# PeterCalifano/gtsam_PeterCdev

Hardware: AMD Instinct MI355X
Metric: lm_iterations_per_sec (higher is better)
Workload: dtype f64; 1 GPU; bal1723; ordering=schur_nd, replicas=1, parallelism=replicas1

## Files before the change

### gtsam_petercdev_amd/csrc/handle.h

```cpp
#pragma once
#include <hip/hip_runtime.h>

#include <algorithm>
#include <new>
#include <stdexcept>
#include <string>
#include <utility>
#include <vector>

#include "gsx_internal.h"
#include "kernels.h"

#define HIPCHK(ctx, expr)                                                                  \
  do {                                                                                     \
    hipError_t e__ = (expr);                                                               \
    if (e__ != hipSuccess) {                                                               \
      (ctx)->err = std::string(#expr) + ": " + hipGetErrorString(e__);                     \
      return GSX_E_NO_DEVICE;                                                              \
    }                                                                                      \
  } while (0)

namespace gsx {

template <class Tp>
// ... 40 lines not shown
};

enum Phase { PH_LINEARIZE, PH_ASSEMBLE_H, PH_FACTORIZE, PH_BACKSOLVE, PH_LINERR, PH_RETRACT, PH_ERROR,
             PH_FACTOR_SMALL, PH_FACTOR_BIG, PH_FACTOR_LEAF, PH_K_SYRK, PH_K_TRSM, PH_K_POTRF0, PH_K_GATHER,
             PH_K_BACKSOLVE, PH_MARGINALS, PH_M_PREP, PH_M_KT, PH_M_SF, PH_M_FF, PH_M_EMIT, PH_M_LEAF, PH_COUNT };

struct Timer {
  std::vector<std::pair<hipEvent_t, hipEvent_t>> pending, pool;
  double ms = 0;
  int64_t count = 0;
};

}

namespace gsx {

struct Context {
  std::string err;
  int device = 0;
  bool has_device = false;
  hipStream_t stream = nullptr;
  HostProblem P;
  Symbolic S;
  bool has_symbolic = false;
  double relax = GSX_AMALGAMATION_AUTO;
  int relax_max_f = 128;
  std::vector<int> order;

  DevBuf<int> d_var_type, d_var_dim, d_var_state_off, d_var_tan_off, d_f_type, d_f_rows, d_f_key_ptr, d_f_vars,
      d_f_noise_kind, d_f_cols;
  DevBuf<i64> d_f_meas_off, d_f_noise_off, d_f_jac_off;
  DevBuf<double> d_meas, d_noise;
  DevBuf<FactorRec> d_frec;
  DevBuf<int> d_type_list[kNumTypeLists];
  int type_count[kNumTypeLists] = {};
  DevProblem DP{};
  int n_smart = 0;
  DevBuf<int> d_smart_slot, d_smart_status, d_smart_counters;
  DevBuf<double> d_smart_cams, d_smart_cache, d_smart_point;
  SmartDev SD{};
  void smart_begin(bool linearize) {
    if (n_smart) hipMemsetAsync(d_smart_counters.p + (linearize ? 0 : 1), 0, (linearize ? 2 : 1) * sizeof(int), stream);
  }
  DevBuf<i64> d_fr_off, d_cmap_ptr, d_gidx_ptr, d_h_off, d_hmap_ptr, d_term_ptr;
  DevBuf<TermRec> d_terms;
  DevBuf<VarRec> d_var_recs;
  DevBuf<ChildRec> d_child_recs;
  DevBuf<FrontRec> d_front_recs;
  DevBuf<i64> d_cond_last, d_cond_prev;
  DevBuf<int> d_cond_front;
  DevBuf<VarRec> d_fvar_recs;
  DevBuf<LeafRec> d_leaf_recs;
  int leaf_base = 0;
  int lin_err_slice = 0;
  DevBuf<int> d_fr_N, d_fr_F, d_fr_nfv, d_fr_fvar_ptr, d_fvars, d_fr_parent, d_fr_lean, d_fr_child_ptr, d_children, d_cmap,
      d_gidx, d_h_rows, d_hmap, d_h_loc, d_sched, d_hvars;
  DevBuf<BigDesc> d_big;
  DevSymbolic DS{};
  std::vector<std::vector<SmallLaunch>> small_launch;
  std::vector<std::vector<SmallLaunch>> leaf_launch;
  std::vector<int> leaf_max_F;
  std::vector<std::vector<SmallLaunch>> rest_launch;
  DevBuf<int> d_usched, d_rest_ids, d_tree_start, d_tree_up, d_tree_npend, d_tree_pending, d_tree_cursor;
  DevBuf<int> d_bst_roots, d_bst_child_ptr, d_bst_children, d_bst_counters;
  DevBuf<unsigned long long> d_bst_ready;
  int bst_roots = 0, bst_total = 0;
  unsigned bst_epoch = 0;
  struct TreeTier {
    int start0, nstart, max_n, threads;
    size_t med_lds;
  };
  std::vector<TreeTier> tree_tiers;
  DevBuf<i64> d_gt_dst;
  DevBuf<GatherSeg> d_gsegs;
  DevBuf<GatherSrc> d_gsrcs;
  DevBuf<int> d_gt_ld, d_gt_dims, d_gm_task, d_gm_slot, d_gm_nslots;
  DevBuf<double> d_gscratch;
  GatherArgs GA{};
  std::vector<BigLevel> big_level;
  struct ConLevel {
    int first = 0, count = 0, max_n = 0;
  };
  std::vector<ConLevel> con_level;
  std::vector<int> con_desc_of_front;
  DevBuf<ConDesc> d_con_descs;
  DevBuf<int> d_con_own_col_ptr, d_con_own_cols, d_con_own_m, d_con_child, d_con_fwd_map, d_con_iwork;
  DevBuf<i64> d_con_own_jac;
  DevBuf<double> d_con_work;
  ConTables CT{};
  int con_hd_n = 0;
  DevBuf<int> d_con_hd_tan, d_con_hd_ptr;
  DevBuf<i64> d_con_hd_jidx;
  DevBuf<double> d_con_hd_w;
  bool constrained() const { return !S.con_fronts.empty(); }
  std::vector<BigDesc> big_descs;
  int big_max_n = 0, big_max_nfv = 0;
  struct HGroup {
    int begin, count, threads, lds;
    bool global;
  };
  std::vector<HGroup> hgroups;
  DevBuf<int2> d_star_bundles;
  int n_star_bundles = 0;
  bool fused_star_env = true;
  bool fused_star = false;
  struct LeafSplit {
    int sbegin, scount;
    int rbegin, rcount;
  };
  std::vector<LeafSplit> leaf_split;
  DevBuf<StarLeafRec> d_star_recs;
  DevBuf<int> d_star_prow;
  DevBuf<LeafRec> d_leaf_rest_recs;
  DevBuf<int> d_star_rest_vars;
  int n_star_rest = 0;
  struct MargLevel {
    int begin[4], count[4];
  };
  struct MargPlan {
    std::vector<MargLevel> levels;
    DevBuf<MargItem> d_items;
    DevBuf<int2> d_emit;
    DevBuf<int> d_leaves;
    DevBuf<i64> d_out_off;
    int n_emit = 0, n_leaves = 0;
    int64_t total = 0;
    bool ready = false;
    void release() {
      levels.clear();
      d_items.release();
      d_emit.release();
      d_leaves.release();
      d_out_off.release();
      n_emit = n_leaves = 0;
      total = 0;
      ready = false;
    }
  };
  MargPlan marg_all;
  DevBuf<i64> d_marg_slot, d_marg_work;
  DevBuf<double> d_marg_cov;
  bool marg_arena = false;
  int64_t marg_cov_doubles = 0;
  void marg_release() {
    marg_all.release();
    d_marg_slot.release();
    d_marg_work.release();
    d_marg_cov.release();
    marg_arena = false;
    marg_cov_doubles = 0;
  }
  DevBuf<double> d_values, d_trial, d_delta, d_udelta, d_jac, d_H, d_arena, d_hdiag, d_damp, d_partials, d_scalars;
  DevBuf<double> d_dlu, d_dld;
  DevBuf<DevStatus> d_status;
  double* h_scalars = nullptr;
  DevStatus* h_status = nullptr;
  static constexpr int kPartials = 4096;
  int solver_kind = GSX_SOLVER_MULTIFRONTAL;
  gsx_pcg_params pcg_params{};
  PcgWork* pcg = nullptr;
  int64_t pcg_iterations = 0, pcg_solves = 0;
  int64_t pcg_run_iterations = 0;
  bool use_pcg() const { return solver_kind == GSX_SOLVER_PCG; }
  double lm_lambda = 0, lm_factor = 0, lm_error = 0;
  int lm_iterations = 0, lm_inner = 0;
  Timer timers[PH_COUNT];
  int profiling = -1;
  int64_t n_cheirality = 0;
  std::vector<LeafRec> h_leaf_recs;
  std::vector<GatherSeg> h_gsegs;
  std::vector<int> hv_list, hv_group_of_var, hv_pos;
  std::vector<int> fr_sched_pos, fr_group;
  std::vector<int> fr_seg_ptr, fr_segs, seg_level;
  std::vector<int> fr_gm_ptr, fr_gms, gm_level;
  struct PartialScratch {
    DevBuf<int> marked, src_off, lists[kNumTypeLists], hv, ids, gm_task, gm_slot, gm_nslots;
    DevBuf<double> states;
    DevBuf<LeafRec> leaf;
    DevBuf<BigDesc> big;
    DevBuf<GatherSeg> segs;
  } ps;
  hipStream_t bulk = nullptr;
  hipEvent_t bulk_go = nullptr, bulk_done = nullptr;
  size_t leaf_side_group0 = 0;
  bool bulk_pending = false;
  int shard_rank = 0, shard_world = 1;
  gsx_allreduce_fn shard_cb = nullptr;
  void* shard_user = nullptr;
  bool shard_failed = false;
  unsigned sc_dirty = 0;
  DevBuf<int> d_f_active;
  DevBuf<unsigned char> d_own_tan, d_sched_tan, d_own_state;
  DevBuf<double> d_xscal;
  std::vector<double> jac_stage;
  bool sharded() const { return shard_world > 1; }
  DevBuf<unsigned char> d_wf_replaced, d_wf_dirty, d_wf_changed;
  DevBuf<double> d_wf_old;
  DevBuf<int> d_wf_ids;
  bool values_set = false, linearized = false, h_ready = false, hdiag_ready = false, solved = false, damp_ready = false;
  bool lin0_ready = false;
  bool fact_valid = false;
  double fact_lambda = 0.0;
  bool fact_pending = false;
  int damp_kind = -1;
  double damp_min = 0, damp_max = 0;
  bool hstar_ready = true;
  bool values_synced = true;
  bool wf_all_replaced = true, wf_clear_pending = true;
  bool wf_delta_valid = false;
  void values_written() {
    values_set = true;
    values_synced = true;
    linearized = h_ready = solved = false;
  }
  void states_scattered() { values_synced = true; }
  void values_gathered() {
    std::swap(d_values.p, d_trial.p);
    values_synced = true;
  }
  void trial_accepted(bool drop_factorization) {
    std::swap(d_values.p, d_trial.p);
    values_synced = false;
    trial_discarded();
    if (drop_factorization) fact_valid = false;
  }
  void trial_discarded() { linearized = h_ready = solved = false; }
  void blocks_written(bool is_linearization) {
    if (is_linearization) linearized = true;
    else hdiag_ready = false;
    h_ready = false;
    lin0_ready = false;
    fact_valid = false;
    solved = false;
    if (damp_kind != 0) damp_ready = false;
  }
  void some_blocks_written() { lin0_ready = false; }
  void linear_graph_given() { linearized = true; }
  void lin0_computed() { lin0_ready = true; }
  void h_assembled(bool star_complete) {
    h_ready = true;
    hstar_ready = star_complete;
    hdiag_ready = false;
  }
  void hstar_completed() { hstar_ready = true; }
  void hdiag_extracted() { hdiag_ready = true; }
  void panels_reassembled() { hdiag_ready = false; }
  bool damping_is(int kind, double mind, double maxd) const {
    return damp_ready && damp_kind == kind && (kind == 0 || (damp_min == mind && damp_max == maxd));
  }
  void damping_made(int kind, double mind, double maxd) {
    damp_ready = true;
    damp_kind = kind;
    damp_min = mind;
    damp_max = maxd;
  }
  void factorization_queued(double lambda) {
    fact_valid = false;
    fact_pending = true;
    fact_lambda = lambda;
    wf_all_replaced = true;
  }
  void factorization_judged(bool bad) {
    if (fact_pending) fact_valid = !bad;
    else if (bad) fact_valid = false;
    fact_pending = false;
  }
  void factorization_failed() { fact_valid = false; }
  void delta_overwritten() { wf_delta_valid = false; }
  void delta_outdated() { solved = false; }
  void step_solved(bool complete_undamped) {
    solved = true;
    if (complete_undamped) {
      wf_delta_valid = true;
      wf_all_replaced = false;
      wf_clear_pending = true;
    }
  }
  void tree_replaced() {
    h_ready = false;
    solved = false;
    fact_valid = fact_pending = false;
    wf_all_replaced = true;
    wf_delta_valid = false;
    damp_ready = hdiag_ready = false;
    if (sharded()) linearized = false;
  }
  void problem_replaced() {
    has_symbolic = values_set = linearized = h_ready = solved = false;
    fact_valid = fact_pending = hdiag_ready = damp_ready = lin0_ready = false;
    wf_delta_valid = false;
    wf_all_replaced = true;
  }
  void problem_uploaded() {
    has_symbolic = true;
    values_set = true;
    values_synced = true;
  }
  void update_finished(bool kept_linearization) { linearized = kept_linearization; }
  hipError_t wf_flags_ready(hipStream_t st) {
    const size_t nf = (size_t)std::max(S.n_fronts, 1);
    if (d_wf_replaced.n != nf) {
      hipError_t e = d_wf_replaced.alloc(nf);
      if (e != hipSuccess) return e;
      wf_clear_pending = true;
    }
    if (wf_clear_pending) {
      hipError_t e = hipMemsetAsync(d_wf_replaced.p, 0, nf, st);
      if (e != hipSuccess) return e;
      wf_clear_pending = false;
    }
    return hipSuccess;
  }
};

int factor_type_list(const HostProblem& P, int f);
void whiten_linear_factor(const HostProblem& P, int f, const double* src, double* J);
gsx_status upload_problem(gsx_context* c);
gsx_status upload_symbolic(gsx_context* c);
void launch_lds_group(const DevProblem& P, const DevSymbolic& S, const int* ids, const SmallLaunch& g, const double* H,
                      const double* damp, const double* scalars, double* arena, DevStatus* status, hipStream_t st);
void timer_begin(gsx_context* c, int ph);
void timer_end(gsx_context* c, int ph);
void dev_linearize(gsx_context* c);
void dev_assemble_h(gsx_context* c);
void dev_ensure_hstar(gsx_context* c);
void dev_damping(gsx_context* c, int diagonal, double mind, double maxd);
void dev_big_factor(gsx_context* c, const BigDesc* descs, int count, const BigPlan& plan, hipStream_t st, bool prof);
void dev_backsolve(gsx_context* c, const WildfireArgs* wf = nullptr);
void dev_linear_error(gsx_context* c, bool solved_step = false);
void dev_retract(gsx_context* c, const double* d_delta);
void dev_error(gsx_context* c, const double* d_vals, int slot);
gsx_status readback(gsx_context* c);
bool factorization_ok(const gsx_context* c);
gsx_status compute_error_sync(gsx_context* c, double* out);
gsx_status need_device(gsx_context* c);
gsx_status begin_call(gsx_context* c, bool need_values, bool need_symbolic);
gsx_status indeterminate(gsx_context* c, uint64_t* bad_key, bool also_nonfinite);
gsx_status download(gsx_context* c, const double* src, double* out, int64_t n);
enum HMode { H_KEEP, H_IF_STALE, H_ALWAYS };
void direct_solve(gsx_context* c, HMode hm, int diagonal, double mind, double maxd, double lambda, bool backsolve);
gsx_status damped_step(gsx_context* c, HMode hm, int diagonal, double mind, double maxd, double lambda);

}

struct gsx_context : gsx::Context {};

#define GSX_GUARD(h, call)                          \
  try {                                             \
    return (call);                                  \
  } catch (const std::bad_alloc&) {                 \
    if (h) (h)->err = "out of host memory";         \
    return GSX_E_NOMEM;                             \
  } catch (const std::exception& e) {               \
    if (h) (h)->err = e.what();                     \
    return GSX_E_INVALID;                           \
  }
```

### gtsam_petercdev_amd/csrc/kernels.h

```cpp
#pragma once
#include <hip/hip_runtime.h>

#include <cstdint>
#include <vector>

#include "../../include/gsx.h"

namespace gsx {

typedef long long i64;

struct FactorRec {
  i64 jac_off;
  int s0, s1;
  int meas_off, noise_off;
  int type_kind;
  int rows_dim;
};
struct DevProblem {
  int n_vars, n_factors;
  const int *var_type, *var_dim, *var_state_off, *var_tan_off;
  const int *f_type, *f_rows, *f_key_ptr, *f_vars, *f_noise_kind, *f_cols;
  const i64 *f_meas_off, *f_noise_off, *f_jac_off;
  const double *meas, *noise;
  const FactorRec* frec;
  const int* f_active;
  int n_active;
};

struct TermRec {
  i64 jac;
  int m, colA, colB, dB, dst, pad;
};

struct VarRec {
  i64 h_off, hmap_off;
  int dA, rows, loc, toff;
};
struct LeafRec {
  i64 off, h_off, hmap_off, gidx_ptr;
  int n, F, nfv, lean;
  int dA, rows, loc, toff;
  int fvar_ptr, front, pad0, pad1;
};
constexpr int kStarMaxD = 3;
struct StarLeafRec {
  i64 off, h_off, t0;
  i64 jac0, prow_off;
  int n, nf, d, toff;
  int colA, colB, colR, dB;
  int front, jstride, rrow, pad0;
};
struct ChildRec {
  i64 src0, cmap_off;
  int nc, s1, pad0, pad1;
};
struct FrontRec {
  i64 off;
  int n, F, nfv, fvar_ptr, child_ptr, nchild;
};

struct DevSymbolic {
  int n_fronts;
  const i64* fr_off;
  const int *fr_N, *fr_F, *fr_nfv, *fr_fvar_ptr, *fvars, *fr_parent, *fr_child_ptr, *children;
  const int* fr_lean;
  const i64 *cmap_ptr, *gidx_ptr;
  const int *cmap, *gidx;
  const i64 *h_off, *hmap_ptr;
  const int *h_rows, *hmap, *h_loc;
  const i64* term_ptr;
  const TermRec* terms;
  const VarRec* var_recs;
  const ChildRec* child_recs;
  const FrontRec* front_recs;
  const VarRec* fvar_recs;
  unsigned char* wf_dirty;
  const unsigned char *wf_replaced, *wf_changed;
};
#ifdef __HIPCC__
__device__ __forceinline__ bool wildfire_skip(const DevSymbolic& S, int f, bool writer) {
  if (S.wf_dirty == nullptr) return false;
  const int p = S.fr_parent[f];
  bool dirty = (p < 0) || S.wf_dirty[p];
  if (dirty && !S.wf_replaced[f]) {
    dirty = false;
    for (int q = S.fr_fvar_ptr[f] + S.fr_nfv[f]; q < S.fr_fvar_ptr[f + 1]; ++q)
      if (S.wf_changed[S.fvars[q]]) {
        dirty = true;
        break;
      }
  }
  if (writer) S.wf_dirty[f] = dirty ? 1 : 0;
  return !dirty;
}
#endif

struct DevStatus {
  int n_fail;
  int first_front;
  int n_nonfinite;
  int n_cheirality;
  int n_backsub;
};

constexpr int kXScalars = 16;
constexpr unsigned kXFact = 1u << 12, kXLin = 1u << 13;
void launch_shard_pack(const double* scalars, const DevStatus* status, unsigned dirty, double* x, hipStream_t st);
void launch_shard_unpack(const double* x, unsigned dirty, double* scalars, DevStatus* status, hipStream_t st);
void launch_scatter_states(const DevProblem& P, const int* vars, const int* src_off, int n, const double* src,
                           double* values, hipStream_t st);
void launch_mask_copy(const double* in, const unsigned char* mask, int64_t n, double* out, hipStream_t st);

enum { SC_LAMBDA = 0, SC_ERR = 1, SC_LIN0 = 2, SC_LIND = 3, SC_TRIAL_ERR = 4, SC_DOT0 = 5, SC_DOT1 = 6, SC_DOT2 = 7,
       SC_DOT3 = 8, SC_LIN0_LOCAL = 9 , SC_COUNT = 12 };

struct BigDesc {
  i64 off, xoff;
  int N, F, front, parent;
};
constexpr int kStandaloneFront = -3;
void launch_cond_check(int n, const i64* last, const i64* prev, const int* front, const double* arena, DevStatus* status,
                       hipStream_t st);
__host__ __device__ inline i64 big_panel_offset(int n) { return ((i64)n * n + 1) & ~(i64)1; }

enum { TL_SFM = 0, TL_BETWEEN_POSE2 = 1, TL_BETWEEN_POSE3 = 2, TL_GENERIC = 3, TL_PROJECTION = 4, TL_BEARINGRANGE = 5,
       TL_RANGE_POSE2_POINT = 6, TL_RANGE_POSE2_POSE = 7, TL_RANGE_POSE3_POINT = 8, TL_RANGE_POSE3_POSE = 9,
       TL_BEARING = 10, TL_STEREO = 11,
       TL_PROJECTION_SENSOR = 12, TL_STEREO_SENSOR = 13, TL_RANGE_POSE2_POINT_SENSOR = 14, TL_RANGE_POSE2_POSE_SENSOR = 15,
       TL_RANGE_POSE3_POINT_SENSOR = 16, TL_RANGE_POSE3_POSE_SENSOR = 17, TL_SFM2 = 18,
       TL_SMART = 19, kNumTypeLists = 20 };
constexpr int kSensorListShift = TL_RANGE_POSE2_POINT_SENSOR - TL_RANGE_POSE2_POINT;
inline int type_list_of(int t, int vt0, int vt1, long long nmeas) {
  switch (t) {
    case GSX_F_LINEAR: return -1;
    case GSX_F_SFM: return TL_SFM;
    case GSX_F_SFM2: return TL_SFM2;
    case GSX_F_PROJECTION: return nmeas > 7 ? TL_PROJECTION_SENSOR : TL_PROJECTION;
    case GSX_F_BEARINGRANGE: return TL_BEARINGRANGE;
    case GSX_F_BETWEEN: return vt0 == GSX_VAR_POSE2 ? TL_BETWEEN_POSE2 : (vt0 == GSX_VAR_POSE3 ? TL_BETWEEN_POSE3 : TL_GENERIC);
    case GSX_F_RANGE:
      return (vt0 == GSX_VAR_POSE2 ? (vt1 == GSX_VAR_POSE2 ? TL_RANGE_POSE2_POSE : TL_RANGE_POSE2_POINT)
                                   : (vt1 == GSX_VAR_POSE3 ? TL_RANGE_POSE3_POSE : TL_RANGE_POSE3_POINT)) +
             (nmeas > 1 ? kSensorListShift : 0);
    case GSX_F_BEARING: return TL_BEARING;
    case GSX_F_STEREO: return nmeas > 9 ? TL_STEREO_SENSOR : TL_STEREO;
    case GSX_F_SMART_PROJECTION: return TL_SMART;
  }
  return TL_GENERIC;
}
struct SmartDev {
  const int* slot;
  double* cams;
  double* cache;
  double* point;
  int* status;
  int* counters;
  int n;
};
void launch_linearize(const DevProblem& P, const int* const type_lists[kNumTypeLists], const int type_counts[kNumTypeLists],
                      const double* values, double* jac, DevStatus* status, hipStream_t st, const SmartDev* smart = nullptr);
void launch_error(const DevProblem& P, const int* const type_lists[kNumTypeLists], const int type_counts[kNumTypeLists],
                  const double* values, double* partials, int n_partials_cap, double* scalars, int slot, hipStream_t st,
                  const SmartDev* smart = nullptr);
void launch_smart_triangulate(const DevProblem& P, const int* list, int n, const double* values, const SmartDev& S, hipStream_t st);
void launch_smart_linearize(const DevProblem& P, const int* list, int n, const SmartDev& S, double* jac, hipStream_t st);
void launch_smart_error(const DevProblem& P, const int* list, int n, const SmartDev& S, double* partials, int blocks,
                        hipStream_t st);
void launch_linear_error(const DevProblem& P, const double* jac, const double* delta, double* partials,
                         int n_partials_cap, double* scalars, int slice, hipStream_t st);
void launch_lin0(const DevProblem& P, const double* jac, double* partials, int cap, double* scalars, hipStream_t st);
void launch_model_error(const DevProblem& P, const DevSymbolic& S, const int* vars, int nvars, const double* H,
                        const double* delta, const double* damp, double* partials, int cap, double* scalars, hipStream_t st);
void launch_retract(const DevProblem& P, const double* values, const double* delta, double* out, hipStream_t st);
void launch_assemble_h_group(const DevProblem& P, const DevSymbolic& S, const int* vars, int count, int threads,
                             int lds_bytes, bool global, const double* jac, double* H, hipStream_t st);
void launch_assemble_h_star_bundles(const DevProblem& P, const DevSymbolic& S, const int* vars, const int2* bundles,
                                    int count, const double* jac, double* H, hipStream_t st);
void launch_assemble_h_diag_star(const DevProblem& P, const DevSymbolic& S, const int* dvars, int dcount, const int* svars,
                                 const int2* bundles, int scount, const double* jac, double* H, hipStream_t st);
void launch_hessian_diag(const DevProblem& P, const DevSymbolic& S, const double* H, double* diag, hipStream_t st);
void launch_make_damping(int n, const double* hdiag, int diagonal, double mind, double maxd, double* damp,
                         hipStream_t st);
void launch_front_small(const DevProblem& P, const DevSymbolic& S, const int* ids, int count, int max_n,
                        int threads, const double* H, const double* damp, const double* scalars, double* arena,
                        DevStatus* status, hipStream_t st);
struct TreeArgs {
  const int* start;
  int nstart;
  int* cursor;
  int* pending;
  const int *up, *npend;
};
void launch_front_tree(const DevProblem& P, const DevSymbolic& S, const TreeArgs& T, int max_n, int threads, const double* H,
                       const double* damp, const double* scalars, double* arena, DevStatus* status, hipStream_t st);
void launch_front_medium(const DevProblem& P, const DevSymbolic& S, const int* ids, int count, int max_panel, int max_n,
                         const double* H, const double* damp, const double* scalars, double* arena, DevStatus* status,
                         hipStream_t st);
void launch_front_tree_med(const DevProblem& P, const DevSymbolic& S, const TreeArgs& T, size_t lds_bytes, const double* H,
                           const double* damp, const double* scalars, double* arena, DevStatus* status, hipStream_t st);
void launch_big_init(const DevProblem& P, const DevSymbolic& S, const BigDesc* descs, int count, int max_n,
                     int max_nfv, const double* H, const double* damp, const double* scalars, double* arena,
                     hipStream_t st);
struct BigPlan {
  int chunk = 0;
  std::vector<int> fw, rb, pairs;
  int rounds() const { return (int)fw.size(); }
};
void plan_big_group(const BigDesc* host_descs, int count, BigPlan& plan);
void launch_big_diag(const BigDesc* descs, int count, const BigPlan& plan, int round, double* arena, DevStatus* status,
                     hipStream_t st);
#ifdef GSX_STAMP
void big_stamp_dump(const char* what);
#endif
size_t big_rows_lds(int fw, long tiles, int cus, int* rows);
void launch_big_rows(const BigDesc* descs, int count, const BigPlan& plan, int round, double* arena, DevStatus* status,
                     hipStream_t st);
void launch_big_schur(const BigDesc* descs, int count, const BigPlan& plan, int round, double* arena, hipStream_t st);
void launch_front_leaf(const DevProblem& P, const DevSymbolic& S, const LeafRec* recs, int count, int max_panel, int threads,
                       const double* H, const double* damp, const double* scalars, double* arena, DevStatus* status,
                       hipStream_t st);
void launch_front_star_leaf(const DevSymbolic& S, const StarLeafRec* recs, int count, const int* prow, const double* jac,
                            const double* damp, const double* scalars, double* H, double* arena, DevStatus* status,
                            hipStream_t st);
struct GatherSrc {
  i64 off;
  int d2;
  int ldF;
};
struct GatherSeg {
  i64 dst;
  i64 src;
  int n, ld, dims;
  int slot;
};
struct GatherArgs {
  const GatherSeg* segs;
  const GatherSrc* srcs;
  const i64* gt_dst;
  const int *gt_ld, *gt_dims, *gm_task, *gm_slot, *gm_nslots;
  double* scratch;
};
void launch_big_gather(const GatherArgs& G, int seg0, int nseg, int m0, int nm, double* arena, hipStream_t st);
void launch_backsolve(const DevSymbolic& S, const int* ids, int count, int threads, int max_n, const double* arena,
                      double* delta, DevStatus* status, hipStream_t st);
size_t backsolve_big_lds(int max_n, int max_F, int max_sep_rows);
void launch_backsolve_big(const DevSymbolic& S, const int* ids, int count, int max_n, int max_F, const double* arena,
                          double* delta, DevStatus* status, hipStream_t st);
bool backsolve_small_fits(int max_n, int max_F);
void launch_backsolve_small(const DevSymbolic& S, const int* ids, int count, int max_F, const double* arena, double* delta,
                            DevStatus* status, hipStream_t st);
struct BacksolveTreeArgs {
  const int* roots;
  int n_roots, n_tickets;
  const int *child_ptr, *children;
  unsigned long long* ready;
  int *head, *tail;
  unsigned epoch;
};
void launch_backsolve_tree(const DevSymbolic& S, const BacksolveTreeArgs& Q, const double* arena, double* delta,
                           DevStatus* status, hipStream_t st);
struct WildfireArgs {
  const unsigned char *replaced, *dirty;
  unsigned char* changed;
  const double* old_delta;
  DevStatus* status;
  double threshold;
};
void launch_mark_fronts(const int* ids, int count, unsigned char* flags, hipStream_t st);
void launch_wildfire_post(const DevSymbolic& S, const int* ids, int count, bool wave_per_clique, const WildfireArgs& W,
                          double* delta, hipStream_t st);
void launch_backsolve_leaf(const DevSymbolic& S, const LeafRec* recs, int count, int max_F, const double* arena,
                           double* delta, DevStatus* status, hipStream_t st);
void launch_gradient(const DevProblem& P, const DevSymbolic& S, const double* H, double* g, hipStream_t st);
void launch_ax_sqnorm(const DevProblem& P, const double* jac, const double* x, double* partials, int cap, double* scalars,
                      int slot, hipStream_t st);
void launch_vec_dot(const double* a, const double* b, int64_t n, double* partials, int cap, double* scalars, int slot,
                    hipStream_t st);
void launch_vec_axpby(double* out, double alpha, const double* a, double beta, const double* b, int64_t n, hipStream_t st);
void launch_marginal_path(const DevSymbolic& S, const int* path, int npath, int loc, int dA, int max_n, const double* arena,
                          double* out, double* Y, int64_t n_tan, hipStream_t st);
void launch_joint_cross(const double* Ya, const double* Yb, int64_t n_tan, int dA, int dB, double* out, hipStream_t st);
struct MargItem {
  int front, ti, tj, pad;
};
struct MargArgs {
  const i64 *slot, *work;
  double* cov;
  const double* arena;
  const i64* out_off;
  const int* var_dim;
  double* out;
};
void launch_marg_prep(const DevSymbolic& S, const MargArgs& M, const MargItem* items, int count, hipStream_t st);
void launch_marg_kt(const DevSymbolic& S, const MargArgs& M, const MargItem* items, int count, hipStream_t st);
void launch_marg_sf(const DevSymbolic& S, const MargArgs& M, const MargItem* items, int count, hipStream_t st);
void launch_marg_ff(const DevSymbolic& S, const MargArgs& M, const MargItem* items, int count, hipStream_t st);
void launch_marg_emit(const DevSymbolic& S, const MargArgs& M, const int2* vars, int count, hipStream_t st);
void launch_marg_leaf(const DevSymbolic& S, const MargArgs& M, const int* ids, int count, hipStream_t st);
void launch_set_scalar(double* scalars, int slot, double v, hipStream_t st);
struct ConDesc {
  i64 off;
  i64 work, fwd;
  i64 iwork;
  int N, F, K, n_fwd;
  int own_begin, own_end;
  int child_begin, child_end;
  int front;
  int fwd_map;
};
struct ConTables {
  const ConDesc* descs;
  const int *own_col_ptr, *own_cols, *own_m;
  const i64* own_jac;
  const int* child_list;
  const int* fwd_map;
  double* work;
  int* iwork;
};
void launch_constraint_fronts(const DevSymbolic& S, const ConTables& T, int first, int count, int max_n, const double* jac,
                              double* arena, DevStatus* status, hipStream_t st);
void launch_constraint_hdiag(int n, const int* tan, const int* ptr, const i64* jidx, const double* w, const double* jac,
                             double* hdiag, hipStream_t st);
constexpr int kTreeCursors = 8;
void launch_begin_factorization(double* scalars, double lambda, DevStatus* status, int* tree_cursors, hipStream_t st);
void launch_dense_partial(double* a, int n, int nf, DevStatus* status, hipStream_t st);
// ... 25 lines not shown
```

### gtsam_petercdev_amd/csrc/kernels.hip

```cpp
#include <hip/hip_runtime.h>

#include <climits>
#include <cstdio>
#include <cstdlib>

#include "device_geometry.h"
#include "gsx_internal.h"
#include "kernels.h"

namespace gsx {
using namespace gsxd;

#define T kTile

__device__ __forceinline__ double wave_sum(double v) {
#pragma unroll
  for (int o = 32; o > 0; o >>= 1) v += __shfl_down(v, o, 64);
  return v;
}
typedef double v4d __attribute__((ext_vector_type(4)));
__device__ __forceinline__ i64 readlane_i64(i64 v, int src_lane) {
  int lo = (int)(v & 0xFFFFFFFFll), hi = (int)(v >> 32);
  lo = __builtin_amdgcn_readlane(lo, src_lane);
  hi = __builtin_amdgcn_readlane(hi, src_lane);
// ... 56 lines not shown
#pragma unroll
    for (int c = 0; c < NC; ++c)
#pragma unroll
      for (int r = 0; r < M; ++r) J[c * M + r] *= inv[r];
  } else if (kind == GSX_NOISE_GAUSSIAN) {
    double R[M * M];
#pragma unroll
    for (int i = 0; i < M * M; ++i) R[i] = np[i];
#pragma unroll
    for (int c = 0; c < NC; ++c) {
      double col[M];
#pragma unroll
      for (int r = 0; r < M; ++r) {
        double s = 0;
#pragma unroll
        for (int k = r; k < M; ++k) s += R[r * M + k] * J[c * M + k];
        col[r] = s;
      }
#pragma unroll
      for (int r = 0; r < M; ++r) J[c * M + r] = col[r];
    }
  }
  if (loss) {
    double s = 0;
#pragma unroll
    for (int r = 0; r < M; ++r) s += J[(NC - 1) * M + r] * J[(NC - 1) * M + r];
    const double w = sqrt(robust_weight(loss, np[noise_base_params(kind, M)], sqrt(s)));
#pragma unroll
    for (int i = 0; i < M * NC; ++i) J[i] *= w;
  }
  if constexpr ((M * NC) % 2 == 0) {
    if ((reinterpret_cast<size_t>(out) & 15) == 0) {
      double2* out2 = reinterpret_cast<double2*>(out);
#pragma unroll
      for (int i = 0; i < M * NC / 2; ++i) out2[i] = double2{J[2 * i], J[2 * i + 1]};
      return;
    }
  }
#pragma unroll
  for (int i = 0; i < M * NC; ++i) out[i] = J[i];
}

template <int M>
__device__ __forceinline__ double whitened_half_sqnorm(double (&e)[M], int kind_full, const double* np) {
  const int kind = kind_full & GSX_NOISE_BASE_MASK, loss = kind_full >> 4;
  double s = 0;
  if (kind == GSX_NOISE_UNIT) {
#pragma unroll
    for (int r = 0; r < M; ++r) s += e[r] * e[r];
  } else if (kind == GSX_NOISE_ISOTROPIC) {
    const double inv = 1.0 / np[0];
#pragma unroll
    for (int r = 0; r < M; ++r) s += (e[r] * inv) * (e[r] * inv);
  } else if (kind == GSX_NOISE_DIAGONAL) {
#pragma unroll
    for (int r = 0; r < M; ++r) {
      const double x = e[r] * (1.0 / np[r]);
      s += x * x;
    }
  } else {
#pragma unroll
    for (int r = 0; r < M; ++r) {
      double x = 0;
#pragma unroll
      for (int k = r; k < M; ++k) x += np[r * M + k] * e[k];
      s += x * x;
    }
  }
  if (loss) return robust_loss(loss, np[noise_base_params(kind, M)], sqrt(s));
  return 0.5 * s;
}

__device__ inline void whiten_inplace(double* J, int m, int nc, int kind_full, const double* np) {
  const int kind = kind_full & GSX_NOISE_BASE_MASK, loss = kind_full >> 4;
  if (kind == GSX_NOISE_UNIT) {
  } else if (kind == GSX_NOISE_ISOTROPIC) {
    const double inv = 1.0 / np[0];
    for (int i = 0; i < m * nc; ++i) J[i] *= inv;
  } else if (kind == GSX_NOISE_DIAGONAL) {
    for (int c = 0; c < nc; ++c)
      for (int r = 0; r < m; ++r) J[c * m + r] *= (1.0 / np[r]);
  } else {
    for (int c = 0; c < nc; ++c)
      for (int r = 0; r < m; ++r) {
        double s = 0;
        for (int k = r; k < m; ++k) s += np[r * m + k] * J[c * m + k];
        J[c * m + r] = s;
      }
  }
  if (loss) {
    double s = 0;
    for (int r = 0; r < m; ++r) s += J[(nc - 1) * m + r] * J[(nc - 1) * m + r];
    const double w = sqrt(robust_weight(loss, np[noise_base_params(kind, m)], sqrt(s)));
    for (int i = 0; i < m * nc; ++i) J[i] *= w;
  }
}

__device__ inline void local_coords(int type, int dim, const double* x, const double* y, double* out) {
  if (type == GSX_VAR_VECTOR) {
    for (int i = 0; i < dim; ++i) out[i] = y[i] - x[i];
  } else if (type == GSX_VAR_POSE2) {
    const P2 h = compose(inverse(load_pose2(x)), load_pose2(y));
    out[0] = h.x; out[1] = h.y; out[2] = theta(h);
  } else {
    pose3_logmap(between(load_pose3(x), load_pose3(y)), out);
    if (type == GSX_VAR_CAMERA) {
      out[6] = y[12] - x[12]; out[7] = y[13] - x[13]; out[8] = y[14] - x[14];
    }
  }
}

__device__ __forceinline__ void linearize_generic_body(const DevProblem& P, const int* list, int n, const double* values,
                                                       double* jac, int bid);
__global__ void __launch_bounds__(256) linearize_sfm_kernel(DevProblem P, const int* list, int n, const double* values,
                                                            double* jac, DevStatus* status, const int* glist, int gn) {
  const int gb = (gn + 255) >> 8;
  if ((int)blockIdx.x < gb) {
    linearize_generic_body(P, glist, gn, values, jac, blockIdx.x);
    return;
  }
  const int i = ((int)blockIdx.x - gb) * blockDim.x + threadIdx.x;
  if (i >= n) return;
  const int f = list[i];
  const FactorRec fr = P.frec[f];
  const double* cam = values + fr.s0;
  const double* pt = values + fr.s1;
  const double* z = P.meas + fr.meas_off;
  double camr[17], ptr3[3], pi[2], H1[18], H2[6], J[26];
#pragma unroll
  for (int k = 0; k < 17; ++k) camr[k] = cam[k];
  ptr3[0] = pt[0]; ptr3[1] = pt[1]; ptr3[2] = pt[2];
  const bool ok = sfm_project(camr, ptr3, pi, H1, H2);
  if (ok) {
#pragma unroll
    for (int c = 0; c < 9; ++c) {
      J[2 * c] = H1[c];
      J[2 * c + 1] = H1[9 + c];
    }
#pragma unroll
    for (int c = 0; c < 3; ++c) {
      J[18 + 2 * c] = H2[c];
      J[18 + 2 * c + 1] = H2[3 + c];
    }
    J[24] = z[0] - pi[0];
    J[25] = z[1] - pi[1];
  } else {
#pragma unroll
    for (int k = 0; k < 26; ++k) J[k] = 0;
    atomicAdd(&status->n_cheirality, 1);
  }
  whiten_store<2, 13>(J, (fr.type_kind >> 8) & 0xffff, P.noise + fr.noise_off, jac + fr.jac_off);
}

__global__ void __launch_bounds__(256) linearize_bearingrange_kernel(DevProblem P, const int* list, int n,
                                                                     const double* values, double* jac) {
  const int i = blockIdx.x * blockDim.x + threadIdx.x;
  if (i >= n) return;
  const int f = list[i];
  const int kp = P.f_key_ptr[f];
  const double* pose = values + P.var_state_off[P.f_vars[kp]];
  const double* pt = values + P.var_state_off[P.f_vars[kp + 1]];
  const double* z = P.meas + P.f_meas_off[f];
  double ps[3] = {pose[0], pose[1], pose[2]}, p2[2] = {pt[0], pt[1]}, br[2], H1[6], H2[4], J[12];
  bearing_range_2d(ps, p2, br, H1, H2);
#pragma unroll
  for (int c = 0; c < 3; ++c) {
    J[2 * c] = H1[c];
    J[2 * c + 1] = H1[3 + c];
  }
#pragma unroll
  for (int c = 0; c < 2; ++c) {
    J[6 + 2 * c] = H2[c];
    J[6 + 2 * c + 1] = H2[2 + c];
  }
  J[10] = -wrap_angle(br[0] - z[0]);
  J[11] = -(br[1] - z[1]);
  whiten_store<2, 6>(J, P.f_noise_kind[f], P.noise + P.f_noise_off[f], jac + P.f_jac_off[f]);
}

template <bool SENSOR>
__global__ void __launch_bounds__(256) linearize_projection_kernel(DevProblem P, const int* list, int n, const double* values,
                                                                   double* jac, DevStatus* status) {
  const int i = blockIdx.x * blockDim.x + threadIdx.x;
  if (i >= n) return;
  const int f = list[i];
  const int kp = P.f_key_ptr[f];
  const double* pose = values + P.var_state_off[P.f_vars[kp]];
  const double* pt = values + P.var_state_off[P.f_vars[kp + 1]];
  const double* z = P.meas + P.f_meas_off[f];
  double pr[12], p3[3], K[5], pi[2], H1[12], H2[6], J[20];
#pragma unroll
  for (int k = 0; k < 12; ++k) pr[k] = pose[k];
  p3[0] = pt[0]; p3[1] = pt[1]; p3[2] = pt[2];
#pragma unroll
  for (int k = 0; k < 5; ++k) K[k] = z[2 + k];
  if constexpr (SENSOR) pose3_compose_sensor(pr, z + 7);
  if (pinhole_project_s2(pr, p3, K, pi, H1, H2)) {
    if constexpr (SENSOR) {
      row_times_sensor_adjoint(H1, z + 7);
      row_times_sensor_adjoint(H1 + 6, z + 7);
    }
#pragma unroll
    for (int c = 0; c < 6; ++c) {
      J[2 * c] = H1[c];
      J[2 * c + 1] = H1[6 + c];
    }
#pragma unroll
    for (int c = 0; c < 3; ++c) {
      J[12 + 2 * c] = H2[c];
      J[12 + 2 * c + 1] = H2[3 + c];
    }
    J[18] = z[0] - pi[0];
    J[19] = z[1] - pi[1];
  } else {
#pragma unroll
    for (int k = 0; k < 18; ++k) J[k] = 0;
    J[18] = J[19] = -2.0 * K[0];
    if constexpr (SENSOR) atomicAdd(&status->n_cheirality, 1);
  }
  whiten_store<2, 10>(J, P.f_noise_kind[f], P.noise + P.f_noise_off[f], jac + P.f_jac_off[f]);
}

__global__ void __launch_bounds__(256) linearize_between_pose2_kernel(DevProblem P, const int* list, int n,
                                                                      const double* values, double* jac, const int* glist,
                                                                      int gn) {
  const int gb = (gn + 255) >> 8;
  if ((int)blockIdx.x < gb) {
    linearize_generic_body(P, glist, gn, values, jac, blockIdx.x);
    return;
  }
  const int i = ((int)blockIdx.x - gb) * blockDim.x + threadIdx.x;
  if (i >= n) return;
  const int f = list[i];
  const FactorRec fr = P.frec[f];
  const P2 x1 = load_pose2(values + fr.s0);
  const P2 x2 = load_pose2(values + fr.s1);
  const P2 h = compose(inverse(x1), x2);
  const P2 zh = compose(inverse(load_pose2(P.meas + fr.meas_off)), h);
  const P2 hi = inverse(h);
  double J[21];
  J[0] = -hi.c; J[1] = -hi.s; J[2] = 0;
  J[3] = hi.s; J[4] = -hi.c; J[5] = 0;
  J[6] = -hi.y; J[7] = hi.x; J[8] = -1;
  J[9] = 1; J[10] = 0; J[11] = 0;
  J[12] = 0; J[13] = 1; J[14] = 0;
  J[15] = 0; J[16] = 0; J[17] = 1;
  J[18] = -zh.x; J[19] = -zh.y; J[20] = -theta(zh);
  whiten_store<3, 7>(J, (fr.type_kind >> 8) & 0xffff, P.noise + fr.noise_off, jac + fr.jac_off);
}

__global__ void __launch_bounds__(256) linearize_between_pose3_kernel(DevProblem P, const int* list, int n,
                                                                      const double* values, double* jac, const int* glist,
                                                                      int gn) {
  const int gb = (gn + 255) >> 8;
  if ((int)blockIdx.x < gb) {
    linearize_generic_body(P, glist, gn, values, jac, blockIdx.x);
    return;
  }
  const int i = ((int)blockIdx.x - gb) * blockDim.x + threadIdx.x;
  if (i >= n) return;
  const int f = list[i];
  const FactorRec fr = P.frec[f];
  const P3 x1 = load_pose3(values + fr.s0);
  const P3 x2 = load_pose3(values + fr.s1);
  const P3 h = between(x1, x2);
  const P3 zh = compose(inverse(load_pose3(P.meas + fr.meas_off)), h);
  double e[6], Ad[36], J[78];
  pose3_logmap(zh, e);
  pose3_adjoint(inverse(h), Ad);
#pragma unroll
  for (int c = 0; c < 6; ++c)
#pragma unroll
    for (int r = 0; r < 6; ++r) {
      J[c * 6 + r] = -Ad[6 * r + c];
      J[36 + c * 6 + r] = (r == c) ? 1.0 : 0.0;
    }
#pragma unroll
  for (int r = 0; r < 6; ++r) J[72 + r] = -e[r];
  whiten_store<6, 13>(J, (fr.type_kind >> 8) & 0xffff, P.noise + fr.noise_off, jac + fr.jac_off);
}

__device__ __forceinline__ void linearize_generic_body(const DevProblem& P, const int* list, int n, const double* values,
                                                       double* jac, int bid) {
  const int i = bid * blockDim.x + threadIdx.x;
  if (i >= n) return;
  const int f = list[i];
  const int kp = P.f_key_ptr[f];
  const int m = P.f_rows[f];
  double* J = jac + P.f_jac_off[f];
  const double* z = P.meas + P.f_meas_off[f];
  if (P.f_type[f] == GSX_F_PRIOR) {
    const int v = P.f_vars[kp];
    double l[9];
    local_coords(P.var_type[v], P.var_dim[v], values + P.var_state_off[v], z, l);
    for (int c = 0; c < m; ++c)
      for (int r = 0; r < m; ++r) J[c * m + r] = (r == c) ? 1.0 : 0.0;
    for (int r = 0; r < m; ++r) J[m * m + r] = l[r];
    whiten_inplace(J, m, m + 1, P.f_noise_kind[f], P.noise + P.f_noise_off[f]);
  } else {
    const double* x1 = values + P.var_state_off[P.f_vars[kp]];
    const double* x2 = values + P.var_state_off[P.f_vars[kp + 1]];
    for (int c = 0; c < m; ++c)
      for (int r = 0; r < m; ++r) {
        J[c * m + r] = (r == c) ? -1.0 : 0.0;
        J[m * m + c * m + r] = (r == c) ? 1.0 : 0.0;
      }
    for (int r = 0; r < m; ++r) J[2 * m * m + r] = -((x2[r] - x1[r]) - z[r]);
    whiten_inplace(J, m, 2 * m + 1, P.f_noise_kind[f], P.noise + P.f_noise_off[f]);
  }
}
__global__ void linearize_generic_kernel(DevProblem P, const int* list, int n, const double* values, double* jac) {
  linearize_generic_body(P, list, n, values, jac, blockIdx.x);
}

template <int V1, int V2, bool SENSOR>
__global__ void __launch_bounds__(256) linearize_range_kernel(DevProblem P, const int* list, int n, const double* values,
                                                              double* jac) {
  const int i = blockIdx.x * blockDim.x + threadIdx.x;
  if (i >= n) return;
  const FactorRec fr = P.frec[list[i]];
  const double* a1 = values + fr.s0;
  const double* a2 = values + fr.s1;
  const double z = P.meas[fr.meas_off];
  if constexpr (V1 == GSX_VAR_POSE2) {
    constexpr int NC = (V2 == GSX_VAR_POSE2) ? 7 : 6;
    double ps[3] = {a1[0], a1[1], a1[2]}, p2[2] = {a2[0], a2[1]}, H1[3], Dd[2], J[NC];
    double r;
    if constexpr (SENSOR) {
      r = range_2d_cs(pose2_compose_sensor(ps, P.meas + fr.meas_off + 1), p2, H1, Dd);
      row_times_sensor_adjoint2(H1, P.meas + fr.meas_off + 1);
    } else {
      r = range_2d(ps, p2, H1, Dd);
    }
    J[0] = H1[0]; J[1] = H1[1]; J[2] = H1[2];
    if constexpr (V2 == GSX_VAR_POSE2) {
      const double c2 = cos(a2[2]), s2 = sin(a2[2]);
      J[3] = Dd[0] * c2 + Dd[1] * s2; J[4] = -Dd[0] * s2 + Dd[1] * c2; J[5] = 0.0;
    } else {
      J[3] = Dd[0]; J[4] = Dd[1];
    }
    J[NC - 1] = -(r - z);
    whiten_store<1, NC>(J, (fr.type_kind >> 8) & 0xffff, P.noise + fr.noise_off, jac + fr.jac_off);
  } else {
    constexpr int NC = (V2 == GSX_VAR_POSE3) ? 13 : 10;
    constexpr int TO = (V2 == GSX_VAR_POSE3) ? 9 : 0;
    double pr[12], p3[3] = {a2[TO], a2[TO + 1], a2[TO + 2]}, H1[6], H2[3], J[NC];
#pragma unroll
    for (int k = 0; k < 12; ++k) pr[k] = a1[k];
    if constexpr (SENSOR) pose3_compose_sensor(pr, P.meas + fr.meas_off + 1);
    const double r = range_3d(pr, p3, H1, H2);
    if constexpr (SENSOR) row_times_sensor_adjoint(H1, P.meas + fr.meas_off + 1);
#pragma unroll
    for (int c = 0; c < 6; ++c) J[c] = H1[c];
    if constexpr (V2 == GSX_VAR_POSE3) {
      J[6] = J[7] = J[8] = 0.0;
#pragma unroll
      for (int c = 0; c < 3; ++c) J[9 + c] = H2[0] * a2[c] + H2[1] * a2[3 + c] + H2[2] * a2[6 + c];
    } else {
      J[6] = H2[0]; J[7] = H2[1]; J[8] = H2[2];
    }
    J[NC - 1] = -(r - z);
    whiten_store<1, NC>(J, (fr.type_kind >> 8) & 0xffff, P.noise + fr.noise_off, jac + fr.jac_off);
  }
}

__global__ void __launch_bounds__(256) linearize_bearing_kernel(DevProblem P, const int* list, int n, const double* values,
                                                                double* jac) {
  const int i = blockIdx.x * blockDim.x + threadIdx.x;
  if (i >= n) return;
  const FactorRec fr = P.frec[list[i]];
  const double* pose = values + fr.s0;
  const double* pt = values + fr.s1;
  double ps[3] = {pose[0], pose[1], pose[2]}, p2[2] = {pt[0], pt[1]}, br[2], H1[6], H2[4], J[6];
  bearing_range_2d(ps, p2, br, H1, H2);
  J[0] = H1[0]; J[1] = H1[1]; J[2] = H1[2];
  J[3] = H2[0]; J[4] = H2[1];
  J[5] = -wrap_angle(br[0] - P.meas[fr.meas_off]);
  whiten_store<1, 6>(J, (fr.type_kind >> 8) & 0xffff, P.noise + fr.noise_off, jac + fr.jac_off);
}

template <bool SENSOR>
__global__ void __launch_bounds__(256) linearize_stereo_kernel(DevProblem P, const int* list, int n, const double* values,
                                                               double* jac, DevStatus* status) {
  const int i = blockIdx.x * blockDim.x + threadIdx.x;
  if (i >= n) return;
  const FactorRec fr = P.frec[list[i]];
  const double* pose = values + fr.s0;
  const double* pt = values + fr.s1;
  const double* z = P.meas + fr.meas_off;
  double pr[12], p3[3], K[6], pi[3], H1[18], H2[9], J[30];
#pragma unroll
  for (int k = 0; k < 12; ++k) pr[k] = pose[k];
  p3[0] = pt[0]; p3[1] = pt[1]; p3[2] = pt[2];
#pragma unroll
  for (int k = 0; k < 6; ++k) K[k] = z[3 + k];
  if constexpr (SENSOR) pose3_compose_sensor(pr, z + 9);
  if (stereo_project(pr, p3, K, pi, H1, H2)) {
    if constexpr (SENSOR) {
#pragma unroll
      for (int r = 0; r < 3; ++r) row_times_sensor_adjoint(H1 + 6 * r, z + 9);
    }
#pragma unroll
    for (int c = 0; c < 6; ++c)
#pragma unroll
      for (int r = 0; r < 3; ++r) J[3 * c + r] = H1[6 * r + c];
#pragma unroll
    for (int c = 0; c < 3; ++c)
#pragma unroll
      for (int r = 0; r < 3; ++r) J[18 + 3 * c + r] = H2[3 * r + c];
#pragma unroll
    for (int r = 0; r < 3; ++r) J[27 + r] = z[r] - pi[r];
  } else {
#pragma unroll
    for (int k = 0; k < 27; ++k) J[k] = 0;
    J[27] = J[28] = J[29] = -2.0 * K[0];
    if constexpr (SENSOR) atomicAdd(&status->n_cheirality, 1);
  }
  whiten_store<3, 10>(J, (fr.type_kind >> 8) & 0xffff, P.noise + fr.noise_off, jac + fr.jac_off);
}

__global__ void __launch_bounds__(256) linearize_sfm2_kernel(DevProblem P, const int* list, int n, const double* values,
                                                             double* jac, DevStatus* status) {
  const int i = blockIdx.x * blockDim.x + threadIdx.x;
  if (i >= n) return;
  const int f = list[i];
  const FactorRec fr = P.frec[f];
  const double* pose = values + fr.s0;
  const double* pt = values + fr.s1;
  const double* cal = values + P.var_state_off[P.f_vars[P.f_key_ptr[f] + 2]];
  const double* z = P.meas + fr.meas_off;
  double pr[12], p3[3], K[5], pi[2], H1[12], H2[6], H3[10], J[30];
#pragma unroll
  for (int k = 0; k < 12; ++k) pr[k] = pose[k];
  p3[0] = pt[0]; p3[1] = pt[1]; p3[2] = pt[2];
#pragma unroll
  for (int k = 0; k < 5; ++k) K[k] = cal[k];
  if (pinhole_project_s2_cal(pr, p3, K, pi, H1, H2, H3)) {
#pragma unroll
    for (int c = 0; c < 6; ++c) {
      J[2 * c] = H1[c];
      J[2 * c + 1] = H1[6 + c];
    }
#pragma unroll
    for (int c = 0; c < 3; ++c) {
      J[12 + 2 * c] = H2[c];
      J[12 + 2 * c + 1] = H2[3 + c];
    }
#pragma unroll
    for (int c = 0; c < 5; ++c) {
      J[18 + 2 * c] = H3[c];
      J[18 + 2 * c + 1] = H3[5 + c];
    }
    J[28] = z[0] - pi[0];
    J[29] = z[1] - pi[1];
  } else {
#pragma unroll
    for (int k = 0; k < 30; ++k) J[k] = 0;
    atomicAdd(&status->n_cheirality, 1);
  }
  whiten_store<2, 15>(J, (fr.type_kind >> 8) & 0xffff, P.noise + fr.noise_off, jac + fr.jac_off);
}

void launch_linearize(const DevProblem& P, const int* const type_lists[kNumTypeLists], const int type_counts[kNumTypeLists],
                      const double* values, double* jac, DevStatus* status, hipStream_t st, const SmartDev* smart) {
  auto grid = [](int n) { return dim3((n + 255) / 256); };
  const int* glist = type_lists[3];
  int gn = type_counts[3];
  auto take = [&](int n) {
    const int g = gn;
    gn = 0;
    return std::make_pair(dim3((n + 255) / 256 + (g + 255) / 256), g);
  };
  if (type_counts[0]) {
    const auto gg = take(type_counts[0]);
    linearize_sfm_kernel<<<gg.first, 256, 0, st>>>(P, type_lists[0], type_counts[0], values, jac, status, glist, gg.second);
  }
  if (type_counts[1]) {
    const auto gg = take(type_counts[1]);
    linearize_between_pose2_kernel<<<gg.first, 256, 0, st>>>(P, type_lists[1], type_counts[1], values, jac, glist, gg.second);
  }
  if (type_counts[2]) {
    const auto gg = take(type_counts[2]);
    linearize_between_pose3_kernel<<<gg.first, 256, 0, st>>>(P, type_lists[2], type_counts[2], values, jac, glist, gg.second);
  }
  if (gn) linearize_generic_kernel<<<grid(gn), 256, 0, st>>>(P, glist, gn, values, jac);
  if (type_counts[4])
    linearize_projection_kernel<false><<<grid(type_counts[4]), 256, 0, st>>>(P, type_lists[4], type_counts[4], values, jac,
                                                                             status);
  if (type_counts[5])
    linearize_bearingrange_kernel<<<grid(type_counts[5]), 256, 0, st>>>(P, type_lists[5], type_counts[5], values, jac);
  auto run = [&](auto kernel, int k) {
    if (type_counts[k]) kernel<<<grid(type_counts[k]), 256, 0, st>>>(P, type_lists[k], type_counts[k], values, jac);
  };
  run(linearize_range_kernel<GSX_VAR_POSE2, GSX_VAR_VECTOR, false>, TL_RANGE_POSE2_POINT);
  run(linearize_range_kernel<GSX_VAR_POSE2, GSX_VAR_POSE2, false>, TL_RANGE_POSE2_POSE);
  run(linearize_range_kernel<GSX_VAR_POSE3, GSX_VAR_VECTOR, false>, TL_RANGE_POSE3_POINT);
  run(linearize_range_kernel<GSX_VAR_POSE3, GSX_VAR_POSE3, false>, TL_RANGE_POSE3_POSE);
  run(linearize_bearing_kernel, TL_BEARING);
  auto run_s = [&](auto kernel, int k) {
    if (type_counts[k]) kernel<<<grid(type_counts[k]), 256, 0, st>>>(P, type_lists[k], type_counts[k], values, jac, status);
  };
  run_s(linearize_stereo_kernel<false>, TL_STEREO);
  run_s(linearize_projection_kernel<true>, TL_PROJECTION_SENSOR);
  run_s(linearize_stereo_kernel<true>, TL_STEREO_SENSOR);
  run(linearize_range_kernel<GSX_VAR_POSE2, GSX_VAR_VECTOR, true>, TL_RANGE_POSE2_POINT_SENSOR);
  run(linearize_range_kernel<GSX_VAR_POSE2, GSX_VAR_POSE2, true>, TL_RANGE_POSE2_POSE_SENSOR);
  run(linearize_range_kernel<GSX_VAR_POSE3, GSX_VAR_VECTOR, true>, TL_RANGE_POSE3_POINT_SENSOR);
  run(linearize_range_kernel<GSX_VAR_POSE3, GSX_VAR_POSE3, true>, TL_RANGE_POSE3_POSE_SENSOR);
  run_s(linearize_sfm2_kernel, TL_SFM2);
  if (type_counts[TL_SMART] && smart) {
    launch_smart_triangulate(P, type_lists[TL_SMART], type_counts[TL_SMART], values, *smart, st);
    launch_smart_linearize(P, type_lists[TL_SMART], type_counts[TL_SMART], *smart, jac, st);
  }
}

template <int FT = -1, int FV = -1, bool SENSOR = false>
__device__ inline double factor_error(const DevProblem& P, int f, const double* values) {
  const FactorRec fr = P.frec[f];
  const int type = FT >= 0 ? FT : (fr.type_kind & 0xff);
  if (type == GSX_F_LINEAR) return 0.0;
  const int kind = (fr.type_kind >> 8) & 0xffff;
  const double* np = P.noise + fr.noise_off;
  const double* z = P.meas + fr.meas_off;
  if (type == GSX_F_SFM) {
    const double* cam = values + fr.s0;
    const double* pt = values + fr.s1;
    double camr[17], ptr3[3], pi[2], e[2];
#pragma unroll
    for (int k = 0; k < 17; ++k) camr[k] = cam[k];
    ptr3[0] = pt[0]; ptr3[1] = pt[1]; ptr3[2] = pt[2];
    if (!sfm_project(camr, ptr3, pi, nullptr, nullptr)) return 0.0;
    e[0] = pi[0] - z[0];
    e[1] = pi[1] - z[1];
    return whitened_half_sqnorm<2>(e, kind, np);
  }
  if (type == GSX_F_BEARINGRANGE) {
    const double* pose = values + fr.s0;
    const double* pt = values + fr.s1;
    double ps[3] = {pose[0], pose[1], pose[2]}, p2[2] = {pt[0], pt[1]}, br[2], e[2];
    bearing_range_2d(ps, p2, br, nullptr, nullptr);
    e[0] = wrap_angle(br[0] - z[0]);
    e[1] = br[1] - z[1];
    return whitened_half_sqnorm<2>(e, kind, np);
  }
  if (type == GSX_F_PROJECTION) {
    const double* pose = values + fr.s0;
    const double* pt = values + fr.s1;
    double pr[12], p3[3], K[5], pi[2], e[2];
#pragma unroll
    for (int k = 0; k < 12; ++k) pr[k] = pose[k];
    p3[0] = pt[0]; p3[1] = pt[1]; p3[2] = pt[2];
#pragma unroll
    for (int k = 0; k < 5; ++k) K[k] = z[2 + k];
    if constexpr (SENSOR) pose3_compose_sensor(pr, z + 7);
    if (pinhole_project_s2(pr, p3, K, pi, nullptr, nullptr)) {
      e[0] = pi[0] - z[0];
      e[1] = pi[1] - z[1];
    } else {
      e[0] = e[1] = 2.0 * K[0];
    }
    return whitened_half_sqnorm<2>(e, kind, np);
  }
  if constexpr (FT == GSX_F_RANGE && FV == GSX_VAR_POSE2) {
    const double* a1 = values + fr.s0;
    const double* a2 = values + fr.s1;
    double ps[3] = {a1[0], a1[1], a1[2]}, p2[2] = {a2[0], a2[1]}, e[1];
    if constexpr (SENSOR) e[0] = range_2d_cs(pose2_compose_sensor(ps, z + 1), p2, nullptr, nullptr) - z[0];
    else e[0] = range_2d(ps, p2, nullptr, nullptr) - z[0];
    return whitened_half_sqnorm<1>(e, kind, np);
  }
  if constexpr (FT == GSX_F_RANGE && FV == GSX_VAR_POSE3) {
    const double* a1 = values + fr.s0;
    const double* a2 = values + fr.s1 + ((fr.rows_dim >> 16) == 13 ? 9 : 0);
    double pr[12], p3[3] = {a2[0], a2[1], a2[2]}, e[1];
#pragma unroll
    for (int k = 0; k < 12; ++k) pr[k] = a1[k];
    if constexpr (SENSOR) pose3_compose_sensor(pr, z + 1);
    e[0] = range_3d(pr, p3, nullptr, nullptr) - z[0];
    return whitened_half_sqnorm<1>(e, kind, np);
  }
  if constexpr (FT == GSX_F_BEARING) {
    const double* pose = values + fr.s0;
    const double* pt = values + fr.s1;
    double ps[3] = {pose[0], pose[1], pose[2]}, p2[2] = {pt[0], pt[1]}, br[2], e[1];
    bearing_range_2d(ps, p2, br, nullptr, nullptr);
    e[0] = wrap_angle(br[0] - z[0]);
    return whitened_half_sqnorm<1>(e, kind, np);
  }
  if constexpr (FT == GSX_F_STEREO) {
    const double* pose = values + fr.s0;
    const double* pt = values + fr.s1;
    double pr[12], p3[3], K[6], pi[3], e[3];
#pragma unroll
    for (int k = 0; k < 12; ++k) pr[k] = pose[k];
    p3[0] = pt[0]; p3[1] = pt[1]; p3[2] = pt[2];
#pragma unroll
    for (int k = 0; k < 6; ++k) K[k] = z[3 + k];
    if constexpr (SENSOR) pose3_compose_sensor(pr, z + 9);
    if (stereo_project(pr, p3, K, pi, nullptr, nullptr)) {
#pragma unroll
      for (int r = 0; r < 3; ++r) e[r] = pi[r] - z[r];
    } else {
      e[0] = e[1] = e[2] = 2.0 * K[0];
    }
    return whitened_half_sqnorm<3>(e, kind, np);
  }
  if constexpr (FT == GSX_F_SFM2) {
    const double* pose = values + fr.s0;
    const double* pt = values + fr.s1;
    const double* cal = values + P.var_state_off[P.f_vars[P.f_key_ptr[f] + 2]];
    double pr[12], p3[3], K[5], pi[2], e[2];
#pragma unroll
    for (int k = 0; k < 12; ++k) pr[k] = pose[k];
    p3[0] = pt[0]; p3[1] = pt[1]; p3[2] = pt[2];
#pragma unroll
    for (int k = 0; k < 5; ++k) K[k] = cal[k];
    if (!pinhole_project_s2(pr, p3, K, pi, nullptr, nullptr)) return 0.0;
    e[0] = pi[0] - z[0];
    e[1] = pi[1] - z[1];
    return whitened_half_sqnorm<2>(e, kind, np);
  }
  const int vt = FV >= 0 ? FV : ((fr.type_kind >> 24) & 0xff);
  if (type == GSX_F_BETWEEN && vt == GSX_VAR_POSE2) {
    const P2 h = compose(inverse(load_pose2(values + fr.s0)), load_pose2(values + fr.s1));
    const P2 zh = compose(inverse(load_pose2(z)), h);
    double e[3] = {zh.x, zh.y, theta(zh)};
    return whitened_half_sqnorm<3>(e, kind, np);
  }
  if (type == GSX_F_BETWEEN && vt == GSX_VAR_POSE3) {
    const P3 h = between(load_pose3(values + fr.s0), load_pose3(values + fr.s1));
    double e[6];
    pose3_logmap(compose(inverse(load_pose3(z)), h), e);
    return whitened_half_sqnorm<6>(e, kind, np);
  }
  const int m = fr.rows_dim & 0xff;
  double e[9];
  if (type == GSX_F_PRIOR) {
    local_coords(vt, (fr.rows_dim >> 8) & 0xff, values + fr.s0, z, e);
  } else {
    const double* x1 = values + fr.s0;
    const double* x2 = values + fr.s1;
    for (int r = 0; r < m; ++r) e[r] = (x2[r] - x1[r]) - z[r];
  }
  const int base = kind & GSX_NOISE_BASE_MASK, loss = kind >> 4;
  double s = 0;
  for (int r = 0; r < m; ++r) {
    double x;
    if (base == GSX_NOISE_UNIT) x = e[r];
    else if (base == GSX_NOISE_ISOTROPIC) x = e[r] * (1.0 / np[0]);
    else if (base == GSX_NOISE_DIAGONAL) x = e[r] * (1.0 / np[r]);
    else {
      x = 0;
      for (int k = r; k < m; ++k) x += np[r * m + k] * e[k];
    }
    s += x * x;
  }
  if (loss) return robust_loss(loss, np[noise_base_params(base, m)], sqrt(s));
  return 0.5 * s;
}

__global__ void __launch_bounds__(256) reduce_final_kernel(const double* partials, int n, int stride, double* scalars,
                                                           int slot) {
  double acc = 0;
  for (int i = threadIdx.x; i < n; i += blockDim.x) acc += partials[(size_t)i * stride];
  const double s = block_sum(acc);
  if (threadIdx.x == 0) scalars[slot] = s;
}

__global__ void __launch_bounds__(256) reduce_final_pair_kernel(const double* partials, int n, double* scalars, int slot0) {
  double acc = 0;
  for (int i = threadIdx.x; i < n; i += blockDim.x) acc += partials[(size_t)i * 2 + blockIdx.x];
  const double s = block_sum(acc);
  if (threadIdx.x == 0) scalars[slot0 + blockIdx.x] = s;
}

template <int FT, int FV, bool SENSOR = false>
__global__ void __launch_bounds__(256) error_list_kernel(DevProblem P, const int* list, int n, const double* values,
                                                         double* partials) {
  double acc = 0;
  for (int i = blockIdx.x * blockDim.x + threadIdx.x; i < n; i += gridDim.x * blockDim.x)
    acc += factor_error<FT, FV, SENSOR>(P, list[i], values);
  const double s = block_sum(acc);
  if (threadIdx.x == 0) partials[blockIdx.x] = s;
}

void launch_error(const DevProblem& P, const int* const type_lists[kNumTypeLists],
                  const int type_counts[kNumTypeLists], const double* values, double* partials, int cap, double* scalars,
                  int slot, hipStream_t st, const SmartDev* smart) {
  long long total = 0;
  for (int k = 0; k < kNumTypeLists; ++k) total += type_counts[k];
  bool new_lists = false;
  for (int k = TL_PROJECTION_SENSOR; k < TL_SMART; ++k) new_lists = new_lists || type_counts[k] > 0;
  const int held = type_counts[TL_SMART] > 0 ? kNumTypeLists : (new_lists ? TL_SMART : TL_PROJECTION_SENSOR);
  int off = 0;
  for (int k = 0; k < kNumTypeLists; ++k) {
    const int n = type_counts[k];
    if (!n) continue;
    int nb = (n + 255) / 256;
    const int share = (int)std::max<long long>(1, (long long)(cap - held) * n / std::max<long long>(total, 1));
    nb = std::min(nb, share);
    double* out = partials + off;
    switch (k) {
      case 0: error_list_kernel<GSX_F_SFM, GSX_VAR_CAMERA><<<nb, 256, 0, st>>>(P, type_lists[k], n, values, out); break;
      case 1: error_list_kernel<GSX_F_BETWEEN, GSX_VAR_POSE2><<<nb, 256, 0, st>>>(P, type_lists[k], n, values, out); break;
      case 2: error_list_kernel<GSX_F_BETWEEN, GSX_VAR_POSE3><<<nb, 256, 0, st>>>(P, type_lists[k], n, values, out); break;
      case 4: error_list_kernel<GSX_F_PROJECTION, GSX_VAR_POSE3><<<nb, 256, 0, st>>>(P, type_lists[k], n, values, out); break;
      case 5: error_list_kernel<GSX_F_BEARINGRANGE, GSX_VAR_POSE2><<<nb, 256, 0, st>>>(P, type_lists[k], n, values, out); break;
      case TL_RANGE_POSE2_POINT:
      case TL_RANGE_POSE2_POSE: error_list_kernel<GSX_F_RANGE, GSX_VAR_POSE2><<<nb, 256, 0, st>>>(P, type_lists[k], n, values, out); break;
      case TL_RANGE_POSE3_POINT:
      case TL_RANGE_POSE3_POSE: error_list_kernel<GSX_F_RANGE, GSX_VAR_POSE3><<<nb, 256, 0, st>>>(P, type_lists[k], n, values, out); break;
      case TL_BEARING: error_list_kernel<GSX_F_BEARING, GSX_VAR_POSE2><<<nb, 256, 0, st>>>(P, type_lists[k], n, values, out); break;
      case TL_STEREO: error_list_kernel<GSX_F_STEREO, GSX_VAR_POSE3><<<nb, 256, 0, st>>>(P, type_lists[k], n, values, out); break;
      case TL_PROJECTION_SENSOR: error_list_kernel<GSX_F_PROJECTION, GSX_VAR_POSE3, true><<<nb, 256, 0, st>>>(P, type_lists[k], n, values, out); break;
      case TL_STEREO_SENSOR: error_list_kernel<GSX_F_STEREO, GSX_VAR_POSE3, true><<<nb, 256, 0, st>>>(P, type_lists[k], n, values, out); break;
      case TL_RANGE_POSE2_POINT_SENSOR:
      case TL_RANGE_POSE2_POSE_SENSOR: error_list_kernel<GSX_F_RANGE, GSX_VAR_POSE2, true><<<nb, 256, 0, st>>>(P, type_lists[k], n, values, out); break;
      case TL_RANGE_POSE3_POINT_SENSOR:
      case TL_RANGE_POSE3_POSE_SENSOR: error_list_kernel<GSX_F_RANGE, GSX_VAR_POSE3, true><<<nb, 256, 0, st>>>(P, type_lists[k], n, values, out); break;
      case TL_SFM2: error_list_kernel<GSX_F_SFM2, GSX_VAR_POSE3><<<nb, 256, 0, st>>>(P, type_lists[k], n, values, out); break;
      case TL_SMART:
        launch_smart_triangulate(P, type_lists[k], n, values, *smart, st);
        launch_smart_error(P, type_lists[k], n, *smart, out, nb, st);
        break;
      default: error_list_kernel<-1, -1><<<nb, 256, 0, st>>>(P, type_lists[k], n, values, out); break;
    }
    off += nb;
  }
  reduce_final_kernel<<<1, 256, 0, st>>>(partials, off, 1, scalars, slot);
}

__global__ void __launch_bounds__(256) linear_error_kernel(DevProblem P, const double* jac, const double* delta,
                                                           double* partials) {
  double acc0 = 0, accd = 0;
  for (int i = blockIdx.x * blockDim.x + threadIdx.x; i < P.n_active; i += gridDim.x * blockDim.x) {
    const int f = P.f_active ? P.f_active[i] : i;
    const int m = P.f_rows[f], nc = P.f_cols[f];
    const double* J = jac + P.f_jac_off[f];
    if (m == 2 && (P.f_jac_off[f] & 1) == 0) {
      const double2* J2 = reinterpret_cast<const double2*>(J);
      const double2 b = J2[nc - 1];
      double e0 = -b.x, e1 = -b.y;
      int col = 0;
      for (int k = P.f_key_ptr[f]; k < P.f_key_ptr[f + 1]; ++k) {
        const int v = P.f_vars[k];
        const double* x = delta + P.var_tan_off[v];
        const int d = P.var_dim[v];
        for (int c = 0; c < d; ++c, ++col) {
          const double2 j = J2[col];
          e0 += j.x * x[c];
          e1 += j.y * x[c];
        }
      }
      acc0 += b.x * b.x;
      accd += e0 * e0;
      acc0 += b.y * b.y;
      accd += e1 * e1;
      continue;
    }
    for (int r = 0; r < m; ++r) {
      const double b = J[(nc - 1) * m + r];
      double e = -b;
      int col = 0;
      for (int k = P.f_key_ptr[f]; k < P.f_key_ptr[f + 1]; ++k) {
        const int v = P.f_vars[k];
        const double* x = delta + P.var_tan_off[v];
        const int d = P.var_dim[v];
        for (int c = 0; c < d; ++c, ++col) e += J[col * m + r] * x[c];
      }
      acc0 += b * b;
      accd += e * e;
    }
  }
  const double s0 = block_sum(0.5 * acc0);
  const double sd = block_sum(0.5 * accd);
  if (threadIdx.x == 0) {
    partials[2 * blockIdx.x] = s0;
    partials[2 * blockIdx.x + 1] = sd;
  }
}

__global__ void __launch_bounds__(128) linear_error_staged_kernel(DevProblem P, const double* jac, const double* delta,
                                                                  double* partials, int slice) {
  extern __shared__ double stage[];
  const int wave = threadIdx.x >> 6, lane = threadIdx.x & 63;
  double* W = stage + (size_t)wave * slice;
  const int ngroups = (P.n_factors + 63) >> 6;
  double acc0 = 0, accd = 0;
  for (int g = blockIdx.x * 2 + wave; g < ngroups; g += gridDim.x * 2) {
    const int i0 = g * 64;
    const bool live = i0 + lane < P.n_factors;
    const int f = live ? i0 + lane : P.n_factors - 1;
    const int m = P.f_rows[f], nc = P.f_cols[f];
    const i64 off = P.f_jac_off[f];
    const i64 base = readlane_i64(off, 0);
    const int last = min(63, P.n_factors - 1 - i0);
    const int len = (int)(readlane_i64(off + (i64)m * nc, last) - base);
    const double* src = jac + base;
    for (int e0 = lane; e0 < len; e0 += 64 * 8) {
      double v[8];
#pragma unroll
      for (int u = 0; u < 8; ++u) v[u] = (e0 + 64 * u < len) ? src[e0 + 64 * u] : 0.0;
#pragma unroll
      for (int u = 0; u < 8; ++u)
        if (e0 + 64 * u < len) W[e0 + 64 * u] = v[u];
    }
    asm volatile("s_waitcnt lgkmcnt(0)" ::: "memory");
    __builtin_amdgcn_wave_barrier();
    if (live) {
      const double* J = W + (off - base);
      for (int r = 0; r < m; ++r) {
        const double b = J[(nc - 1) * m + r];
        double e = -b;
        int col = 0;
        for (int k = P.f_key_ptr[f]; k < P.f_key_ptr[f + 1]; ++k) {
          const int v = P.f_vars[k];
          const double* x = delta + P.var_tan_off[v];
          const int d = P.var_dim[v];
          for (int c = 0; c < d; ++c, ++col) e += J[col * m + r] * x[c];
        }
        acc0 += b * b;
        accd += e * e;
      }
    }
    asm volatile("s_waitcnt lgkmcnt(0)" ::: "memory");
    __builtin_amdgcn_wave_barrier();
  }
  const double s0 = block_sum(0.5 * acc0);
  const double sd = block_sum(0.5 * accd);
  if (threadIdx.x == 0) {
    partials[2 * blockIdx.x] = s0;
    partials[2 * blockIdx.x + 1] = sd;
  }
}

void launch_linear_error(const DevProblem& P, const double* jac, const double* delta, double* partials, int cap,
                         double* scalars, int slice, hipStream_t st) {
  int nb;
  if (slice > 0 && !P.f_active) {
    static bool attr = false;
    if (!attr) {
      hipFuncSetAttribute((const void*)linear_error_staged_kernel, hipFuncAttributeMaxDynamicSharedMemorySize, 128 * 1024);
      attr = true;
    }
    nb = ((P.n_factors + 63) / 64 + 1) / 2;
    nb = nb < 1 ? 1 : (nb > cap / 2 ? cap / 2 : nb);
    linear_error_staged_kernel<<<nb, 128, (size_t)2 * slice * sizeof(double), st>>>(P, jac, delta, partials, slice);
  } else {
    nb = (P.n_active + 255) / 256;
    nb = nb < 1 ? 1 : (nb > cap / 2 ? cap / 2 : nb);
    linear_error_kernel<<<nb, 256, 0, st>>>(P, jac, delta, partials);
  }
  static_assert(SC_LIND == SC_LIN0 + 1, "the two linearized errors are reduced by one launch, a block each");
  reduce_final_pair_kernel<<<2, 256, 0, st>>>(partials, nb, scalars, SC_LIN0);
}

__global__ void __launch_bounds__(256) lin0_kernel(DevProblem P, const double* jac, double* partials) {
  double acc = 0;
  for (int k = blockIdx.x * blockDim.x + threadIdx.x; k < P.n_active; k += gridDim.x * blockDim.x) {
    const int f = P.f_active ? P.f_active[k] : k;
    const FactorRec fr = P.frec[f];
    const int m = fr.rows_dim & 0xff;
    const double* b = jac + fr.jac_off + (i64)m * (int)(((unsigned)fr.rows_dim >> 16) - 1u);
    double s = 0;
    for (int r = 0; r < m; ++r) s += b[r] * b[r];
    acc += 0.5 * s;
  }
  const double t = block_sum(acc);
  if (threadIdx.x == 0) partials[blockIdx.x] = t;
}
__global__ void __launch_bounds__(256) model_error_kernel(DevProblem P, DevSymbolic S, const int* vars, int nvars,
                                                          const double* H, const double* delta, const double* damp,
                                                          const double* scalars, double* partials) {
  const double lambda = scalars[SC_LAMBDA];
  double acc = 0;
  for (int k = blockIdx.x * blockDim.x + threadIdx.x; k < nvars; k += gridDim.x * blockDim.x) {
    const int v = vars[k];
    const int d = P.var_dim[v], rows = S.h_rows[v], to = P.var_tan_off[v];
    const double* p = H + S.h_off[v] + (rows - 1);
    for (int j = 0; j < d; ++j) {
      const double x = delta[to + j];
      acc += x * (p[(i64)j * rows] + lambda * damp[to + j] * x);
    }
  }
  const double t = block_sum(acc);
  if (threadIdx.x == 0) partials[blockIdx.x] = t;
}
__global__ void __launch_bounds__(256) model_final_kernel(const double* partials, int n, double* scalars) {
  double acc = 0;
  for (int i = threadIdx.x; i < n; i += blockDim.x) acc += partials[i];
  const double s = block_sum(acc);
  if (threadIdx.x == 0) {
    const double e0 = scalars[SC_LIN0_LOCAL];
    scalars[SC_LIN0] = e0;
    scalars[SC_LIND] = e0 - 0.5 * s;
  }
}
void launch_lin0(const DevProblem& P, const double* jac, double* partials, int cap, double* scalars, hipStream_t st) {
  int nb = (P.n_active + 255) / 256;
  nb = nb < 1 ? 1 : (nb > cap ? cap : nb);
  lin0_kernel<<<nb, 256, 0, st>>>(P, jac, partials);
  reduce_final_kernel<<<1, 256, 0, st>>>(partials, nb, 1, scalars, SC_LIN0_LOCAL);
}
void launch_model_error(const DevProblem& P, const DevSymbolic& S, const int* vars, int nvars, const double* H,
                        const double* delta, const double* damp, double* partials, int cap, double* scalars,
                        hipStream_t st) {
  int nb = (nvars + 255) / 256;
  nb = nb < 1 ? 1 : (nb > cap ? cap : nb);
  model_error_kernel<<<nb, 256, 0, st>>>(P, S, vars, nvars, H, delta, damp, scalars, partials);
  model_final_kernel<<<1, 256, 0, st>>>(partials, nb, scalars);
}

__global__ void __launch_bounds__(256) retract_kernel(DevProblem P, const double* values, const double* delta,
                                                      double* out) {
  const int v = blockIdx.x * blockDim.x + threadIdx.x;
  if (v >= P.n_vars) return;
  const double* x = values + P.var_state_off[v];
  const double* d = delta + P.var_tan_off[v];
  double* y = out + P.var_state_off[v];
  const int type = P.var_type[v];
  if (type == GSX_VAR_VECTOR) {
    for (int i = 0; i < P.var_dim[v]; ++i) y[i] = x[i] + d[i];
  } else if (type == GSX_VAR_POSE2) {
    const P2 r = compose(load_pose2(x), load_pose2(d));
    y[0] = r.x; y[1] = r.y; y[2] = theta(r);
  } else {
    double xi[6];
#pragma unroll
    for (int i = 0; i < 6; ++i) xi[i] = d[i];
    store_pose3(compose(load_pose3(x), pose3_expmap(xi)), y);
    if (type == GSX_VAR_CAMERA) {
      y[12] = x[12] + d[6]; y[13] = x[13] + d[7]; y[14] = x[14] + d[8];
      y[15] = x[15]; y[16] = x[16];
    }
  }
}
void launch_retract(const DevProblem& P, const double* values, const double* delta, double* out, hipStream_t st) {
  if (P.n_vars) retract_kernel<<<(P.n_vars + 255) / 256, 256, 0, st>>>(P, values, delta, out);
}

__global__ void assemble_h_kernel(DevProblem P, DevSymbolic S, const int* vars, const double* jac, double* H) {
  extern __shared__ double lds[];
  const int v = vars[blockIdx.x];
  const int dA = P.var_dim[v], rows = S.h_rows[v], psize = rows * dA;
  const int wave = threadIdx.x >> 6, lane = threadIdx.x & 63, nw = blockDim.x >> 6;
  double* panel = lds + (size_t)wave * psize;
  for (int e = lane; e < psize; e += 64) panel[e] = 0;
  constexpr int kTG = 3;
  const int uw = __builtin_amdgcn_readfirstlane(wave);
  const i64 tb0 = S.term_ptr[v], tn = S.term_ptr[v + 1] - tb0;
  const i64 chunk = ((tn + nw - 1) / nw + 1) & ~i64(1);
  const i64 t1 = min(tb0 + tn, tb0 + (uw + 1) * chunk);
  for (i64 base = tb0 + uw * chunk; base < t1; base += 64) {
    const int nblk = (int)min((i64)64, t1 - base);
    TermRec rec{0, 0, 0, 0, 0, 0, 0};
    if (lane < nblk) rec = S.terms[base + lane];
    for (int g = 0; g < nblk; g += kTG) {
      const double* tj[kTG];
      int tm[kTG], tA[kTG], tB[kTG], tdB[kTG], tdst[kTG];
      float trd[kTG];
      bool tpair[kTG];
      int mmax = 0, nemax = 0;
#pragma unroll
      for (int i = 0; i < kTG; ++i) {
        const int src = min(g + i, 63);
        const bool in = g + i < nblk;
        const i64 joff = readlane_i64(rec.jac, src);
        tj[i] = jac + joff;
        tm[i] = in ? __builtin_amdgcn_readlane(rec.m, src) : 0;
        tA[i] = __builtin_amdgcn_readlane(rec.colA, src);
        tB[i] = __builtin_amdgcn_readlane(rec.colB, src);
        tdB[i] = in ? __builtin_amdgcn_readlane(rec.dB, src) : 0;
        tdst[i] = __builtin_amdgcn_readlane(rec.dst, src);
        trd[i] = __builtin_amdgcn_rcpf((float)max(tdB[i], 1));
        tpair[i] = tm[i] == 2 && (joff & 1) == 0;
        mmax = max(mmax, tm[i]);
        nemax = max(nemax, tdB[i] * dA);
      }
      for (int e = lane; e < nemax; e += 64) {
        double acc[kTG], a0[kTG], b0[kTG], a1[kTG], b1[kTG];
        unsigned oa[kTG], ob[kTG];
        bool on[kTG];
        int ii[kTG], jj[kTG];
#pragma unroll
        for (int i = 0; i < kTG; ++i) {
          on[i] = e < tdB[i] * dA;
          divmod_small(e, tdB[i], trd[i], jj[i], ii[i]);
          oa[i] = (unsigned)((tB[i] + ii[i]) * tm[i]);
          ob[i] = (unsigned)((tA[i] + jj[i]) * tm[i]);
        }
#pragma unroll
        for (int i = 0; i < kTG; ++i) {
          if (tpair[i]) {
            double2 av = {0.0, 0.0}, bv = {0.0, 0.0};
            if (on[i]) {
              av = *reinterpret_cast<const double2*>(tj[i] + oa[i]);
              bv = *reinterpret_cast<const double2*>(tj[i] + ob[i]);
            }
            a0[i] = av.x; a1[i] = av.y; b0[i] = bv.x; b1[i] = bv.y;
          } else {
            const bool r0 = on[i] && tm[i] > 0, r1 = on[i] && tm[i] > 1;
            a0[i] = r0 ? tj[i][oa[i]] : 0.0;
            b0[i] = r0 ? tj[i][ob[i]] : 0.0;
            a1[i] = r1 ? tj[i][oa[i] + 1u] : 0.0;
            b1[i] = r1 ? tj[i][ob[i] + 1u] : 0.0;
          }
        }
#pragma unroll
        for (int i = 0; i < kTG; ++i) acc[i] = a0[i] * b0[i] + a1[i] * b1[i];
        for (int r = 2; r < mmax; ++r) {
          double ar[kTG], br[kTG];
#pragma unroll
          for (int i = 0; i < kTG; ++i) {
            const bool rr = on[i] && r < tm[i];
            ar[i] = rr ? tj[i][oa[i] + (unsigned)r] : 0.0;
            br[i] = rr ? tj[i][ob[i] + (unsigned)r] : 0.0;
          }
#pragma unroll
          for (int i = 0; i < kTG; ++i) acc[i] += ar[i] * br[i];
        }
#pragma unroll
        for (int i = 0; i < kTG; ++i)
          if (on[i]) panel[tdst[i] + ii[i] + jj[i] * rows] += acc[i];
      }
    }
  }
  __syncthreads();
  double* out = H + S.h_off[v];
  for (int e = threadIdx.x; e < psize; e += blockDim.x) {
    double s = 0;
    for (int w = 0; w < nw; ++w) s += lds[(size_t)w * psize + e];
    out[e] = s;
  }
}
constexpr int kTF = 8;
__global__ void __launch_bounds__(256) assemble_h_tile_kernel(DevProblem P, DevSymbolic S, const int* vars, int count,
                                                              int panel_stride, const double* jac, double* H) {
  extern __shared__ double lds[];
  const int wave = threadIdx.x >> 6, lane = threadIdx.x & 63;
  const int slot = __builtin_amdgcn_readfirstlane(blockIdx.x * 4 + wave);
  if (slot >= count) return;
  const int v = vars[slot];
  const int dA = P.var_dim[v], rows = S.h_rows[v], psize = rows * dA;
  double* panel = lds + (size_t)wave * panel_stride;
  for (int e = lane; e < psize; e += 64) panel[e] = 0;
  const i64 tb0 = S.term_ptr[v];
  const int nt = (int)(S.term_ptr[v + 1] - tb0);
  TermRec rec{0, 0, 0, 0, 0, 0, 0};
  if (lane < nt) rec = S.terms[tb0 + lane];
  const int li = lane & 15, lk = lane >> 4;
  int t = 0;
  while (t < nt) {
    int fbeg[kTF + 1];
    double x0[kTF], x1[kTF];
    int nf = 0, tt = t;
#pragma unroll
    for (int q = 0; q < kTF; ++q) {
      fbeg[q] = tt;
      if (tt < nt) {
        const i64 jo = readlane_i64(rec.jac, tt);
        int te = tt + 1;
        while (te < nt && readlane_i64(rec.jac, te) == jo) ++te;
        const int m = __builtin_amdgcn_readlane(rec.m, tt);
        const int ncols = __builtin_amdgcn_readlane(rec.colB, te - 1) + 1;
        const double* J = jac + jo;
        const bool in = li < ncols;
        x0[q] = (in && lk < m) ? J[li * m + lk] : 0.0;
        x1[q] = (in && lk + 4 < m) ? J[li * m + lk + 4] : 0.0;
        tt = te;
        nf = q + 1;
      } else {
        x0[q] = x1[q] = 0.0;
      }
    }
    fbeg[kTF] = tt;
#pragma unroll
    for (int q = 0; q < kTF; ++q) {
      if (q >= nf) break;
      v4d g = {0.0, 0.0, 0.0, 0.0};
      g = __builtin_amdgcn_mfma_f64_16x16x4f64(x0[q], x0[q], g, 0, 0, 0);
      g = __builtin_amdgcn_mfma_f64_16x16x4f64(x1[q], x1[q], g, 0, 0, 0);
      const int te = fbeg[q + 1];
      for (int k = fbeg[q]; k < te; ++k) {
        const int colA = __builtin_amdgcn_readlane(rec.colA, k), colB = __builtin_amdgcn_readlane(rec.colB, k);
        const int dB = __builtin_amdgcn_readlane(rec.dB, k), dst = __builtin_amdgcn_readlane(rec.dst, k);
        const int j = li - colA;
        if (j >= 0 && j < dA) {
#pragma unroll
          for (int r4 = 0; r4 < 4; ++r4) {
            const int i = lk + 4 * r4 - colB;
            if (i >= 0 && i < dB) panel[dst + i + j * rows] += g[r4];
// ... 2198 lines not shown
```

### gtsam_petercdev_amd/csrc/optimizers.hip

```cpp
#include <hip/hip_runtime.h>

#include <algorithm>
#include <cstdlib>
#include <chrono>
#include <climits>
#include <cmath>
#include <cstdio>
#include <cstring>
#include <limits>
#include <array>
#include <map>
#include <string>
#include <vector>

#include "handle.h"

using namespace gsx;

using namespace gsx;

namespace {

struct Trace {
  gsx_lm_result* r;
  void push(double err, double lambda, int acc) {
    if (!r) return;
    if (r->trace_len < r->trace_cap) {
      if (r->trace_error) r->trace_error[r->trace_len] = err;
      if (r->trace_lambda) r->trace_lambda[r->trace_len] = lambda;
      if (r->trace_accepted) r->trace_accepted[r->trace_len] = acc;
    }
    r->trace_len++;
  }
};

gsx_status lm_try_lambda(gsx_context* c, const gsx_lm_params& p, Trace& tr, gsx_lm_result* res, bool* done) {
  gsx_status ps = damped_step(c, H_KEEP, p.diagonal_damping, p.min_diagonal, p.max_diagonal, c->lm_lambda);
  if (ps != GSX_OK && ps != GSX_E_INDETERMINATE) return ps;
  const bool pcg_ok = ps == GSX_OK;
  if (!pcg_ok) hipMemsetAsync(c->d_delta.p, 0, (size_t)c->P.tan_size * sizeof(double), c->stream);
  dev_linear_error(c, true);
  dev_retract(c, c->d_delta.p);
  dev_error(c, c->d_trial.p, SC_TRIAL_ERR);
  gsx_status st = readback(c);
  if (st != GSX_OK) return st;
  const bool solved = c->use_pcg() ? pcg_ok : factorization_ok(c);
  if (!solved && res) res->n_solve_failures++;
  gsx_lm_state ctl{c->lm_lambda, c->lm_factor, c->lm_error, c->lm_iterations, c->lm_inner};
  gsx_lm_decision d;
  gsx_lm_decide(&p, &ctl, solved, c->h_scalars[SC_LIN0], c->h_scalars[SC_LIND], c->h_scalars[SC_TRIAL_ERR], &d);
  if (p.verbosity >= 1)
    std::printf("%4d %12.6g %12.2e %10.2e %6d\n", c->lm_iterations, d.trial_cost, d.cost_change, d.lambda_tried, d.solved);
  if (d.verdict == GSX_LM_TAKE) c->trial_accepted(true);
  c->lm_lambda = ctl.lambda;
  c->lm_factor = ctl.factor;
  c->lm_error = ctl.cost;
  c->lm_iterations = ctl.outer_iterations;
  c->lm_inner = ctl.inner_iterations;
  tr.push(d.trial_cost, d.lambda_tried, d.verdict == GSX_LM_TAKE ? 1 : (solved ? 0 : -1));
  *done = d.verdict != GSX_LM_RETRY;
  return GSX_OK;
}

gsx_status lm_iterate(gsx_context* c, const gsx_lm_params& p, Trace& tr, gsx_lm_result* res) {
  dev_linearize(c);
  if (!c->use_pcg() || p.diagonal_damping) dev_assemble_h(c);
  bool done = false;
  while (!done) {
    gsx_status st = lm_try_lambda(c, p, tr, res, &done);
    if (st != GSX_OK) return st;
  }
  return GSX_OK;
}

bool check_convergence(double relTol, double absTol, double errTol, double currentError, double newError) {
  if (newError <= errTol) return true;
  const double absoluteDecrease = currentError - newError;
  const double relativeDecrease = absoluteDecrease / currentError;
  return (relTol && (relativeDecrease <= relTol)) || (absoluteDecrease <= absTol);
}

template <class Iterate>
gsx_status default_optimize(gsx_context* h, int max_iterations, double relTol, double absTol, double errTol,
                            gsx_lm_result* r, Iterate& iterate) {
  gsx_status st = compute_error_sync(h, &h->lm_error);
  if (st != GSX_OK) return st;
  h->lm_iterations = 0;
  h->pcg_run_iterations = 0;
  Trace tr{r};
  if (r) {
    r->initial_error = h->lm_error;
    r->trace_len = 0;
    r->n_solve_failures = 0;
  }
  double currentError = h->lm_error;
  if (!(currentError <= errTol) && !(h->lm_iterations >= max_iterations)) {
    double newError = currentError;
    do {
      currentError = newError;
      st = iterate(tr);
      if (st != GSX_OK) return st;
      newError = h->lm_error;
    } while (h->lm_iterations < max_iterations && !check_convergence(relTol, absTol, errTol, currentError, newError) &&
             std::isfinite(currentError));
  }
  if (r) {
    r->final_error = h->lm_error;
    r->iterations = h->lm_iterations;
    r->inner_iterations = h->lm_iterations;
    if (h->use_pcg()) r->pcg_iterations = (int32_t)h->pcg_run_iterations;
  }
  return GSX_OK;
}

}

extern "C" {

void gsx_lm_params_legacy(gsx_lm_params* p) {
  *p = gsx_lm_params{100, 1e-5, 1e-5, 0.0, 1e-5, 10.0, 1e5, 0.0, 1e-3, 0, 1, 1e-6, 1e32, 0};
}
void gsx_lm_params_ceres(gsx_lm_params* p) {
  *p = gsx_lm_params{50, 1e-6, 0.0, 0.0, 1e-4, 2.0, 1e32, 1e-16, 1e-3, 1, 0, 1e-6, 1e32, 0};
}

gsx_status gsx_lm_reset(gsx_handle h, const gsx_lm_params* p) {
  if (!h || !p) return GSX_E_INVALID;
  gsx_status st = begin_call(h, true, false);
  if (st != GSX_OK) return st;
  st = compute_error_sync(h, &h->lm_error);
  if (st != GSX_OK) return st;
  h->lm_lambda = p->lambda_initial;
  h->lm_factor = p->lambda_factor;
  h->lm_iterations = 0;
  h->lm_inner = 0;
  return GSX_OK;
}

gsx_status gsx_lm_iterate(gsx_handle h, const gsx_lm_params* p, double* error, double* lambda) {
  if (!h || !p) return GSX_E_INVALID;
  gsx_status st = begin_call(h, true, true);
  if (st != GSX_OK) return st;
  Trace tr{nullptr};
  st = lm_iterate(h, *p, tr, nullptr);
  if (st != GSX_OK) return st;
  if (error) *error = h->lm_error;
  if (lambda) *lambda = h->lm_lambda;
  return GSX_OK;
}

gsx_status gsx_lm_trial(gsx_handle h, int32_t relinearize, double lambda, int32_t diagonal_damping, double min_diagonal,
                        double max_diagonal, double* lin0, double* lind, double* trial_error) {
  if (!h || !(lambda >= 0.0)) return GSX_E_INVALID;
  gsx_status st = begin_call(h, true, true);
  if (st != GSX_OK) return st;
  if (!relinearize && !h->linearized) {
    h->err = "linearize first";
    return GSX_E_STATE;
  }
  if (relinearize) dev_linearize(h);
  st = damped_step(h, H_IF_STALE, diagonal_damping, min_diagonal, max_diagonal, lambda);
  if (st != GSX_OK) return st;
  dev_linear_error(h, true);
  dev_retract(h, h->d_delta.p);
  dev_error(h, h->d_trial.p, SC_TRIAL_ERR);
  st = readback(h);
  if (st != GSX_OK) return st;
  if (!h->use_pcg()) {
    st = indeterminate(h, nullptr, true);
    if (st != GSX_OK) {
      h->delta_outdated();
      return st;
    }
  }
  h->step_solved(false);
  if (lin0) *lin0 = h->h_scalars[SC_LIN0];
  if (lind) *lind = h->h_scalars[SC_LIND];
  if (trial_error) *trial_error = h->h_scalars[SC_TRIAL_ERR];
  return GSX_OK;
}

gsx_status gsx_lm_optimize(gsx_handle h, const gsx_lm_params* p, gsx_lm_result* r) {
  if (!h || !p) return GSX_E_INVALID;
  gsx_status st = begin_call(h, true, true);
  if (st != GSX_OK) return st;
  h->lm_lambda = p->lambda_initial;
  h->lm_factor = p->lambda_factor;
  h->lm_inner = 0;
  auto iterate = [&](Trace& tr) -> gsx_status { return lm_iterate(h, *p, tr, r); };
  st = default_optimize(h, p->max_iterations, p->relative_error_tol, p->absolute_error_tol, p->error_tol, r, iterate);
  if (st == GSX_OK && r) {
    r->final_lambda = h->lm_lambda;
    r->inner_iterations = h->lm_inner;
  }
  return st;
}

gsx_status gsx_gn_optimize(gsx_handle h, int32_t max_iterations, double relTol, double absTol, double errTol,
                           gsx_lm_result* r) {
  if (!h) return GSX_E_INVALID;
  gsx_status st = begin_call(h, true, true);
  if (st != GSX_OK) return st;
  auto iterate = [&](Trace& tr) -> gsx_status {
    dev_linearize(h);
    gsx_status is = damped_step(h, H_ALWAYS, 0, 0, 0, 0.0);
    if (is != GSX_OK) return is;
    dev_retract(h, h->d_delta.p);
    dev_error(h, h->d_trial.p, SC_TRIAL_ERR);
    is = readback(h);
    if (is != GSX_OK) return is;
    if (!h->use_pcg()) {
      is = indeterminate(h, nullptr, true);
      if (is != GSX_OK) return is;
    }
    h->trial_accepted(false);
    h->lm_error = h->h_scalars[SC_TRIAL_ERR];
    h->lm_iterations++;
    tr.push(h->lm_error, 0.0, 1);
    return GSX_OK;
  };
  st = default_optimize(h, max_iterations, relTol, absTol, errTol, r, iterate);
  if (st == GSX_OK && r) r->final_lambda = 0;
  return st;
}

static void dogleg_coefficients(double delta, double uu, double nn, double un, double* cu, double* cn) {
  const double deltaSq = delta * delta;
  if (deltaSq < uu) {
    *cu = std::sqrt(deltaSq / uu);
    *cn = 0.0;
  } else if (deltaSq < nn) {
    const double a = uu - 2. * un + nn, b = 2. * (un - uu), c = uu - deltaSq;
    const double sq = std::sqrt(b * b - 4 * a * c);
    const double tau1 = (-b + sq) / (2. * a), tau2 = (-b - sq) / (2. * a);
    const double eps = std::numeric_limits<double>::epsilon();
    const double tau = (-eps <= tau1 && tau1 <= 1.0 + eps) ? tau1 : tau2;
    *cu = 1. - tau;
    *cn = tau;
  } else {
    *cu = 0.0;
    *cn = 1.0;
  }
}

gsx_status gsx_dogleg_point(double delta, const double* dx_u, const double* dx_n, int64_t n, double* out) {
  if (!dx_u || !dx_n || !out || n < 0 || !(delta >= 0)) return GSX_E_INVALID;
  double uu = 0, nn = 0, un = 0;
  for (int64_t i = 0; i < n; ++i) {
    uu += dx_u[i] * dx_u[i];
    nn += dx_n[i] * dx_n[i];
    un += dx_u[i] * dx_n[i];
  }
  double cu, cn;
  dogleg_coefficients(delta, uu, nn, un, &cu, &cn);
  for (int64_t i = 0; i < n; ++i) out[i] = (cn == 0.0 ? cu * dx_u[i] : (cu == 0.0 ? dx_n[i] : cu * dx_u[i] + cn * dx_n[i]));
  return GSX_OK;
}

gsx_status gsx_dogleg_optimize(gsx_handle h, double delta_initial, int32_t max_iterations, double relTol, double absTol,
                               double errTol, gsx_lm_result* r) {
  if (!h || !(delta_initial >= 0)) return GSX_E_INVALID;
  gsx_status st = begin_call(h, true, true);
  if (st != GSX_OK) return st;
  if (h->sharded()) {
    h->err = "Dogleg is not available on a sharded handle";
    return GSX_E_STATE;
  }
  if (h->constrained()) {
    h->err = "Dogleg is not available on a problem with hard constraints";
    return GSX_E_STATE;
  }
  if (h->use_pcg()) {
    h->err = "Dogleg is not available on a handle whose linear solver is PCG";
    return GSX_E_STATE;
  }
  const int64_t nt = h->P.tan_size;
  if (!h->d_dlu.p) {
    HIPCHK(h, h->d_dlu.alloc(std::max<int64_t>(nt, 1)));
    HIPCHK(h, h->d_dld.alloc(std::max<int64_t>(nt, 1)));
  }
  double delta = delta_initial;
  auto iterate = [&](Trace& tr) -> gsx_status {
    dev_linearize(h);
    direct_solve(h, H_ALWAYS, 0, 0, 0, 0.0, true);
    dev_ensure_hstar(h);
    launch_gradient(h->DP, h->DS, h->d_H.p, h->d_dlu.p, h->stream);
    launch_vec_dot(h->d_dlu.p, h->d_dlu.p, nt, h->d_partials.p, gsx_context::kPartials, h->d_scalars.p, SC_DOT0, h->stream);
    launch_ax_sqnorm(h->DP, h->d_jac.p, h->d_dlu.p, h->d_partials.p, gsx_context::kPartials, h->d_scalars.p, SC_DOT1,
                     h->stream);
    launch_vec_dot(h->d_delta.p, h->d_delta.p, nt, h->d_partials.p, gsx_context::kPartials, h->d_scalars.p, SC_DOT2,
                   h->stream);
    launch_vec_dot(h->d_dlu.p, h->d_delta.p, nt, h->d_partials.p, gsx_context::kPartials, h->d_scalars.p, SC_DOT3,
                   h->stream);
    gsx_status is = readback(h);
    if (is != GSX_OK) return is;
    is = indeterminate(h, nullptr, true);
    if (is != GSX_OK) return is;
    const double gg = h->h_scalars[SC_DOT0], ag2 = h->h_scalars[SC_DOT1];
    const double step = gg / ag2;
    const double uu = step * step * gg, nn = h->h_scalars[SC_DOT2], un = step * h->h_scalars[SC_DOT3];
    const double f_error = h->lm_error;
    double result_f = f_error, cu = 0, cn = 0;
    bool stay = true, zero_step = false;
    while (stay) {
      dogleg_coefficients(delta, uu, nn, un, &cu, &cn);
      launch_vec_axpby(h->d_dld.p, cu * step, h->d_dlu.p, cn, h->d_delta.p, nt, h->stream);
      dev_retract(h, h->d_dld.p);
      dev_error(h, h->d_trial.p, SC_TRIAL_ERR);
      launch_linear_error(h->DP, h->d_jac.p, h->d_dld.p, h->d_partials.p, gsx_context::kPartials, h->d_scalars.p,
                          h->lin_err_slice, h->stream);
      is = readback(h);
      if (is != GSX_OK) return is;
      result_f = h->h_scalars[SC_TRIAL_ERR];
      const double M_error = h->h_scalars[SC_LIN0], new_M = h->h_scalars[SC_LIND];
      const double rho = (std::abs(f_error - result_f) < 1e-15 || std::abs(M_error - new_M) < 1e-15)
                             ? 0.5
                             : (f_error - result_f) / (M_error - new_M);
      if (rho >= 0.75) {
// ... 33 lines not shown
```

### gtsam_petercdev_amd/csrc/solver.hip

```cpp
#include <hip/hip_runtime.h>

#include <algorithm>
#include <cstdlib>
#include <chrono>
#include <climits>
#include <cmath>
#include <cstdio>
#include <cstring>
#include <limits>
#include <array>
#include <map>
#include <string>
#include <vector>

#include "handle.h"

using namespace gsx;

using namespace gsx;

namespace gsx {

void launch_lds_group(const DevProblem& P, const DevSymbolic& S, const int* ids, const SmallLaunch& g, const double* H,
                      const double* damp, const double* scalars, double* arena, DevStatus* status, hipStream_t st) {
  if (g.medium) launch_front_medium(P, S, ids, g.count, g.max_panel, g.max_n, H, damp, scalars, arena, status, st);
  else launch_front_small(P, S, ids, g.count, g.max_n, g.threads, H, damp, scalars, arena, status, st);
}

static const char* kPhaseNames[PH_COUNT] = {"linearize", "assemble_hessian", "factorize", "backsolve", "linear_error",
                                     "retract", "error", "factor_small", "factor_big", "factor_leaf",
                                     "big_schur", "big_rows", "big_diag", "big_gather", "backsolve_launch",
                                     "all_marginals", "marg_prep", "marg_kt", "marg_sf", "marg_ff", "marg_emit",
                                     "marg_leaf"};

void timer_begin(gsx_context* c, int ph) {
  if (c->profiling < 0) return;
  Timer& t = c->timers[ph];
  std::pair<hipEvent_t, hipEvent_t> ev;
  if (!t.pool.empty()) {
    ev = t.pool.back();
    t.pool.pop_back();
  } else {
    hipEventCreate(&ev.first);
    hipEventCreate(&ev.second);
  }
  hipEventRecord(ev.first, c->stream);
  t.pending.push_back(ev);
}
void timer_end(gsx_context* c, int ph) {
  if (c->profiling < 0) return;
  hipEventRecord(c->timers[ph].pending.back().second, c->stream);
}
static void timers_resolve(gsx_context* c) {
  hipStreamSynchronize(c->stream);
  for (int ph = 0; ph < PH_COUNT; ++ph) {
    Timer& t = c->timers[ph];
    for (auto& ev : t.pending) {
      float ms = 0;
      if (hipEventElapsedTime(&ms, ev.first, ev.second) == hipSuccess) {
        t.ms += ms;
        t.count++;
      }
      t.pool.push_back(ev);
    }
    t.pending.clear();
  }
}

static void shard_allreduce(gsx_context* c, double* dptr, int64_t n) {
  if (!c->sharded() || n <= 0) return;
  if (hipStreamSynchronize(c->stream) != hipSuccess) {
    c->shard_failed = true;
    (void)hipGetLastError();
    (void)hipMemset(dptr, 0xFF, (size_t)n * sizeof(double));
  }
  if (c->shard_cb(c->shard_user, dptr, n) != 0) c->shard_failed = true;
}

void dev_linearize(gsx_context* c) {
  timer_begin(c, PH_LINEARIZE);
  hipMemsetAsync(&c->d_status.p->n_cheirality, 0, sizeof(int), c->stream);
  c->smart_begin(true);
  const int* lists[kNumTypeLists];
  for (int k = 0; k < kNumTypeLists; ++k) lists[k] = c->d_type_list[k].p;
  launch_linearize(c->DP, lists, c->type_count, c->d_values.p, c->d_jac.p, c->d_status.p, c->stream, &c->SD);
  timer_end(c, PH_LINEARIZE);
  c->sc_dirty |= kXLin;
  c->blocks_written(true);
}

void dev_assemble_h(gsx_context* c) {
  timer_begin(c, PH_ASSEMBLE_H);
  const gsx_context::HGroup *gs = nullptr, *gd = nullptr;
  for (const auto& g : c->hgroups) {
    if (g.threads == -1 && c->n_star_bundles) gs = &g;
    if (g.threads == 0 && g.count > 0) gd = &g;
  }
  const bool fs = c->fused_star;
  const bool fused = gs && gd && !fs;
  if (fused)
    launch_assemble_h_diag_star(c->DP, c->DS, c->d_hvars.p + gd->begin, gd->count, c->d_hvars.p + gs->begin,
                                c->d_star_bundles.p, c->n_star_bundles, c->d_jac.p, c->d_H.p, c->stream);
  for (const auto& g : c->hgroups) {
    if (fused && (&g == gs || &g == gd)) continue;
    if (fs && g.threads == -1) {
      if (c->n_star_rest)
        launch_assemble_h_group(c->DP, c->DS, c->d_star_rest_vars.p, c->n_star_rest, -1, 0, false, c->d_jac.p, c->d_H.p,
                                c->stream);
      continue;
    }
    if (g.threads == -1 && c->n_star_bundles) {
      launch_assemble_h_star_bundles(c->DP, c->DS, c->d_hvars.p + g.begin, c->d_star_bundles.p, c->n_star_bundles,
                                     c->d_jac.p, c->d_H.p, c->stream);
      continue;
    }
    launch_assemble_h_group(c->DP, c->DS, c->d_hvars.p + g.begin, g.count, g.threads, g.lds, g.global, c->d_jac.p,
                            c->d_H.p, c->stream);
  }
  timer_end(c, PH_ASSEMBLE_H);
  c->h_assembled(!fs);
}

void dev_ensure_hstar(gsx_context* c) {
  if (c->hstar_ready) return;
  for (const auto& g : c->hgroups) {
    if (g.threads != -1) continue;
    if (c->n_star_bundles)
      launch_assemble_h_star_bundles(c->DP, c->DS, c->d_hvars.p + g.begin, c->d_star_bundles.p, c->n_star_bundles,
                                     c->d_jac.p, c->d_H.p, c->stream);
    else
      launch_assemble_h_group(c->DP, c->DS, c->d_hvars.p + g.begin, g.count, g.threads, g.lds, g.global, c->d_jac.p,
                              c->d_H.p, c->stream);
  }
  c->hstar_completed();
}

static void dev_hessian_diag(gsx_context* c) {
  if (c->hdiag_ready) return;
  dev_ensure_hstar(c);
  launch_hessian_diag(c->DP, c->DS, c->d_H.p, c->d_hdiag.p, c->stream);
  if (c->con_hd_n)
    launch_constraint_hdiag(c->con_hd_n, c->d_con_hd_tan.p, c->d_con_hd_ptr.p, c->d_con_hd_jidx.p, c->d_con_hd_w.p,
                            c->d_jac.p, c->d_hdiag.p, c->stream);
  if (c->sharded()) {
    launch_mask_copy(c->d_hdiag.p, c->d_sched_tan.p, c->P.tan_size, c->d_hdiag.p, c->stream);
    shard_allreduce(c, c->d_hdiag.p, c->P.tan_size);
  }
  c->hdiag_extracted();
}

void dev_damping(gsx_context* c, int diagonal, double mind, double maxd) {
  if (c->damping_is(diagonal, mind, maxd)) return;
  if (diagonal) dev_hessian_diag(c);
  launch_make_damping((int)c->P.tan_size, c->d_hdiag.p, diagonal, mind, maxd, c->d_damp.p, c->stream);
  if (c->sharded()) launch_mask_copy(c->d_damp.p, c->d_own_tan.p, c->P.tan_size, c->d_damp.p, c->stream);
  c->damping_made(diagonal, mind, maxd);
}

void dev_big_factor(gsx_context* c, const BigDesc* descs, int count, const BigPlan& plan, hipStream_t st, bool prof) {
  for (int r = 0; r < plan.rounds(); ++r) {
    if (prof) timer_begin(c, PH_K_POTRF0);
    launch_big_diag(descs, count, plan, r, c->d_arena.p, c->d_status.p, st);
    if (prof) timer_end(c, PH_K_POTRF0);
    if (prof) timer_begin(c, PH_K_TRSM);
    launch_big_rows(descs, count, plan, r, c->d_arena.p, c->d_status.p, st);
    if (prof) timer_end(c, PH_K_TRSM);
    if (prof) timer_begin(c, PH_K_SYRK);
    launch_big_schur(descs, count, plan, r, c->d_arena.p, st);
    if (prof) timer_end(c, PH_K_SYRK);
  }
}

static void debug_sync(gsx_context* c, const char* what, int a, int b) {
  static const bool on = std::getenv("GSX_DEBUG_LAUNCH") != nullptr;
  if (!on) return;
  fprintf(stderr, "[gsx] %s (%d, %d) ...", what, a, b);
  fflush(stderr);
  const hipError_t e = hipStreamSynchronize(c->stream);
  const hipError_t e2 = hipGetLastError();
  fprintf(stderr, " %s / %s\n", hipGetErrorString(e), hipGetErrorString(e2));
  fflush(stderr);
}

static void dev_leaf_group(gsx_context* c, size_t g, hipStream_t st) {
  const SmallLaunch& sl = c->leaf_launch[0][g];
  if (c->fused_star && c->leaf_split[g].scount) {
    const gsx_context::LeafSplit& ls = c->leaf_split[g];
    launch_front_star_leaf(c->DS, c->d_star_recs.p + ls.sbegin, ls.scount, c->d_star_prow.p, c->d_jac.p, c->d_damp.p,
                           c->d_scalars.p, c->d_H.p, c->d_arena.p, c->d_status.p, st);
    if (ls.rcount)
      launch_front_leaf(c->DP, c->DS, c->d_leaf_rest_recs.p + ls.rbegin, ls.rcount, sl.max_panel, sl.threads, c->d_H.p,
                        c->d_damp.p, c->d_scalars.p, c->d_arena.p, c->d_status.p, st);
    return;
  }
  launch_front_leaf(c->DP, c->DS, c->d_leaf_recs.p + (sl.begin - c->leaf_base), sl.count, sl.max_panel, sl.threads, c->d_H.p,
                    c->d_damp.p, c->d_scalars.p, c->d_arena.p, c->d_status.p, st);
}

static bool bulk_ready(gsx_context* c) {
  if (c->bulk) return true;
  int least = 0, greatest = 0;
  if (hipDeviceGetStreamPriorityRange(&least, &greatest) != hipSuccess) return false;
  if (hipStreamCreateWithPriority(&c->bulk, hipStreamNonBlocking, least) != hipSuccess) {
    c->bulk = nullptr;
    return false;
  }
  if (hipEventCreateWithFlags(&c->bulk_go, hipEventDisableTiming) != hipSuccess ||
      hipEventCreateWithFlags(&c->bulk_done, hipEventDisableTiming) != hipSuccess)
    return false;
  return true;
}

static void dev_factorize(gsx_context* c, double lambda) {
  const Symbolic& S = c->S;
  c->factorization_queued(lambda);
  c->sc_dirty |= kXFact;
  timer_begin(c, PH_FACTORIZE);
  launch_begin_factorization(c->d_scalars.p, lambda, c->d_status.p, c->d_tree_cursor.p, c->stream);
  if (!c->big_descs.empty())
    launch_big_init(c->DP, c->DS, c->d_big.p, (int)c->big_descs.size(), c->big_max_n, c->big_max_nfv, c->d_H.p,
                    c->d_damp.p, c->d_scalars.p, c->d_arena.p, c->stream);
  const int sg = S.n_ulevels;
  const bool have_side = S.side_level0 >= 0;
  const bool use_bulk = have_side && c->profiling <= 0 && bulk_ready(c);
  if (S.n_levels > 0) {
    const std::vector<SmallLaunch>& LL = c->leaf_launch[0];
    const size_t n_main_leaf = c->leaf_side_group0 != (size_t)-1 ? c->leaf_side_group0 : LL.size();
    if (use_bulk) {
      hipEventRecord(c->bulk_go, c->stream);
      hipStreamWaitEvent(c->bulk, c->bulk_go, 0);
      for (size_t g = n_main_leaf; g < LL.size(); ++g) dev_leaf_group(c, g, c->bulk);
      launch_big_gather(c->GA, S.gseg_lvl_ptr[sg], S.gseg_lvl_ptr[sg + 1] - S.gseg_lvl_ptr[sg], S.gm_lvl_ptr[sg],
                        S.gm_lvl_ptr[sg + 1] - S.gm_lvl_ptr[sg], c->d_arena.p, c->bulk);
      hipEventRecord(c->bulk_done, c->bulk);
      c->bulk_pending = true;
    }
    for (size_t g = 0; g < (use_bulk ? n_main_leaf : LL.size()); ++g) {
      if (c->profiling > 0) timer_begin(c, PH_FACTOR_LEAF);
      dev_leaf_group(c, g, c->stream);
      if (c->profiling > 0) timer_end(c, PH_FACTOR_LEAF);
    }
// ... 36 lines not shown
    }
    if (l == 0 && have_side && !use_bulk && S.gseg_lvl_ptr[sg + 1] > S.gseg_lvl_ptr[sg]) {
      if (prof) timer_begin(c, PH_K_GATHER);
      launch_big_gather(c->GA, S.gseg_lvl_ptr[sg], S.gseg_lvl_ptr[sg + 1] - S.gseg_lvl_ptr[sg], S.gm_lvl_ptr[sg],
                        S.gm_lvl_ptr[sg + 1] - S.gm_lvl_ptr[sg], c->d_arena.p, c->stream);
      if (prof) timer_end(c, PH_K_GATHER);
    }
    if (B.count) {
      if (l == S.cap_ulevel0) shard_allreduce(c, c->d_arena.p + S.cap_begin, S.cap_end - S.cap_begin);
      if (c->con_level[l].count)
        launch_constraint_fronts(c->DS, c->CT, c->con_level[l].first, c->con_level[l].count, c->con_level[l].max_n,
                                 c->d_jac.p, c->d_arena.p, c->d_status.p, c->stream);
      dev_big_factor(c, c->d_big.p + B.begin, B.count, B.plan, c->stream, prof);
      if (prof) timer_end(c, PH_FACTOR_BIG);
    }
  }
  launch_cond_check((int)S.cond_last.size(), c->d_cond_last.p, c->d_cond_prev.p, c->d_cond_front.p, c->d_arena.p,
                    c->d_status.p, c->stream);
  timer_end(c, PH_FACTORIZE);
}

static void dev_backsolve_levels(gsx_context* c, const WildfireArgs* wf) {
  const Symbolic& S = c->S;
  timer_begin(c, PH_BACKSOLVE);
  c->delta_overwritten();
  for (int l = S.n_levels - 1; l >= 0; --l) {
    const int se = S.lvl_small_end[l];
    const struct {
      int count;
    } B{S.lvl_ptr[l + 1] - se};
    const int le = S.lvl_leaf_end[l], n_rest = S.lvl_ptr[l + 1] - le;
    int big_maxn = 0, big_maxF = 0, big_maxS = 0;
    for (int k = se; k < S.lvl_ptr[l + 1]; ++k) {
      big_maxn = std::max(big_maxn, S.N[S.sched[k]]);
      big_maxF = std::max(big_maxF, S.F[S.sched[k]]);
      big_maxS = std::max(big_maxS, S.N[S.sched[k]] - S.F[S.sched[k]]);
    }
    const bool big_own = B.count > 0 && backsolve_big_lds(big_maxn, big_maxF, big_maxS) > 0;
    if (big_own) {
      if (c->profiling > 0) timer_begin(c, PH_K_BACKSOLVE);
      launch_backsolve_big(c->DS, c->d_sched.p + se, S.lvl_ptr[l + 1] - se, big_maxn, big_maxF, c->d_arena.p, c->d_delta.p,
                           c->d_status.p, c->stream);
      if (c->profiling > 0) timer_end(c, PH_K_BACKSOLVE);
    }
    const int* small_ids = c->d_sched.p + le;
    const int n_small = se - le;
    int small_maxn = 0, small_maxF = 0;
    for (int k = le; k < se; ++k) {
      small_maxn = std::max(small_maxn, S.N[S.sched[k]]);
      small_maxF = std::max(small_maxF, S.F[S.sched[k]]);
    }
    const bool small_own = n_small > 0 && backsolve_small_fits(small_maxn, small_maxF);
    if (small_own) {
      if (c->profiling > 0) timer_begin(c, PH_K_BACKSOLVE);
      launch_backsolve_small(c->DS, small_ids, n_small, small_maxF, c->d_arena.p, c->d_delta.p, c->d_status.p,
                             c->stream);
      if (c->profiling > 0) timer_end(c, PH_K_BACKSOLVE);
    }
    const bool big_left = B.count > 0 && !big_own, small_left = n_small > 0 && !small_own;
    if (big_left && small_left && n_rest <= 512 && n_rest > B.count) {
      int maxn = 0;
      for (int k = le; k < S.lvl_ptr[l + 1]; ++k) maxn = std::max(maxn, S.N[S.sched[k]]);
      if (c->profiling > 0) timer_begin(c, PH_K_BACKSOLVE);
      launch_backsolve(c->DS, c->d_sched.p + le, n_rest, 1024, maxn, c->d_arena.p, c->d_delta.p, c->d_status.p, c->stream);
      if (c->profiling > 0) timer_end(c, PH_K_BACKSOLVE);
    } else {
      if (big_left) {
        int maxn = 0;
        for (int k = se; k < S.lvl_ptr[l + 1]; ++k) maxn = std::max(maxn, S.N[S.sched[k]]);
        if (c->profiling > 0) timer_begin(c, PH_K_BACKSOLVE);
        launch_backsolve(c->DS, c->d_sched.p + se, S.lvl_ptr[l + 1] - se, 1024, maxn, c->d_arena.p, c->d_delta.p,
                         c->d_status.p, c->stream);
        if (c->profiling > 0) timer_end(c, PH_K_BACKSOLVE);
      }
      if (small_left) {
        if (c->profiling > 0) timer_begin(c, PH_K_BACKSOLVE);
        launch_backsolve(c->DS, small_ids, n_small, small_maxn <= 48 ? 64 : 256, small_maxn, c->d_arena.p,
                         c->d_delta.p, c->d_status.p, c->stream);
        if (c->profiling > 0) timer_end(c, PH_K_BACKSOLVE);
      }
    }
    if (S.lvl_leaf_end[l] > S.lvl_ptr[l])
      launch_backsolve_leaf(c->DS, c->d_leaf_recs.p + (S.lvl_ptr[l] - c->leaf_base), S.lvl_leaf_end[l] - S.lvl_ptr[l],
                            c->leaf_max_F[l], c->d_arena.p, c->d_delta.p, c->d_status.p, c->stream);
    if (wf) {
      launch_wildfire_post(c->DS, c->d_sched.p + S.lvl_ptr[l], le - S.lvl_ptr[l], false, *wf, c->d_delta.p, c->stream);
      launch_wildfire_post(c->DS, c->d_sched.p + le, n_rest, true, *wf, c->d_delta.p, c->stream);
    }
  }
  timer_end(c, PH_BACKSOLVE);
}


void dev_backsolve(gsx_context* c, const WildfireArgs* wf) {
  static const bool levels_only = std::getenv("GSX_BS_TREE_OFF") != nullptr;
  if (wf != nullptr || levels_only) {
    dev_backsolve_levels(c, wf);
    return;
  }
  const Symbolic& S = c->S;
  timer_begin(c, PH_BACKSOLVE);
  c->delta_overwritten();
  for (int l = S.n_ulevels - 1; l >= 0; --l) {
    const int b0 = S.ulvl_ptr[l], se = S.ulvl_small_end[l], e = S.ulvl_ptr[l + 1];
    if (e > se) {
      int big_maxn = 0, big_maxF = 0, big_maxS = 0;
      for (int k = se; k < e; ++k) {
        big_maxn = std::max(big_maxn, S.N[S.usched[k]]);
        big_maxF = std::max(big_maxF, S.F[S.usched[k]]);
        big_maxS = std::max(big_maxS, S.N[S.usched[k]] - S.F[S.usched[k]]);
      }
      if (c->profiling > 0) timer_begin(c, PH_K_BACKSOLVE);
      if (backsolve_big_lds(big_maxn, big_maxF, big_maxS) > 0)
        launch_backsolve_big(c->DS, c->d_usched.p + se, e - se, big_maxn, big_maxF, c->d_arena.p, c->d_delta.p, c->d_status.p,
                             c->stream);
      else
        launch_backsolve(c->DS, c->d_usched.p + se, e - se, 1024, big_maxn, c->d_arena.p, c->d_delta.p, c->d_status.p,
                         c->stream);
      if (c->profiling > 0) timer_end(c, PH_K_BACKSOLVE);
    }
    if (se > b0) {
      int maxn = 0, maxF = 0;
      for (int k = b0; k < se; ++k) {
        maxn = std::max(maxn, S.N[S.usched[k]]);
        maxF = std::max(maxF, S.F[S.usched[k]]);
      }
      if (c->profiling > 0) timer_begin(c, PH_K_BACKSOLVE);
      if (backsolve_small_fits(maxn, maxF))
        launch_backsolve_small(c->DS, c->d_usched.p + b0, se - b0, maxF, c->d_arena.p, c->d_delta.p, c->d_status.p, c->stream);
      else
        launch_backsolve(c->DS, c->d_usched.p + b0, se - b0, maxn <= 48 ? 64 : 256, maxn, c->d_arena.p, c->d_delta.p,
                         c->d_status.p, c->stream);
      if (c->profiling > 0) timer_end(c, PH_K_BACKSOLVE);
    }
  }
  if (c->bst_total > 0) {
    hipMemsetAsync(c->d_bst_counters.p, 0, 2 * sizeof(int), c->stream);
    if (++c->bst_epoch == 0) c->bst_epoch = 1;
    if (c->profiling > 0) timer_begin(c, PH_K_BACKSOLVE);
    launch_backsolve_tree(c->DS,
                          BacksolveTreeArgs{c->d_bst_roots.p, c->bst_roots, c->bst_total, c->d_bst_child_ptr.p,
                                            c->d_bst_children.p, c->d_bst_ready.p, c->d_bst_counters.p,
                                            c->d_bst_counters.p + 1, c->bst_epoch},
                          c->d_arena.p, c->d_delta.p, c->d_status.p, c->stream);
    if (c->profiling > 0) timer_end(c, PH_K_BACKSOLVE);
    debug_sync(c, "backsolve_tree", c->bst_roots, c->bst_total);
  }
  if (S.n_levels > 0 && S.lvl_leaf_end[0] > S.lvl_ptr[0])
    launch_backsolve_leaf(c->DS, c->d_leaf_recs.p + (S.lvl_ptr[0] - c->leaf_base), S.lvl_leaf_end[0] - S.lvl_ptr[0],
                          c->leaf_max_F[0], c->d_arena.p, c->d_delta.p, c->d_status.p, c->stream);
  timer_end(c, PH_BACKSOLVE);
}

void dev_linear_error(gsx_context* c, bool solved_step) {
  static const bool direct_env = std::getenv("GSX_LINERR_DIRECT") != nullptr;
  const bool direct_only = direct_env || c->constrained() || c->use_pcg();
  timer_begin(c, PH_LINERR);
  if (solved_step && !direct_only && c->h_ready) {
    if (!c->lin0_ready) {
      launch_lin0(c->DP, c->d_jac.p, c->d_partials.p, gsx_context::kPartials, c->d_scalars.p, c->stream);
      c->lin0_computed();
    }
    launch_model_error(c->DP, c->DS, c->d_hvars.p, (int)c->hv_list.size(), c->d_H.p, c->d_delta.p, c->d_damp.p,
                       c->d_partials.p, gsx_context::kPartials, c->d_scalars.p, c->stream);
  } else {
    launch_linear_error(c->DP, c->d_jac.p, c->d_delta.p, c->d_partials.p, gsx_context::kPartials, c->d_scalars.p,
                        c->lin_err_slice, c->stream);
  }
  c->sc_dirty |= (1u << SC_LIN0) | (1u << SC_LIND);
  timer_end(c, PH_LINERR);
}
void dev_retract(gsx_context* c, const double* d_delta) {
  timer_begin(c, PH_RETRACT);
  launch_retract(c->DP, c->d_values.p, d_delta, c->d_trial.p, c->stream);
  timer_end(c, PH_RETRACT);
}
void dev_error(gsx_context* c, const double* d_vals, int slot) {
  timer_begin(c, PH_ERROR);
  const int* lists[kNumTypeLists];
  for (int k = 0; k < kNumTypeLists; ++k) lists[k] = c->d_type_list[k].p;
  c->smart_begin(false);
  launch_error(c->DP, lists, c->type_count, d_vals, c->d_partials.p, gsx_context::kPartials, c->d_scalars.p, slot, c->stream,
               &c->SD);
  c->sc_dirty |= 1u << slot;
  timer_end(c, PH_ERROR);
}
gsx_status readback(gsx_context* c) {
  if (c->sharded() && c->sc_dirty) {
    launch_shard_pack(c->d_scalars.p, c->d_status.p, c->sc_dirty, c->d_xscal.p, c->stream);
    shard_allreduce(c, c->d_xscal.p, kXScalars);
    launch_shard_unpack(c->d_xscal.p, c->sc_dirty, c->d_scalars.p, c->d_status.p, c->stream);
  }
  c->sc_dirty = 0;
  if (c->shard_failed) {
    c->shard_failed = false;
    c->err = "the all-reduce callback of a sharded handle failed";
    return GSX_E_NO_DEVICE;
  }
  HIPCHK(c, hipMemcpyAsync(c->h_scalars, c->d_scalars.p, SC_COUNT * sizeof(double), hipMemcpyDeviceToHost, c->stream));
  HIPCHK(c, hipMemcpyAsync(c->h_status, c->d_status.p, sizeof(DevStatus), hipMemcpyDeviceToHost, c->stream));
  HIPCHK(c, hipStreamSynchronize(c->stream));
  HIPCHK(c, hipGetLastError());
  c->n_cheirality = c->h_status->n_cheirality;
  c->factorization_judged(c->h_status->n_fail > 0 || c->h_status->n_nonfinite > 0);
  return GSX_OK;
}

bool factorization_ok(const gsx_context* c) { return c->h_status->n_fail == 0 && c->h_status->n_nonfinite == 0; }

static uint64_t failing_key(gsx_context* c) {
  const DevStatus& s = *c->h_status;
  if (s.n_fail > 0 && s.first_front >= 0 && s.first_front < c->S.n_fronts)
    return c->P.keys[c->S.fvars[c->S.fvar_ptr[s.first_front]]];
  return c->P.n_vars ? c->P.keys[c->S.order.empty() ? 0 : c->S.order[0]] : 0;
}

gsx_status need_device(gsx_context* c) {
  if (!c->has_device) {
    c->err = "no usable gfx950 device (the hot path has no CPU fallback)";
    return GSX_E_NO_DEVICE;
  }
  return GSX_OK;
}

static gsx_status ensure_ready(gsx_context* c, bool need_values, bool need_symbolic) {
  gsx_status st = need_device(c);
  if (st != GSX_OK) return st;
  if (need_values && !c->values_set && c->P.state_size > 0) {
    c->err = "values not set";
    return GSX_E_STATE;
  }
  if (need_symbolic && !c->has_symbolic) {
    c->err = "ordering not set";
    return GSX_E_STATE;
  }
  return GSX_OK;
}
gsx_status begin_call(gsx_context* c, bool need_values, bool need_symbolic) {
  gsx_status st = ensure_ready(c, need_values, need_symbolic);
  if (st != GSX_OK) return st;
  hipSetDevice(c->device);
  return GSX_OK;
}

gsx_status indeterminate(gsx_context* c, uint64_t* bad_key, bool also_nonfinite) {
  if (!(c->h_status->n_fail > 0 || (also_nonfinite && c->h_status->n_nonfinite > 0))) return GSX_OK;
  if (bad_key) *bad_key = failing_key(c);
  c->factorization_failed();
  c->err = "indeterminate linear system";
  return GSX_E_INDETERMINATE;
}

gsx_status download(gsx_context* c, const double* src, double* out, int64_t n) {
  if (!out || n <= 0) return GSX_OK;
  HIPCHK(c, hipMemcpyAsync(out, src, n * sizeof(double), hipMemcpyDeviceToHost, c->stream));
  HIPCHK(c, hipStreamSynchronize(c->stream));
  return GSX_OK;
}

static const char* pcg_params_error(const gsx_pcg_params& p) {
  if (p.max_iterations < 0 || p.min_iterations < 0) return "PCG: negative iteration bound";
  if (p.reset < 1) return "PCG: reset must be at least 1 (the reference takes k % reset)";
  if (!(p.epsilon_rel >= 0.0) || !(p.epsilon_abs >= 0.0)) return "PCG: a negative or NaN epsilon";
  if (p.preconditioner != GSX_PRECOND_DUMMY && p.preconditioner != GSX_PRECOND_BLOCK_JACOBI)
    return "PCG: unknown preconditioner (the subgraph preconditioner is not offered)";
  return nullptr;
}
static gsx_status pcg_refusal(gsx_context* c) {
  if (c->sharded()) {
    c->err = "the PCG solver is not available on a sharded handle";
    return GSX_E_STATE;
  }
  if (!c->P.con_factor.empty()) {
    c->err = "the PCG solver is not available on a problem with hard constraints (the step there is a KKT solve)";
    return GSX_E_STATE;
  }
  return GSX_OK;
}
static gsx_status pcg_solve(gsx_context* c, double lambda, const gsx_pcg_params& prm, gsx_pcg_stats* stats, uint64_t* bad_key) {
  gsx_status rs = pcg_refusal(c);
  if (rs != GSX_OK) return rs;
  if (pcg_max_dim(c->P) > kPcgMaxDim) {
    c->err = "PCG takes variables of tangent dimension up to 32";
    return GSX_E_INVALID;
  }
  if (!c->pcg) HIPCHK(c, pcg_work_create(c->P, c->stream, &c->pcg));
  PcgScalars sc{};
  HIPCHK(c, pcg_run(c->pcg, c->d_jac.p, c->d_damp.p, lambda, prm, c->d_delta.p, c->d_status.p, c->stream, &sc));
  c->delta_overwritten();
  c->pcg_iterations += sc.k;
  c->pcg_run_iterations += sc.k;
  c->pcg_solves++;
  if (stats) {
    stats->iterations = sc.k;
    stats->converged = sc.gamma <= sc.threshold ? 1 : 0;
    stats->gamma_initial = sc.gamma0;
    stats->gamma_final = sc.gamma;
    stats->threshold = sc.threshold;
  }
  if (sc.fail) {
    c->delta_outdated();
    if (sc.fail == 2) {
      if (bad_key && sc.bad_var >= 0 && sc.bad_var < c->P.n_vars) *bad_key = c->P.keys[sc.bad_var];
      c->err = "indeterminate linear system: a diagonal block of the damped Hessian has no Cholesky factor";
    } else {
      c->err = "indeterminate linear system: p'Ap is not positive in the conjugate-gradient iteration";
    }
    return GSX_E_INDETERMINATE;
  }
  c->step_solved(false);
  return GSX_OK;
}

void direct_solve(gsx_context* c, HMode hm, int diagonal, double mind, double maxd, double lambda, bool backsolve) {
  if (hm == H_ALWAYS || (hm == H_IF_STALE && !c->h_ready)) dev_assemble_h(c);
  dev_damping(c, diagonal, mind, maxd);
  dev_factorize(c, lambda);
  if (backsolve) dev_backsolve(c);
}
gsx_status damped_step(gsx_context* c, HMode hm, int diagonal, double mind, double maxd, double lambda) {
  if (!c->use_pcg()) {
    direct_solve(c, hm, diagonal, mind, maxd, lambda, true);
    return GSX_OK;
// ... 1045 lines not shown
```

### gtsam_petercdev_amd/csrc/upload.hip

```cpp
#include <hip/hip_runtime.h>

#include <algorithm>
#include <cstdlib>
#include <chrono>
#include <climits>
#include <cmath>
#include <cstdio>
#include <cstring>
#include <limits>
#include <array>
#include <map>
#include <string>
#include <vector>

#include "handle.h"

using namespace gsx;

namespace gsx {

int factor_type_list(const HostProblem& P, int f) {
  const int kp = P.f_key_ptr[f], nk = P.f_key_ptr[f + 1] - kp;
  return type_list_of(P.f_type[f], nk > 0 ? P.types[P.f_vars[kp]] : -1, nk > 1 ? P.types[P.f_vars[kp + 1]] : -1,
                      P.f_meas_ptr[f + 1] - P.f_meas_ptr[f]);
}
gsx_status upload_factor_lists(gsx_context* c, const std::vector<char>* owned) {
  const HostProblem& P = c->P;
  hipStream_t st = c->stream;
  std::vector<int> lists[kNumTypeLists], active;
  for (int f = 0; f < P.n_factors; ++f) {
    if (owned && !(*owned)[f]) continue;
    active.push_back(f);
    const int k = factor_type_list(P, f);
    if (k >= 0) lists[k].push_back(f);
  }
  for (int k = 0; k < kNumTypeLists; ++k) {
    c->type_count[k] = (int)lists[k].size();
    HIPCHK(c, c->d_type_list[k].upload(lists[k], st));
  }
  if (owned) {
    HIPCHK(c, c->d_f_active.upload(active, st));
    c->DP.f_active = c->d_f_active.p;
  } else {
    c->DP.f_active = nullptr;
  }
  c->DP.n_active = (int)active.size();
  HIPCHK(c, hipStreamSynchronize(st));
  return GSX_OK;
}

void whiten_linear_factor(const HostProblem& P, int f, const double* src, double* J) {
  const int m = P.f_rows[f], nc = P.f_cols[f];
  std::copy(src, src + (size_t)m * nc, J);
  const double* np = P.noise.data() + P.f_noise_ptr[f];
  const int kind = P.f_noise_kind[f];
  for (int cidx = 0; cidx < nc; ++cidx) {
    if (kind == GSX_NOISE_ISOTROPIC)
      for (int r = 0; r < m; ++r) J[cidx * m + r] *= 1.0 / np[0];
    else if (kind == GSX_NOISE_DIAGONAL)
      for (int r = 0; r < m; ++r) J[cidx * m + r] *= 1.0 / np[r];
    else if (kind == GSX_NOISE_GAUSSIAN)
      for (int r = 0; r < m; ++r) {
        double sacc = 0;
        for (int k = r; k < m; ++k) sacc += np[r * m + k] * J[cidx * m + k];
        J[cidx * m + r] = sacc;
      }
  }
}

gsx_status upload_problem(gsx_context* c) {
  const HostProblem& P = c->P;
  hipStream_t st = c->stream;
  pcg_work_destroy(c->pcg);
  c->pcg = nullptr;
  HIPCHK(c, c->d_var_type.upload(P.types, st));
  HIPCHK(c, c->d_var_dim.upload(P.dims, st));
  HIPCHK(c, c->d_var_state_off.upload(P.state_off, st));
  HIPCHK(c, c->d_var_tan_off.upload(P.tan_off, st));
  HIPCHK(c, c->d_f_type.upload(P.f_type, st));
  HIPCHK(c, c->d_f_rows.upload(P.f_rows, st));
  HIPCHK(c, c->d_f_key_ptr.upload(P.f_key_ptr, st));
  HIPCHK(c, c->d_f_vars.upload(P.f_vars, st));
  HIPCHK(c, c->d_f_noise_kind.upload(P.f_noise_kind, st));
  HIPCHK(c, c->d_f_cols.upload(P.f_cols, st));
  std::vector<i64> mo(P.f_meas_ptr.begin(), P.f_meas_ptr.end()), no(P.f_noise_ptr.begin(), P.f_noise_ptr.end()),
      jo(P.f_jac_off.begin(), P.f_jac_off.end());
  HIPCHK(c, c->d_f_meas_off.upload(mo, st));
  HIPCHK(c, c->d_f_noise_off.upload(no, st));
  HIPCHK(c, c->d_f_jac_off.upload(jo, st));
  {
    int64_t worst = 0;
    bool ordered = true;
    for (int i0 = 0; i0 < P.n_factors; i0 += 64) {
      const int l = std::min(P.n_factors, i0 + 64) - 1;
      worst = std::max<int64_t>(worst, P.f_jac_off[l] + (int64_t)P.f_rows[l] * P.f_cols[l] - P.f_jac_off[i0]);
    }
    for (int f = 1; f < P.n_factors; ++f) ordered = ordered && P.f_jac_off[f] >= P.f_jac_off[f - 1];
    worst = (worst + 1) & ~(int64_t)1;
    c->lin_err_slice = (ordered && worst > 0 && 2 * worst * (int64_t)sizeof(double) <= 96 * 1024) ? (int)worst : 0;
  }
  HIPCHK(c, c->d_meas.upload(P.meas, st));
  HIPCHK(c, c->d_noise.upload(P.noise, st));
  c->con_hd_n = 0;
  if (!P.con_factor.empty()) {
    struct E {
      int tan;
      i64 jidx;
      double w;
    };
    std::vector<E> es;
    for (size_t i = 0; i < P.con_factor.size(); ++i) {
      const int f = P.con_factor[i], m = P.f_rows[f];
      int col = 0;
      for (int q = P.f_key_ptr[f]; q < P.f_key_ptr[f + 1]; ++q)
        for (int d = 0; d < P.dims[P.f_vars[q]]; ++d, ++col)
          es.push_back(E{P.tan_off[P.f_vars[q]] + d, P.f_jac_off[f] + (i64)col * m + P.con_row[i], 1.0 - 1.0 / P.con_mu[i]});
    }
    std::stable_sort(es.begin(), es.end(), [](const E& a, const E& b) { return a.tan < b.tan; });
    std::vector<int> tan, ptr;
    std::vector<i64> jidx;
    std::vector<double> w;
    for (const E& e : es) {
      if (tan.empty() || tan.back() != e.tan) {
        tan.push_back(e.tan);
        ptr.push_back((int)jidx.size());
      }
      jidx.push_back(e.jidx);
      w.push_back(e.w);
    }
    ptr.push_back((int)jidx.size());
    c->con_hd_n = (int)tan.size();
    HIPCHK(c, c->d_con_hd_tan.upload(tan, st));
    HIPCHK(c, c->d_con_hd_ptr.upload(ptr, st));
    HIPCHK(c, c->d_con_hd_jidx.upload(jidx, st));
    HIPCHK(c, c->d_con_hd_w.upload(w, st));
  }
  gsx_status fl = upload_factor_lists(c, nullptr);
  if (fl != GSX_OK) return fl;
  if (c->n_smart) {
    std::vector<int> slot(P.n_factors, -1), never(c->n_smart, -1);
    int ns = 0;
    for (int f = 0; f < P.n_factors; ++f)
      if (P.f_type[f] == GSX_F_SMART_PROJECTION) slot[f] = ns++;
    HIPCHK(c, c->d_smart_slot.upload(slot, st));
    HIPCHK(c, c->d_smart_status.upload(never, st));
    HIPCHK(c, c->d_smart_counters.alloc(2));
    HIPCHK(c, c->d_smart_cams.alloc((size_t)ns * 8 * 32));
    HIPCHK(c, c->d_smart_cache.alloc((size_t)ns * 8 * 12));
    HIPCHK(c, c->d_smart_point.alloc((size_t)ns * 3));
    HIPCHK(c, hipMemsetAsync(c->d_smart_counters.p, 0, 2 * sizeof(int), st));
    HIPCHK(c, hipMemsetAsync(c->d_smart_cache.p, 0, (size_t)ns * 8 * 12 * sizeof(double), st));
    HIPCHK(c, hipMemsetAsync(c->d_smart_point.p, 0xFF, (size_t)ns * 3 * sizeof(double), st));
    c->SD = SmartDev{c->d_smart_slot.p, c->d_smart_cams.p, c->d_smart_cache.p, c->d_smart_point.p, c->d_smart_status.p,
                     c->d_smart_counters.p, ns};
  } else {
    c->SD = SmartDev{};
  }
  HIPCHK(c, c->d_values.alloc(std::max<int64_t>(P.state_size, 1)));
  HIPCHK(c, c->d_trial.alloc(std::max<int64_t>(P.state_size, 1)));
  HIPCHK(c, c->d_delta.alloc(std::max<int64_t>(P.tan_size, 1)));
  HIPCHK(c, c->d_udelta.alloc(std::max<int64_t>(P.tan_size, 1)));
  HIPCHK(c, c->d_hdiag.alloc(std::max<int64_t>(P.tan_size, 1)));
  HIPCHK(c, c->d_damp.alloc(std::max<int64_t>(P.tan_size, 1)));
  HIPCHK(c, c->d_jac.alloc(std::max<int64_t>(P.jac_size, 1)));
  HIPCHK(c, c->d_partials.alloc(gsx_context::kPartials));
  HIPCHK(c, c->d_scalars.alloc(SC_COUNT));
  HIPCHK(c, c->d_status.alloc(1));
  if (!c->h_scalars) HIPCHK(c, hipHostMalloc((void**)&c->h_scalars, SC_COUNT * sizeof(double)));
  if (!c->h_status) HIPCHK(c, hipHostMalloc((void**)&c->h_status, sizeof(DevStatus)));
  HIPCHK(c, hipMemsetAsync(c->d_scalars.p, 0, SC_COUNT * sizeof(double), st));
  HIPCHK(c, hipMemsetAsync(c->d_delta.p, 0, std::max<int64_t>(P.tan_size, 1) * sizeof(double), st));
  {
    std::vector<double> jac;
    bool any = false;
    for (int f = 0; f < P.n_factors; ++f) any = any || P.f_type[f] == GSX_F_LINEAR;
    if (any) {
      jac.assign(P.jac_size, 0.0);
      for (int f = 0; f < P.n_factors; ++f)
        if (P.f_type[f] == GSX_F_LINEAR) whiten_linear_factor(P, f, P.meas.data() + P.f_meas_ptr[f], jac.data() + P.f_jac_off[f]);
      HIPCHK(c, hipMemcpyAsync(c->d_jac.p, jac.data(), jac.size() * sizeof(double), hipMemcpyHostToDevice, st));
      HIPCHK(c, hipStreamSynchronize(st));
    }
  }
  {
    if (P.meas.size() >= (size_t)INT32_MAX || P.noise.size() >= (size_t)INT32_MAX || P.state_size >= INT32_MAX) {
      c->err = "problem too large for 32-bit measurement / noise / state offsets";
      return GSX_E_INVALID;
    }
    std::vector<FactorRec> fr(std::max(P.n_factors, 1));
    for (int f = 0; f < P.n_factors; ++f) {
      if (P.f_cols[f] >= 32768 || P.f_rows[f] > 255) {
        c->err = "factor too wide for the packed factor record";
        return GSX_E_INVALID;
      }
      const int kp = P.f_key_ptr[f], nk = P.f_key_ptr[f + 1] - kp;
      const int v0 = nk > 0 ? P.f_vars[kp] : -1, v1 = nk > 1 ? P.f_vars[kp + 1] : -1;
      fr[f] = FactorRec{(i64)P.f_jac_off[f], v0 >= 0 ? P.state_off[v0] : -1, v1 >= 0 ? P.state_off[v1] : -1,
                        (int)P.f_meas_ptr[f], (int)P.f_noise_ptr[f],
                        P.f_type[f] | (P.f_noise_kind[f] << 8) | ((v0 >= 0 ? P.types[v0] : 0) << 24),
                        P.f_rows[f] | (std::min(v0 >= 0 ? P.dims[v0] : 0, 255) << 8) | (P.f_cols[f] << 16)};
    }
    HIPCHK(c, c->d_frec.upload(fr, st));
  }
  DevProblem& D = c->DP;
  D.n_vars = P.n_vars;
  D.n_factors = P.n_factors;
  D.frec = c->d_frec.p;
  D.var_type = c->d_var_type.p; D.var_dim = c->d_var_dim.p;
  D.var_state_off = c->d_var_state_off.p; D.var_tan_off = c->d_var_tan_off.p;
  D.f_type = c->d_f_type.p; D.f_rows = c->d_f_rows.p; D.f_key_ptr = c->d_f_key_ptr.p; D.f_vars = c->d_f_vars.p;
  D.f_noise_kind = c->d_f_noise_kind.p; D.f_cols = c->d_f_cols.p;
  D.f_meas_off = c->d_f_meas_off.p; D.f_noise_off = c->d_f_noise_off.p; D.f_jac_off = c->d_f_jac_off.p;
  D.meas = c->d_meas.p; D.noise = c->d_noise.p;
  HIPCHK(c, hipStreamSynchronize(st));
  return GSX_OK;
}

static int small_threads_for(int n) {
  static const int shift = std::getenv("GSX_SMALL_THREADS_SHIFT") ? std::atoi(std::getenv("GSX_SMALL_THREADS_SHIFT")) : 1;
  int t = 512;
  if (n <= 48) t = 64;
  else if (n <= 72) t = 128;
  else if (n <= 100) t = 256;
  return std::min(512, t << shift);
}

gsx_status upload_symbolic(gsx_context* c) {
  const Symbolic& S = c->S;
  const HostProblem& P = c->P;
  hipStream_t st = c->stream;
  c->marg_release();
  HIPCHK(c, c->d_fr_off.upload(std::vector<i64>(S.off.begin(), S.off.end()), st));
  HIPCHK(c, c->d_fr_N.upload(S.N, st));
  HIPCHK(c, c->d_fr_F.upload(S.F, st));
  HIPCHK(c, c->d_fr_nfv.upload(S.nfrontal_vars, st));
  HIPCHK(c, c->d_fr_fvar_ptr.upload(S.fvar_ptr, st));
  HIPCHK(c, c->d_fvars.upload(S.fvars, st));
  HIPCHK(c, c->d_fr_parent.upload(S.parent, st));
  {
    std::vector<int> flags(S.n_fronts);
    for (int f = 0; f < S.n_fronts; ++f) flags[f] = (S.lean[f] ? 1 : 0) | (S.cls[f] == 2 ? 2 : 0);
    HIPCHK(c, c->d_fr_lean.upload(flags, st));
  }
  if (c->sharded()) {
    gsx_status fl = upload_factor_lists(c, &S.f_owned);
    if (fl != GSX_OK) return fl;
    std::vector<unsigned char> own_tan(std::max<int64_t>(P.tan_size, 1), 0), sched_tan(own_tan.size(), 0),
        own_state(std::max<int64_t>(P.state_size, 1), 0);
    for (int v = 0; v < P.n_vars; ++v) {
      const int o = S.owner[S.front_of_var[v]];
      const bool own = o < 0 ? c->shard_rank == 0 : o == c->shard_rank;
      const bool sched = o < 0 || o == c->shard_rank;
      for (int d = 0; d < P.dims[v]; ++d) {
        own_tan[P.tan_off[v] + d] = own;
        sched_tan[P.tan_off[v] + d] = sched;
      }
      const int sd = (v + 1 < P.n_vars ? P.state_off[v + 1] : (int)P.state_size) - P.state_off[v];
      for (int d = 0; d < sd; ++d) own_state[P.state_off[v] + d] = own;
    }
    HIPCHK(c, c->d_own_tan.upload(own_tan, st));
    HIPCHK(c, c->d_sched_tan.upload(sched_tan, st));
    HIPCHK(c, c->d_own_state.upload(own_state, st));
    HIPCHK(c, c->d_xscal.alloc(kXScalars));
    HIPCHK(c, hipMemsetAsync(c->d_delta.p, 0, std::max<int64_t>(P.tan_size, 1) * sizeof(double), st));
  }
  HIPCHK(c, c->d_fr_child_ptr.upload(S.child_ptr, st));
  HIPCHK(c, c->d_children.upload(S.children, st));
  HIPCHK(c, c->d_cmap_ptr.upload(std::vector<i64>(S.cmap_ptr.begin(), S.cmap_ptr.end()), st));
  HIPCHK(c, c->d_gidx_ptr.upload(std::vector<i64>(S.gidx_ptr.begin(), S.gidx_ptr.end()), st));
  HIPCHK(c, c->d_cmap.upload(S.cmap, st));
  HIPCHK(c, c->d_gidx.upload(S.gidx, st));
  HIPCHK(c, c->d_h_off.upload(std::vector<i64>(S.h_off.begin(), S.h_off.end()), st));
  HIPCHK(c, c->d_hmap_ptr.upload(std::vector<i64>(S.hmap_ptr.begin(), S.hmap_ptr.end()), st));
  HIPCHK(c, c->d_h_rows.upload(S.h_rows, st));
  HIPCHK(c, c->d_hmap.upload(S.hmap, st));
  HIPCHK(c, c->d_h_loc.upload(S.h_loc, st));
  HIPCHK(c, c->d_term_ptr.upload(std::vector<i64>(S.term_ptr.begin(), S.term_ptr.end()), st));
  {
    std::vector<TermRec> terms(S.t_jac.size());
    for (size_t i = 0; i < terms.size(); ++i)
      terms[i] = TermRec{(i64)S.t_jac[i], S.t_m[i], S.t_colA[i], S.t_colB[i], S.t_dB[i], S.t_dst[i], 0};
    HIPCHK(c, c->d_terms.upload(terms, st));
    std::vector<VarRec> vrec(P.n_vars);
    for (int v = 0; v < P.n_vars; ++v)
      vrec[v] = VarRec{(i64)S.h_off[v], (i64)S.hmap_ptr[v], P.dims[v], S.h_rows[v], S.h_loc[v], P.tan_off[v]};
    std::vector<ChildRec> crec(S.children.size());
    for (size_t i = 0; i < crec.size(); ++i) {
      const int ch = S.children[i];
      crec[i] = ChildRec{(i64)S.off[ch] + (i64)S.F[ch] * S.N[ch] + S.F[ch], (i64)S.cmap_ptr[ch], S.N[ch],
                         S.N[ch] - S.F[ch], 0, 0};
    }
    std::vector<VarRec> fvrec(S.fvars.size());
    for (size_t i = 0; i < fvrec.size(); ++i) fvrec[i] = vrec[S.fvars[i]];
    std::vector<FrontRec> frec(S.n_fronts);
    for (int f = 0; f < S.n_fronts; ++f)
      frec[f] = FrontRec{(i64)S.off[f], S.N[f], S.F[f], S.nfrontal_vars[f], S.fvar_ptr[f], S.child_ptr[f],
                         S.child_ptr[f + 1] - S.child_ptr[f]};
    HIPCHK(c, c->d_var_recs.upload(vrec, st));
    HIPCHK(c, c->d_child_recs.upload(crec, st));
    HIPCHK(c, c->d_front_recs.upload(frec, st));
    HIPCHK(c, c->d_cond_last.upload(std::vector<i64>(S.cond_last.begin(), S.cond_last.end()), st));
    HIPCHK(c, c->d_cond_prev.upload(std::vector<i64>(S.cond_prev.begin(), S.cond_prev.end()), st));
    HIPCHK(c, c->d_cond_front.upload(S.cond_front, st));
    HIPCHK(c, c->d_fvar_recs.upload(fvrec, st));
    HIPCHK(c, hipStreamSynchronize(st));
  }
  HIPCHK(c, c->d_sched.upload(S.sched, st));
  {
    const int b = S.n_levels ? S.lvl_ptr[0] : 0, e = S.n_levels ? S.lvl_leaf_end[0] : 0;
    std::vector<LeafRec> lr((size_t)std::max(e - b, 0));
    for (int k = b; k < e; ++k) {
      const int f = S.sched[k];
      const int v0 = S.fvars[S.fvar_ptr[f]];
      lr[k - b] = LeafRec{(i64)S.off[f], (i64)S.h_off[v0], (i64)S.hmap_ptr[v0], (i64)S.gidx_ptr[f],
                          S.N[f], S.F[f], S.nfrontal_vars[f], (int)S.lean[f],
                          P.dims[v0], S.h_rows[v0], S.h_loc[v0], P.tan_off[v0],
                          S.fvar_ptr[f], f, 0, 0};
    }
    c->leaf_base = b;
    c->h_leaf_recs = lr;
    HIPCHK(c, c->d_leaf_recs.upload(lr, st));
  }
  HIPCHK(c, c->d_H.alloc(std::max<int64_t>(S.h_size, 1)));
  HIPCHK(c, c->d_arena.alloc(std::max<int64_t>(S.arena_size, 1)));
  {
    struct VI {
      int v, psize;
      int64_t terms;
    };
    std::vector<VI> light, heavy, huge, diag, star, tile;
    static const bool tile_off = std::getenv("GSX_H_TILE_OFF") != nullptr;
    auto is_tile = [&](int v) {
      const int64_t tb = S.term_ptr[v], te = S.term_ptr[v + 1];
      if (tile_off || te - tb < 2 || te - tb > 64 || (int64_t)S.h_rows[v] * P.dims[v] * 8 * 4 > 48 * 1024) return false;
      int64_t t = tb;
      while (t < te) {
        int64_t e = t + 1;
        while (e < te && S.t_jac[e] == S.t_jac[t]) ++e;
        if (S.t_m[t] > 8 || S.t_dB[e - 1] != 1 || S.t_dst[e - 1] != S.h_rows[v] - 1 || S.t_colB[e - 1] + 1 > 16) return false;
        t = e;
      }
      return true;
    };
    std::vector<int> star_dst;
    auto is_star = [&](int v) {
      const int64_t tb = S.term_ptr[v], te = S.term_ptr[v + 1];
      if (te - tb < 3 || (te - tb) % 3 != 0 || P.dims[v] > 7) return false;
      star_dst.clear();
      for (int64_t t = tb; t < te; t += 3) {
        star_dst.push_back(S.t_dst[t + 1]);
        if (S.t_dst[t] != 0 || S.t_dst[t + 2] != S.h_rows[v] - 1 || S.t_dB[t + 2] != 1) return false;
        if (S.t_dst[t + 1] == 0 || S.t_dst[t + 1] == S.h_rows[v] - 1) return false;
        if (S.t_m[t] != S.t_m[tb] || S.t_colA[t] != S.t_colA[tb] || S.t_colB[t + 1] != S.t_colB[tb + 1] ||
            S.t_dB[t + 1] != S.t_dB[tb + 1] || S.t_colB[t + 2] != S.t_colB[tb + 2] || S.t_jac[t] != S.t_jac[t + 1] ||
            S.t_jac[t] != S.t_jac[t + 2])
          return false;
      }
      std::sort(star_dst.begin(), star_dst.end());
      return std::adjacent_find(star_dst.begin(), star_dst.end()) == star_dst.end();
    };
    for (int v = 0; v < P.n_vars; ++v) {
      if (!S.scheduled[S.front_of_var[v]]) continue;
      const int psize = S.h_rows[v] * P.dims[v];
      const int64_t terms = S.term_ptr[v + 1] - S.term_ptr[v];
      if (is_star(v)) {
        star.push_back({v, psize, terms});
        continue;
      }
      if (terms >= 64 && S.h_rows[v] == P.dims[v] + 1 && P.dims[v] <= 15) diag.push_back({v, psize, terms});
      else if (is_tile(v)) tile.push_back({v, psize, terms});
      else if (terms >= 96 && (int64_t)psize * 4 * 8 <= 48 * 1024) heavy.push_back({v, psize, terms});
      else if ((int64_t)psize * 8 <= 48 * 1024) light.push_back({v, psize, terms});
      else huge.push_back({v, psize, terms});
    }
    auto by_psize = [](const VI& a, const VI& b) { return a.psize < b.psize; };
    std::stable_sort(light.begin(), light.end(), by_psize);
    std::stable_sort(heavy.begin(), heavy.end(), by_psize);
    std::vector<int> hv;
    c->hgroups.clear();
    auto emit = [&](std::vector<VI>& L, int threads, int copies, bool global) {
      size_t i = 0;
      while (i < L.size()) {
        size_t j = i;
        const int lo = std::max(L[i].psize, 128);
        while (j < L.size() && L[j].psize <= 2 * lo) ++j;
        const int maxp = L[j - 1].psize;
        c->hgroups.push_back({(int)hv.size(), (int)(j - i), threads, global ? 0 : maxp * copies * 8, global});
        for (size_t k = i; k < j; ++k) hv.push_back(L[k].v);
        i = j;
      }
    };
    std::stable_sort(tile.begin(), tile.end(), by_psize);
    emit(tile, -2, 4, false);
    emit(light, 64, 1, false);
    emit(heavy, 256, 4, false);
    emit(huge, 64, 1, true);
    c->n_star_bundles = 0;
    if (!star.empty()) {
      c->hgroups.push_back({(int)hv.size(), (int)star.size(), -1, 0, false});
      for (const VI& x : star) hv.push_back(x.v);
      auto shape = [&](int v) {
        const int64_t t = S.term_ptr[v];
        return std::array<int, 6>{P.dims[v], S.t_m[t], S.t_colA[t], S.t_colB[t + 1], S.t_dB[t + 1], S.t_colB[t + 2]};
      };
      std::vector<int2> bundles;
      size_t i = 0;
      while (i < star.size()) {
        const auto sh = shape(star[i].v);
        const int nown = sh[0] * sh[0] + sh[0];
        int nf = (int)(star[i].terms / 3), nv = 1;
        if (nf > 64 || nown > 64) {
          bundles.clear();
          break;
        }
        while (i + nv < star.size() && nv < 5 && (nv + 1) * nown <= 64 && shape(star[i + nv].v) == sh &&
               nf + (int)(star[i + nv].terms / 3) <= 64) {
          nf += (int)(star[i + nv].terms / 3);
          ++nv;
        }
        bundles.push_back(int2{(int)i, nv});
        i += nv;
      }
      c->n_star_bundles = (int)bundles.size();
      if (c->n_star_bundles) HIPCHK(c, c->d_star_bundles.upload(bundles, st));
    }
    if (!diag.empty()) {
      c->hgroups.push_back({(int)hv.size(), (int)diag.size(), 0, 0, false});
      for (const VI& x : diag) hv.push_back(x.v);
    }
    c->hv_list = hv;
    c->hv_group_of_var.assign(P.n_vars, -1);
    c->hv_pos.assign(P.n_vars, -1);
    for (size_t g = 0; g < c->hgroups.size(); ++g)
      for (int k = c->hgroups[g].begin; k < c->hgroups[g].begin + c->hgroups[g].count; ++k) {
        c->hv_group_of_var[hv[k]] = (int)g;
        c->hv_pos[hv[k]] = k;
      }
    HIPCHK(c, c->d_hvars.upload(hv, st));
  }
  c->small_launch.assign(S.n_levels, {});
  c->big_descs.clear();
  c->big_max_n = c->big_max_nfv = 0;
  c->leaf_launch.assign(S.n_levels, {});
  c->leaf_max_F.assign(S.n_levels, 0);
  std::vector<int> rest_ids;
  for (int l = 0; l < S.n_levels; ++l) {
    int i = S.lvl_ptr[l];
    for (int k = i; k < S.lvl_leaf_end[l]; ++k) c->leaf_max_F[l] = std::max(c->leaf_max_F[l], S.F[S.sched[k]]);
    const int le_all = S.lvl_leaf_end[l];
    if (l == 0) c->leaf_side_group0 = (size_t)-1;
    for (int part = 0; part < 2; ++part) {
    const int le = (l == 0 && part == 0) ? S.leaf_side_begin : le_all;
    if (l == 0 && part == 1) c->leaf_side_group0 = c->leaf_launch[l].size();
    while (i < le) {
      const int F0 = S.F[S.sched[i]], n0 = std::max(S.N[S.sched[i]], 8);
      int j = i, maxp = 0, maxn = 0;
      bool narrow = F0 <= 4;
      for (int k = i; narrow && k < le && S.F[S.sched[k]] == F0; ++k) narrow = S.lean[S.sched[k]] != 0;
      const bool all = !narrow && (le - S.lvl_ptr[l]) <= 16384;
      static const int pack_limit = std::getenv("GSX_LEAF_SPLIT") ? std::atoi(std::getenv("GSX_LEAF_SPLIT")) : (1 << 30);
      auto packable = [&](int k) { return S.N[S.sched[k]] * S.F[S.sched[k]] <= pack_limit; };
      while (j < le && (all || (S.F[S.sched[j]] == F0 &&
                                ((narrow && packable(j) == packable(i)) || (!narrow && S.N[S.sched[j]] * 2 <= n0 * 3))))) {
        maxp = std::max(maxp, S.N[S.sched[j]] * S.F[S.sched[j]]);
        maxn = std::max(maxn, S.N[S.sched[j]]);
        ++j;
      }
      int rows_below = 0;
      for (int k = i; k < j; ++k) rows_below = std::max(rows_below, S.N[S.sched[k]] - S.F[S.sched[k]]);
      c->leaf_launch[l].push_back({i, j - i, maxn, narrow ? 64 : (maxn <= 72 && rows_below <= 64 ? 64 : (maxn <= 110 ? 128 : 256)), maxp});
      i = j;
    }
    }
    const int se = S.lvl_small_end[l];
    int se_lds = se;
    while (se_lds > i && S.med[S.sched[se_lds - 1]]) --se_lds;
    while (i < se_lds) {
      const int thr = small_threads_for(S.N[S.sched[i]]);
      int j = i, maxn = 0;
      const int n0 = std::max(S.N[S.sched[i]], 12);
      while (j < se_lds && small_threads_for(S.N[S.sched[j]]) == thr && S.N[S.sched[j]] * 10 <= n0 * 16) {
        maxn = std::max(maxn, S.N[S.sched[j]]);
        ++j;
      }
      c->small_launch[l].push_back({i, j - i, maxn, thr});
      i = j;
    }
    {
      std::vector<SmallLaunch>& G = c->small_launch[l];
      std::vector<SmallLaunch> merged;
      size_t k = 0;
      while (k < G.size()) {
        const bool narrow = G[k].threads == 64;
        size_t e = k;
        int total = 0, maxn = 0, thr = 0;
        while (e < G.size() && (G[e].threads == 64) == narrow) {
          total += G[e].count;
          maxn = std::max(maxn, G[e].max_n);
          thr = std::max(thr, G[e].threads);
          ++e;
        }
        if (total <= (narrow ? 2048 : 256)) {
          merged.push_back({G[k].begin, total, maxn, thr});
        } else {
          for (size_t q = k; q < e; ++q) merged.push_back(G[q]);
        }
        k = e;
      }
      G.swap(merged);
      int total = 0, maxn = 0;
      for (const SmallLaunch& g : G) {
        total += g.count;
        maxn = std::max(maxn, g.max_n);
      }
      if (G.size() > 1 && total <= 256) {
        const SmallLaunch one{G[0].begin, total, maxn, std::max(256, small_threads_for(maxn))};
        G.assign(1, one);
      }
      if (se_lds < se) {
        SmallLaunch m{se_lds, se - se_lds, 0, 512};
        m.medium = true;
        for (int k = se_lds; k < se; ++k) {
          m.max_n = std::max(m.max_n, S.N[S.sched[k]]);
          m.max_panel = std::max(m.max_panel, S.N[S.sched[k]] * S.F[S.sched[k]]);
        }
        G.push_back(m);
      }
    }
  }
  c->big_level.assign(S.n_ulevels, BigLevel());
  c->rest_launch.assign(S.n_ulevels, {});
  for (int l = 0; l < S.n_ulevels; ++l) {
    const int b0 = S.ulvl_ptr[l], se = S.ulvl_small_end[l];
    for (int pass = 0; pass < 2; ++pass) {
      SmallLaunch r{(int)rest_ids.size(), 0, 0, 0};
      r.medium = pass == 1;
      for (int k = b0; k < se; ++k) {
        const int f = S.usched[k];
        if ((S.med[f] != 0) != r.medium) continue;
        rest_ids.push_back(f);
        r.count++;
        r.max_n = std::max(r.max_n, S.N[f]);
        r.max_F = std::max(r.max_F, S.F[f]);
        r.max_panel = std::max(r.max_panel, S.N[f] * S.F[f]);
      }
      r.threads = r.medium ? 512 : small_threads_for(r.max_n);
      if (r.count) c->rest_launch[l].push_back(r);
    }
    BigLevel& B = c->big_level[l];
    B.begin = (int)c->big_descs.size();
    for (int k = se; k < S.ulvl_ptr[l + 1]; ++k) {
      const int f = S.usched[k];
      c->big_descs.push_back(BigDesc{(i64)S.off[f], (i64)S.off[f] + big_panel_offset(S.N[f]), S.N[f], S.F[f], f,
                                     S.parent[f]});
      c->big_max_n = std::max(c->big_max_n, S.N[f]);
      c->big_max_nfv = std::max(c->big_max_nfv, S.nfrontal_vars[f]);
    }
    B.count = (int)c->big_descs.size() - B.begin;
    plan_big_group(c->big_descs.data() + B.begin, B.count, B.plan);
  }
  HIPCHK(c, c->d_usched.upload(S.usched, st));
  HIPCHK(c, c->d_rest_ids.upload(rest_ids, st));
  c->con_level.assign(S.n_ulevels, gsx_context::ConLevel());
  c->con_desc_of_front.assign(S.n_fronts, -1);
  c->CT = ConTables{};
  if (!S.con_fronts.empty()) {
    const int nc = (int)S.con_fronts.size();
    std::vector<int> perm(nc);
    for (int k = 0; k < nc; ++k) perm[k] = k;
    std::stable_sort(perm.begin(), perm.end(),
                     [&](int a, int b) { return S.ulevel[S.con_fronts[a]] < S.ulevel[S.con_fronts[b]]; });
    std::vector<int> where(nc);
    for (int k = 0; k < nc; ++k) where[perm[k]] = k;
    std::vector<ConDesc> descs(nc);
    std::vector<int> child_list;
    i64 work = 0, iwork = 0;
    for (int k = 0; k < nc; ++k) {
      const int q = perm[k], f = S.con_fronts[q], l = S.ulevel[f];
      ConDesc& d = descs[k];
      d.off = S.off[f];
      d.N = S.N[f];
      d.F = S.F[f];
      d.K = S.con_in[q];
      d.n_fwd = S.con_fwd[q];
      d.work = work;
      work += 3 * (i64)d.K * d.N;
      d.fwd = work;
      work += (i64)d.n_fwd * (d.N - d.F);
      d.iwork = iwork;
      iwork += d.N + 2 * d.K + 1;
      d.own_begin = S.con_own_ptr[q];
// ... 233 lines not shown
```

Baseline: 590.4 LM iterations/s.

## Fuse LM trial tail: lin0 during linearize, model error with retract, single final reduction

Linearization kernels now optionally emit per-block partial sums of the stored residual norm (lin0), so a separate lin0 pass is avoided. A new trial_vars kernel computes the model-error term and performs the retraction in one pass over variables. A single trial_final kernel then reduces the lin0, model and trial-error partials. The intent is to cut kernel launches and redundant passes over the Jacobian and state in each LM iteration. In exchange it adds block reductions to every linearize kernel and more state flags that must stay consistent.

```diff
diff --git a/gtsam_petercdev_amd/csrc/handle.h b/gtsam_petercdev_amd/csrc/handle.h
--- a/gtsam_petercdev_amd/csrc/handle.h
+++ b/gtsam_petercdev_amd/csrc/handle.h
@@ -216,6 +216,10 @@
   }
   DevBuf<double> d_values, d_trial, d_delta, d_udelta, d_jac, d_H, d_arena, d_hdiag, d_damp, d_partials, d_scalars;
   DevBuf<double> d_dlu, d_dld;
+  DevBuf<double> d_lin0_partials, d_model_partials;
+  DevBuf<TrialVarRec> d_trial_recs;
+  int lin0_n = 0;
+  bool lin0_lists_cover = false;
   DevBuf<DevStatus> d_status;
   double* h_scalars = nullptr;
   DevStatus* h_status = nullptr;
@@ -262,7 +266,7 @@
   DevBuf<double> d_wf_old;
   DevBuf<int> d_wf_ids;
   bool values_set = false, linearized = false, h_ready = false, hdiag_ready = false, solved = false, damp_ready = false;
-  bool lin0_ready = false;
+  bool lin0_ready = false, lin0_partials_ready = false;
   bool fact_valid = false;
   double fact_lambda = 0.0;
   bool fact_pending = false;
@@ -289,18 +293,22 @@
     if (drop_factorization) fact_valid = false;
   }
   void trial_discarded() { linearized = h_ready = solved = false; }
-  void blocks_written(bool is_linearization) {
+  void blocks_written(bool is_linearization, bool e0_partials = false) {
     if (is_linearization) linearized = true;
     else hdiag_ready = false;
     h_ready = false;
     lin0_ready = false;
+    lin0_partials_ready = is_linearization && e0_partials;
     fact_valid = false;
     solved = false;
     if (damp_kind != 0) damp_ready = false;
   }
-  void some_blocks_written() { lin0_ready = false; }
+  void some_blocks_written() { lin0_ready = lin0_partials_ready = false; }
   void linear_graph_given() { linearized = true; }
-  void lin0_computed() { lin0_ready = true; }
+  void lin0_computed() {
+    lin0_ready = true;
+    lin0_partials_ready = false;
+  }
   void h_assembled(bool star_complete) {
     h_ready = true;
     hstar_ready = star_complete;
@@ -351,7 +359,7 @@
   }
   void problem_replaced() {
     has_symbolic = values_set = linearized = h_ready = solved = false;
-    fact_valid = fact_pending = hdiag_ready = damp_ready = lin0_ready = false;
+    fact_valid = fact_pending = hdiag_ready = damp_ready = lin0_ready = lin0_partials_ready = false;
     wf_delta_valid = false;
     wf_all_replaced = true;
   }
@@ -391,9 +399,10 @@
 void dev_damping(gsx_context* c, int diagonal, double mind, double maxd);
 void dev_big_factor(gsx_context* c, const BigDesc* descs, int count, const BigPlan& plan, hipStream_t st, bool prof);
 void dev_backsolve(gsx_context* c, const WildfireArgs* wf = nullptr);
-void dev_linear_error(gsx_context* c, bool solved_step = false);
+void dev_linear_error(gsx_context* c);
 void dev_retract(gsx_context* c, const double* d_delta);
 void dev_error(gsx_context* c, const double* d_vals, int slot);
+void dev_trial_tail(gsx_context* c);
 gsx_status readback(gsx_context* c);
 bool factorization_ok(const gsx_context* c);
 gsx_status compute_error_sync(gsx_context* c, double* out);
diff --git a/gtsam_petercdev_amd/csrc/kernels.h b/gtsam_petercdev_amd/csrc/kernels.h
--- a/gtsam_petercdev_amd/csrc/kernels.h
+++ b/gtsam_petercdev_amd/csrc/kernels.h
@@ -36,6 +36,10 @@
 struct VarRec {
   i64 h_off, hmap_off;
   int dA, rows, loc, toff;
+};
+struct TrialVarRec {
+  i64 h_off;
+  int rows, dim, tan_off, state_off, type, pad;
 };
 struct LeafRec {
   i64 off, h_off, hmap_off, gidx_ptr;
@@ -158,20 +162,25 @@
   int* counters;
   int n;
 };
-void launch_linearize(const DevProblem& P, const int* const type_lists[kNumTypeLists], const int type_counts[kNumTypeLists],
-                      const double* values, double* jac, DevStatus* status, hipStream_t st, const SmartDev* smart = nullptr);
-void launch_error(const DevProblem& P, const int* const type_lists[kNumTypeLists], const int type_counts[kNumTypeLists],
-                  const double* values, double* partials, int n_partials_cap, double* scalars, int slot, hipStream_t st,
-                  const SmartDev* smart = nullptr);
+bool linearize_sums_e0(const int type_counts[kNumTypeLists]);
+int linearize_partials(const int type_counts[kNumTypeLists]);
+int launch_linearize(const DevProblem& P, const int* const type_lists[kNumTypeLists], const int type_counts[kNumTypeLists],
+                     const double* values, double* jac, DevStatus* status, hipStream_t st, const SmartDev* smart = nullptr,
+                     double* lin0_partials = nullptr);
+int launch_error(const DevProblem& P, const int* const type_lists[kNumTypeLists], const int type_counts[kNumTypeLists],
+                 const double* values, double* partials, int n_partials_cap, double* scalars, int slot, hipStream_t st,
+                 const SmartDev* smart = nullptr, bool reduce = true);
 void launch_smart_triangulate(const DevProblem& P, const int* list, int n, const double* values, const SmartDev& S, hipStream_t st);
 void launch_smart_linearize(const DevProblem& P, const int* list, int n, const SmartDev& S, double* jac, hipStream_t st);
 void launch_smart_error(const DevProblem& P, const int* list, int n, const SmartDev& S, double* partials, int blocks,
                         hipStream_t st);
 void launch_linear_error(const DevProblem& P, const double* jac, const double* delta, double* partials,
                          int n_partials_cap, double* scalars, int slice, hipStream_t st);
-void launch_lin0(const DevProblem& P, const double* jac, double* partials, int cap, double* scalars, hipStream_t st);
-void launch_model_error(const DevProblem& P, const DevSymbolic& S, const int* vars, int nvars, const double* H,
-                        const double* delta, const double* damp, double* partials, int cap, double* scalars, hipStream_t st);
+int launch_lin0(const DevProblem& P, const double* jac, double* partials, int cap, hipStream_t st);
+int launch_trial_vars(const TrialVarRec* recs, int nvars, const double* H, const double* delta, const double* damp,
+                      const double* scalars, const double* values, double* out, double* partials, int cap, hipStream_t st);
+void launch_trial_final(const double* lin0, int n_lin0, bool sum_lin0, const double* model, int n_model, const double* err,
+                        int n_err, double* scalars, int slot, hipStream_t st);
 void launch_retract(const DevProblem& P, const double* values, const double* delta, double* out, hipStream_t st);
 void launch_assemble_h_group(const DevProblem& P, const DevSymbolic& S, const int* vars, int count, int threads,
                              int lds_bytes, bool global, const double* jac, double* H, hipStream_t st);
diff --git a/gtsam_petercdev_amd/csrc/kernels.hip b/gtsam_petercdev_amd/csrc/kernels.hip
--- a/gtsam_petercdev_amd/csrc/kernels.hip
+++ b/gtsam_petercdev_amd/csrc/kernels.hip
@@ -232,10 +232,30 @@
   whiten_store<2, 13>(J, (fr.type_kind >> 8) & 0xffff, P.noise + fr.noise_off, jac + fr.jac_off);
 }
 
-__global__ void __launch_bounds__(256) linearize_bearingrange_kernel(DevProblem P, const int* list, int n,
-                                                                     const double* values, double* jac) {
+struct StoredB {
+  const double* b;
+  int m;
+};
+__device__ __forceinline__ void lin0_emit(StoredB sb, double* lin0p) {
+  if (!lin0p) return;
+  double s = 0;
+  for (int r = 0; r < sb.m; ++r) s += sb.b[r] * sb.b[r];
+  const double t = block_sum(0.5 * s);
+  if (threadIdx.x == 0) lin0p[blockIdx.x] = t;
+}
+__device__ __forceinline__ StoredB linearize_generic_located(const DevProblem& P, const int* list, int n,
+                                                             const double* values, double* jac, int bid) {
+  linearize_generic_body(P, list, n, values, jac, bid);
+  const int i = bid * blockDim.x + threadIdx.x;
+  if (i >= n) return StoredB{nullptr, 0};
+  const int f = list[i], m = P.f_rows[f];
+  return StoredB{jac + P.f_jac_off[f] + (i64)(P.f_cols[f] - 1) * m, m};
+}
+
+__device__ __forceinline__ StoredB linearize_bearingrange_factor(const DevProblem& P, const int* list, int n,
+                                                                const double* values, double* jac) {
   const int i = blockIdx.x * blockDim.x + threadIdx.x;
-  if (i >= n) return;
+  if (i >= n) return StoredB{nullptr, 0};
   const int f = list[i];
   const int kp = P.f_key_ptr[f];
   const double* pose = values + P.var_state_off[P.f_vars[kp]];
@@ -256,13 +276,18 @@
   J[10] = -wrap_angle(br[0] - z[0]);
   J[11] = -(br[1] - z[1]);
   whiten_store<2, 6>(J, P.f_noise_kind[f], P.noise + P.f_noise_off[f], jac + P.f_jac_off[f]);
+  return StoredB{jac + P.f_jac_off[f] + (6 - 1) * 2, 2};
+}
+__global__ void __launch_bounds__(256) linearize_bearingrange_kernel(DevProblem P, const int* list, int n,
+                                                                     const double* values, double* jac, double* lin0p) {
+  lin0_emit(linearize_bearingrange_factor(P, list, n, values, jac), lin0p);
 }
 
 template <bool SENSOR>
-__global__ void __launch_bounds__(256) linearize_projection_kernel(DevProblem P, const int* list, int n, const double* values,
-                                                                   double* jac, DevStatus* status) {
+__device__ __forceinline__ StoredB linearize_projection_factor(const DevProblem& P, const int* list, int n,
+                                                              const double* values, double* jac, DevStatus* status) {
   const int i = blockIdx.x * blockDim.x + threadIdx.x;
-  if (i >= n) return;
+  if (i >= n) return StoredB{nullptr, 0};
   const int f = list[i];
   const int kp = P.f_key_ptr[f];
   const double* pose = values + P.var_state_off[P.f_vars[kp]];
@@ -299,18 +324,21 @@
     if constexpr (SENSOR) atomicAdd(&status->n_cheirality, 1);
   }
   whiten_store<2, 10>(J, P.f_noise_kind[f], P.noise + P.f_noise_off[f], jac + P.f_jac_off[f]);
-}
-
-__global__ void __launch_bounds__(256) linearize_between_pose2_kernel(DevProblem P, const int* list, int n,
-                                                                      const double* values, double* jac, const int* glist,
-                                                                      int gn) {
+  return StoredB{jac + P.f_jac_off[f] + (10 - 1) * 2, 2};
+}
+template <bool SENSOR>
+__global__ void __launch_bounds__(256) linearize_projection_kernel(DevProblem P, const int* list, int n, const double* values,
+                                                                   double* jac, DevStatus* status, double* lin0p) {
+  lin0_emit(linearize_projection_factor<SENSOR>(P, list, n, values, jac, status), lin0p);
+}
+
+__device__ __forceinline__ StoredB linearize_between_pose2_factor(const DevProblem& P, const int* list, int n,
+                                                                 const double* values, double* jac, const int* glist,
+                                                                 int gn) {
   const int gb = (gn + 255) >> 8;
-  if ((int)blockIdx.x < gb) {
-    linearize_generic_body(P, glist, gn, values, jac, blockIdx.x);
-    return;
-  }
+  if ((int)blockIdx.x < gb) return linearize_generic_located(P, glist, gn, values, jac, blockIdx.x);
   const int i = ((int)blockIdx.x - gb) * blockDim.x + threadIdx.x;
-  if (i >= n) return;
+  if (i >= n) return StoredB{nullptr, 0};
   const int f = list[i];
   const FactorRec fr = P.frec[f];
   const P2 x1 = load_pose2(values + fr.s0);
@@ -327,18 +355,21 @@
   J[15] = 0; J[16] = 0; J[17] = 1;
   J[18] = -zh.x; J[19] = -zh.y; J[20] = -theta(zh);
   whiten_store<3, 7>(J, (fr.type_kind >> 8) & 0xffff, P.noise + fr.noise_off, jac + fr.jac_off);
-}
-
-__global__ void __launch_bounds__(256) linearize_between_pose3_kernel(DevProblem P, const int* list, int n,
+  return StoredB{jac + fr.jac_off + (7 - 1) * 3, 3};
+}
+__global__ void __launch_bounds__(256) linearize_between_pose2_kernel(DevProblem P, const int* list, int n,
                                                                       const double* values, double* jac, const int* glist,
-                                                                      int gn) {
+                                                                      int gn, double* lin0p) {
+  lin0_emit(linearize_between_pose2_factor(P, list, n, values, jac, glist, gn), lin0p);
+}
+
+__device__ __forceinline__ StoredB linearize_between_pose3_factor(const DevProblem& P, const int* list, int n,
+                                                                 const double* values, double* jac, const int* glist,
+                                                                 int gn) {
   const int gb = (gn + 255) >> 8;
-  if ((int)blockIdx.x < gb) {
-    linearize_generic_body(P, glist, gn, values, jac, blockIdx.x);
-    return;
-  }
+  if ((int)blockIdx.x < gb) return linearize_generic_located(P, glist, gn, values, jac, blockIdx.x);
   const int i = ((int)blockIdx.x - gb) * blockDim.x + threadIdx.x;
-  if (i >= n) return;
+  if (i >= n) return StoredB{nullptr, 0};
   const int f = list[i];
   const FactorRec fr = P.frec[f];
   const P3 x1 = load_pose3(values + fr.s0);
@@ -358,6 +389,12 @@
 #pragma unroll
   for (int r = 0; r < 6; ++r) J[72 + r] = -e[r];
   whiten_store<6, 13>(J, (fr.type_kind >> 8) & 0xffff, P.noise + fr.noise_off, jac + fr.jac_off);
+  return StoredB{jac + fr.jac_off + (13 - 1) * 6, 6};
+}
+__global__ void __launch_bounds__(256) linearize_between_pose3_kernel(DevProblem P, const int* list, int n,
+                                                                      const double* values, double* jac, const int* glist,
+                                                                      int gn, double* lin0p) {
+  lin0_emit(linearize_between_pose3_factor(P, list, n, values, jac, glist, gn), lin0p);
 }
 
 __device__ __forceinline__ void linearize_generic_body(const DevProblem& P, const int* list, int n, const double* values,
@@ -389,15 +426,16 @@
     whiten_inplace(J, m, 2 * m + 1, P.f_noise_kind[f], P.noise + P.f_noise_off[f]);
   }
 }
-__global__ void linearize_generic_kernel(DevProblem P, const int* list, int n, const double* values, double* jac) {
-  linearize_generic_body(P, list, n, values, jac, blockIdx.x);
+__global__ void linearize_generic_kernel(DevProblem P, const int* list, int n, const double* values, double* jac,
+                                         double* lin0p) {
+  lin0_emit(linearize_generic_located(P, list, n, values, jac, blockIdx.x), lin0p);
 }
 
 template <int V1, int V2, bool SENSOR>
-__global__ void __launch_bounds__(256) linearize_range_kernel(DevProblem P, const int* list, int n, const double* values,
-                                                              double* jac) {
+__device__ __forceinline__ StoredB linearize_range_factor(const DevProblem& P, const int* list, int n, const double* values,
+                                                         double* jac) {
   const int i = blockIdx.x * blockDim.x + threadIdx.x;
-  if (i >= n) return;
+  if (i >= n) return StoredB{nullptr, 0};
   const FactorRec fr = P.frec[list[i]];
   const double* a1 = values + fr.s0;
   const double* a2 = values + fr.s1;
@@ -421,6 +459,7 @@
     }
     J[NC - 1] = -(r - z);
     whiten_store<1, NC>(J, (fr.type_kind >> 8) & 0xffff, P.noise + fr.noise_off, jac + fr.jac_off);
+    return StoredB{jac + fr.jac_off + (NC - 1) * 1, 1};
   } else {
     constexpr int NC = (V2 == GSX_VAR_POSE3) ? 13 : 10;
     constexpr int TO = (V2 == GSX_VAR_POSE3) ? 9 : 0;
@@ -441,13 +480,19 @@
     }
     J[NC - 1] = -(r - z);
     whiten_store<1, NC>(J, (fr.type_kind >> 8) & 0xffff, P.noise + fr.noise_off, jac + fr.jac_off);
-  }
-}
-
-__global__ void __launch_bounds__(256) linearize_bearing_kernel(DevProblem P, const int* list, int n, const double* values,
-                                                                double* jac) {
+    return StoredB{jac + fr.jac_off + (NC - 1) * 1, 1};
+  }
+}
+template <int V1, int V2, bool SENSOR>
+__global__ void __launch_bounds__(256) linearize_range_kernel(DevProblem P, const int* list, int n, const double* values,
+                                                              double* jac, double* lin0p) {
+  lin0_emit(linearize_range_factor<V1, V2, SENSOR>(P, list, n, values, jac), lin0p);
+}
+
+__device__ __forceinline__ StoredB linearize_bearing_factor(const DevProblem& P, const int* list, int n, const double* values,
+                                                           double* jac) {
   const int i = blockIdx.x * blockDim.x + threadIdx.x;
-  if (i >= n) return;
+  if (i >= n) return StoredB{nullptr, 0};
   const FactorRec fr = P.frec[list[i]];
   const double* pose = values + fr.s0;
   const double* pt = values + fr.s1;
@@ -457,13 +502,18 @@
   J[3] = H2[0]; J[4] = H2[1];
   J[5] = -wrap_angle(br[0] - P.meas[fr.meas_off]);
   whiten_store<1, 6>(J, (fr.type_kind >> 8) & 0xffff, P.noise + fr.noise_off, jac + fr.jac_off);
+  return StoredB{jac + fr.jac_off + (6 - 1) * 1, 1};
+}
+__global__ void __launch_bounds__(256) linearize_bearing_kernel(DevProblem P, const int* list, int n, const double* values,
+                                                                double* jac, double* lin0p) {
+  lin0_emit(linearize_bearing_factor(P, list, n, values, jac), lin0p);
 }
 
 template <bool SENSOR>
-__global__ void __launch_bounds__(256) linearize_stereo_kernel(DevProblem P, const int* list, int n, const double* values,
-                                                               double* jac, DevStatus* status) {
+__device__ __forceinline__ StoredB linearize_stereo_factor(const DevProblem& P, const int* list, int n, const double* values,
+                                                          double* jac, DevStatus* status) {
   const int i = blockIdx.x * blockDim.x + threadIdx.x;
-  if (i >= n) return;
+  if (i >= n) return StoredB{nullptr, 0};
   const FactorRec fr = P.frec[list[i]];
   const double* pose = values + fr.s0;
   const double* pt = values + fr.s1;
@@ -497,12 +547,18 @@
     if constexpr (SENSOR) atomicAdd(&status->n_cheirality, 1);
   }
   whiten_store<3, 10>(J, (fr.type_kind >> 8) & 0xffff, P.noise + fr.noise_off, jac + fr.jac_off);
-}
-
-__global__ void __launch_bounds__(256) linearize_sfm2_kernel(DevProblem P, const int* list, int n, const double* values,
-                                                             double* jac, DevStatus* status) {
+  return StoredB{jac + fr.jac_off + (10 - 1) * 3, 3};
+}
+template <bool SENSOR>
+__global__ void __launch_bounds__(256) linearize_stereo_kernel(DevProblem P, const int* list, int n, const double* values,
+                                                               double* jac, DevStatus* status, double* lin0p) {
+  lin0_emit(linearize_stereo_factor<SENSOR>(P, list, n, values, jac, status), lin0p);
+}
+
+__device__ __forceinline__ StoredB linearize_sfm2_factor(const DevProblem& P, const int* list, int n, const double* values,
+                                                        double* jac, DevStatus* status) {
   const int i = blockIdx.x * blockDim.x + threadIdx.x;
-  if (i >= n) return;
+  if (i >= n) return StoredB{nullptr, 0};
   const int f = list[i];
   const FactorRec fr = P.frec[f];
   const double* pose = values + fr.s0;
@@ -539,10 +595,31 @@
     atomicAdd(&status->n_cheirality, 1);
   }
   whiten_store<2, 15>(J, (fr.type_kind >> 8) & 0xffff, P.noise + fr.noise_off, jac + fr.jac_off);
-}
-
-void launch_linearize(const DevProblem& P, const int* const type_lists[kNumTypeLists], const int type_counts[kNumTypeLists],
-                      const double* values, double* jac, DevStatus* status, hipStream_t st, const SmartDev* smart) {
+  return StoredB{jac + fr.jac_off + (15 - 1) * 2, 2};
+}
+__global__ void __launch_bounds__(256) linearize_sfm2_kernel(DevProblem P, const int* list, int n, const double* values,
+                                                             double* jac, DevStatus* status, double* lin0p) {
+  lin0_emit(linearize_sfm2_factor(P, list, n, values, jac, status), lin0p);
+}
+
+bool linearize_sums_e0(const int type_counts[kNumTypeLists]) {
+  return type_counts[TL_SFM] == 0 && type_counts[TL_SMART] == 0;
+}
+int linearize_partials(const int type_counts[kNumTypeLists]) {
+  int total = 0;
+  for (int k = 0; k < kNumTypeLists; ++k) total += (type_counts[k] + 255) / 256;
+  return total;
+}
+
+int launch_linearize(const DevProblem& P, const int* const type_lists[kNumTypeLists], const int type_counts[kNumTypeLists],
+                     const double* values, double* jac, DevStatus* status, hipStream_t st, const SmartDev* smart,
+                     double* lin0_partials) {
+  int lin0_n = 0;
+  auto lin0_at = [&](dim3 blocks) -> double* {
+    double* p = lin0_partials ? lin0_partials + lin0_n : nullptr;
+    lin0_n += (int)blocks.x;
+    return p;
+  };
   auto grid = [](int n) { return dim3((n + 255) / 256); };
   const int* glist = type_lists[3];
   int gn = type_counts[3];
@@ -557,20 +634,25 @@
   }
   if (type_counts[1]) {
     const auto gg = take(type_counts[1]);
-    linearize_between_pose2_kernel<<<gg.first, 256, 0, st>>>(P, type_lists[1], type_counts[1], values, jac, glist, gg.second);
+    linearize_between_pose2_kernel<<<gg.first, 256, 0, st>>>(P, type_lists[1], type_counts[1], values, jac, glist, gg.second,
+                                                             lin0_at(gg.first));
   }
   if (type_counts[2]) {
     const auto gg = take(type_counts[2]);
-    linearize_between_pose3_kernel<<<gg.first, 256, 0, st>>>(P, type_lists[2], type_counts[2], values, jac, glist, gg.second);
-  }
-  if (gn) linearize_generic_kernel<<<grid(gn), 256, 0, st>>>(P, glist, gn, values, jac);
+    linearize_between_pose3_kernel<<<gg.first, 256, 0, st>>>(P, type_lists[2], type_counts[2], values, jac, glist, gg.second,
+                                                             lin0_at(gg.first));
+  }
+  if (gn) linearize_generic_kernel<<<grid(gn), 256, 0, st>>>(P, glist, gn, values, jac, lin0_at(grid(gn)));
   if (type_counts[4])
     linearize_projection_kernel<false><<<grid(type_counts[4]), 256, 0, st>>>(P, type_lists[4], type_counts[4], values, jac,
-                                                                             status);
+                                                                             status, lin0_at(grid(type_counts[4])));
   if (type_counts[5])
-    linearize_bearingrange_kernel<<<grid(type_counts[5]), 256, 0, st>>>(P, type_lists[5], type_counts[5], values, jac);
+    linearize_bearingrange_kernel<<<grid(type_counts[5]), 256, 0, st>>>(P, type_lists[5], type_counts[5], values, jac,
+                                                                        lin0_at(grid(type_counts[5])));
   auto run = [&](auto kernel, int k) {
-    if (type_counts[k]) kernel<<<grid(type_counts[k]), 256, 0, st>>>(P, type_lists[k], type_counts[k], values, jac);
+    if (type_counts[k])
+      kernel<<<grid(type_counts[k]), 256, 0, st>>>(P, type_lists[k], type_counts[k], values, jac,
+                                                   lin0_at(grid(type_counts[k])));
   };
   run(linearize_range_kernel<GSX_VAR_POSE2, GSX_VAR_VECTOR, false>, TL_RANGE_POSE2_POINT);
   run(linearize_range_kernel<GSX_VAR_POSE2, GSX_VAR_POSE2, false>, TL_RANGE_POSE2_POSE);
@@ -578,7 +660,9 @@
   run(linearize_range_kernel<GSX_VAR_POSE3, GSX_VAR_POSE3, false>, TL_RANGE_POSE3_POSE);
   run(linearize_bearing_kernel, TL_BEARING);
   auto run_s = [&](auto kernel, int k) {
-    if (type_counts[k]) kernel<<<grid(type_counts[k]), 256, 0, st>>>(P, type_lists[k], type_counts[k], values, jac, status);
+    if (type_counts[k])
+      kernel<<<grid(type_counts[k]), 256, 0, st>>>(P, type_lists[k], type_counts[k], values, jac, status,
+                                                   lin0_at(grid(type_counts[k])));
   };
   run_s(linearize_stereo_kernel<false>, TL_STEREO);
   run_s(linearize_projection_kernel<true>, TL_PROJECTION_SENSOR);
@@ -592,6 +676,7 @@
     launch_smart_triangulate(P, type_lists[TL_SMART], type_counts[TL_SMART], values, *smart, st);
     launch_smart_linearize(P, type_lists[TL_SMART], type_counts[TL_SMART], *smart, jac, st);
   }
+  return lin0_partials ? lin0_n : 0;
 }
 
 template <int FT = -1, int FV = -1, bool SENSOR = false>
@@ -764,9 +849,9 @@
   if (threadIdx.x == 0) partials[blockIdx.x] = s;
 }
 
-void launch_error(const DevProblem& P, const int* const type_lists[kNumTypeLists],
-                  const int type_counts[kNumTypeLists], const double* values, double* partials, int cap, double* scalars,
-                  int slot, hipStream_t st, const SmartDev* smart) {
+int launch_error(const DevProblem& P, const int* const type_lists[kNumTypeLists],
+                 const int type_counts[kNumTypeLists], const double* values, double* partials, int cap, double* scalars,
+                 int slot, hipStream_t st, const SmartDev* smart, bool reduce) {
   long long total = 0;
   for (int k = 0; k < kNumTypeLists; ++k) total += type_counts[k];
   bool new_lists = false;
@@ -807,7 +892,8 @@
     }
     off += nb;
   }
-  reduce_final_kernel<<<1, 256, 0, st>>>(partials, off, 1, scalars, slot);
+  if (reduce) reduce_final_kernel<<<1, 256, 0, st>>>(partials, off, 1, scalars, slot);
+  return off;
 }
 
 __global__ void __launch_bounds__(256) linear_error_kernel(DevProblem P, const double* jac, const double* delta,
@@ -949,58 +1035,16 @@
   const double t = block_sum(acc);
   if (threadIdx.x == 0) partials[blockIdx.x] = t;
 }
-__global__ void __launch_bounds__(256) model_error_kernel(DevProblem P, DevSymbolic S, const int* vars, int nvars,
-                                                          const double* H, const double* delta, const double* damp,
-                                                          const double* scalars, double* partials) {
-  const double lambda = scalars[SC_LAMBDA];
-  double acc = 0;
-  for (int k = blockIdx.x * blockDim.x + threadIdx.x; k < nvars; k += gridDim.x * blockDim.x) {
-    const int v = vars[k];
-    const int d = P.var_dim[v], rows = S.h_rows[v], to = P.var_tan_off[v];
-    const double* p = H + S.h_off[v] + (rows - 1);
-    for (int j = 0; j < d; ++j) {
-      const double x = delta[to + j];
-      acc += x * (p[(i64)j * rows] + lambda * damp[to + j] * x);
-    }
-  }
-  const double t = block_sum(acc);
-  if (threadIdx.x == 0) partials[blockIdx.x] = t;
-}
-__global__ void __launch_bounds__(256) model_final_kernel(const double* partials, int n, double* scalars) {
-  double acc = 0;
-  for (int i = threadIdx.x; i < n; i += blockDim.x) acc += partials[i];
-  const double s = block_sum(acc);
-  if (threadIdx.x == 0) {
-    const double e0 = scalars[SC_LIN0_LOCAL];
-    scalars[SC_LIN0] = e0;
-    scalars[SC_LIND] = e0 - 0.5 * s;
-  }
-}
-void launch_lin0(const DevProblem& P, const double* jac, double* partials, int cap, double* scalars, hipStream_t st) {
+int launch_lin0(const DevProblem& P, const double* jac, double* partials, int cap, hipStream_t st) {
   int nb = (P.n_active + 255) / 256;
   nb = nb < 1 ? 1 : (nb > cap ? cap : nb);
   lin0_kernel<<<nb, 256, 0, st>>>(P, jac, partials);
-  reduce_final_kernel<<<1, 256, 0, st>>>(partials, nb, 1, scalars, SC_LIN0_LOCAL);
-}
-void launch_model_error(const DevProblem& P, const DevSymbolic& S, const int* vars, int nvars, const double* H,
-                        const double* delta, const double* damp, double* partials, int cap, double* scalars,
-                        hipStream_t st) {
-  int nb = (nvars + 255) / 256;
-  nb = nb < 1 ? 1 : (nb > cap ? cap : nb);
-  model_error_kernel<<<nb, 256, 0, st>>>(P, S, vars, nvars, H, delta, damp, scalars, partials);
-  model_final_kernel<<<1, 256, 0, st>>>(partials, nb, scalars);
-}
-
-__global__ void __launch_bounds__(256) retract_kernel(DevProblem P, const double* values, const double* delta,
-                                                      double* out) {
-  const int v = blockIdx.x * blockDim.x + threadIdx.x;
-  if (v >= P.n_vars) return;
-  const double* x = values + P.var_state_off[v];
-  const double* d = delta + P.var_tan_off[v];
-  double* y = out + P.var_state_off[v];
-  const int type = P.var_type[v];
+  return nb;
+}
+
+__device__ __forceinline__ void retract_var(int type, int dim, const double* x, const double* d, double* y) {
   if (type == GSX_VAR_VECTOR) {
-    for (int i = 0; i < P.var_dim[v]; ++i) y[i] = x[i] + d[i];
+    for (int i = 0; i < dim; ++i) y[i] = x[i] + d[i];
   } else if (type == GSX_VAR_POSE2) {
     const P2 r = compose(load_pose2(x), load_pose2(d));
     y[0] = r.x; y[1] = r.y; y[2] = theta(r);
@@ -1015,8 +1059,73 @@
     }
   }
 }
+__global__ void __launch_bounds__(256) retract_kernel(DevProblem P, const double* values, const double* delta,
+                                                      double* out) {
+  const int v = blockIdx.x * blockDim.x + threadIdx.x;
+  if (v >= P.n_vars) return;
+  retract_var(P.var_type[v], P.var_dim[v], values + P.var_state_off[v], delta + P.var_tan_off[v],
+              out + P.var_state_off[v]);
+}
 void launch_retract(const DevProblem& P, const double* values, const double* delta, double* out, hipStream_t st) {
   if (P.n_vars) retract_kernel<<<(P.n_vars + 255) / 256, 256, 0, st>>>(P, values, delta, out);
+}
+
+__global__ void __launch_bounds__(256) trial_vars_kernel(const TrialVarRec* recs, int nvars, const double* H,
+                                                         const double* delta, const double* damp, const double* scalars,
+                                                         const double* values, double* out, double* partials) {
+  const double lambda = scalars[SC_LAMBDA];
+  double acc = 0;
+  for (int k = blockIdx.x * blockDim.x + threadIdx.x; k < nvars; k += gridDim.x * blockDim.x) {
+    const TrialVarRec r = recs[k];
+    const int d = r.dim, rows = r.rows, to = r.tan_off;
+    const double* p = H + r.h_off + (rows - 1);
+    for (int j = 0; j < d; ++j) {
+      const double x = delta[to + j];
+      acc += x * (p[(i64)j * rows] + lambda * damp[to + j] * x);
+    }
+    if (out) retract_var(r.type, d, values + r.state_off, delta + to, out + r.state_off);
+  }
+  const double t = block_sum(acc);
+  if (threadIdx.x == 0) partials[blockIdx.x] = t;
+}
+int launch_trial_vars(const TrialVarRec* recs, int nvars, const double* H, const double* delta, const double* damp,
+                      const double* scalars, const double* values, double* out, double* partials, int cap,
+                      hipStream_t st) {
+  int nb = (nvars + 255) / 256;
+  nb = nb < 1 ? 1 : (nb > cap ? cap : nb);
+  trial_vars_kernel<<<nb, 256, 0, st>>>(recs, nvars, H, delta, damp, scalars, values, out, partials);
+  return nb;
+}
+
+__global__ void __launch_bounds__(256) trial_final_kernel(const double* lin0, int n_lin0, bool sum_lin0, const double* model,
+                                                          int n_model, const double* err, int n_err, double* scalars,
+                                                          int slot) {
+  if (blockIdx.x == 1) {
+    double acc = 0;
+    for (int i = threadIdx.x; i < n_err; i += blockDim.x) acc += err[i];
+    const double s = block_sum(acc);
+    if (threadIdx.x == 0) scalars[slot] = s;
+    return;
+  }
+  double e0 = 0;
+  if (sum_lin0) {
+    double acc = 0;
+    for (int i = threadIdx.x; i < n_lin0; i += blockDim.x) acc += lin0[i];
+    e0 = block_sum(acc);
+  }
+  double acc = 0;
+  for (int i = threadIdx.x; i < n_model; i += blockDim.x) acc += model[i];
+  const double s = block_sum(acc);
+  if (threadIdx.x == 0) {
+    if (!sum_lin0) e0 = scalars[SC_LIN0_LOCAL];
+    scalars[SC_LIN0_LOCAL] = e0;
+    scalars[SC_LIN0] = e0;
+    scalars[SC_LIND] = e0 - 0.5 * s;
+  }
+}
+void launch_trial_final(const double* lin0, int n_lin0, bool sum_lin0, const double* model, int n_model, const double* err,
+                        int n_err, double* scalars, int slot, hipStream_t st) {
+  trial_final_kernel<<<2, 256, 0, st>>>(lin0, n_lin0, sum_lin0, model, n_model, err, n_err, scalars, slot);
 }
 
 __global__ void assemble_h_kernel(DevProblem P, DevSymbolic S, const int* vars, const double* jac, double* H) {
diff --git a/gtsam_petercdev_amd/csrc/optimizers.hip b/gtsam_petercdev_amd/csrc/optimizers.hip
--- a/gtsam_petercdev_amd/csrc/optimizers.hip
+++ b/gtsam_petercdev_amd/csrc/optimizers.hip
@@ -39,9 +39,7 @@
   if (ps != GSX_OK && ps != GSX_E_INDETERMINATE) return ps;
   const bool pcg_ok = ps == GSX_OK;
   if (!pcg_ok) hipMemsetAsync(c->d_delta.p, 0, (size_t)c->P.tan_size * sizeof(double), c->stream);
-  dev_linear_error(c, true);
-  dev_retract(c, c->d_delta.p);
-  dev_error(c, c->d_trial.p, SC_TRIAL_ERR);
+  dev_trial_tail(c);
   gsx_status st = readback(c);
   if (st != GSX_OK) return st;
   const bool solved = c->use_pcg() ? pcg_ok : factorization_ok(c);
@@ -161,9 +159,7 @@
   if (relinearize) dev_linearize(h);
   st = damped_step(h, H_IF_STALE, diagonal_damping, min_diagonal, max_diagonal, lambda);
   if (st != GSX_OK) return st;
-  dev_linear_error(h, true);
-  dev_retract(h, h->d_delta.p);
-  dev_error(h, h->d_trial.p, SC_TRIAL_ERR);
+  dev_trial_tail(h);
   st = readback(h);
   if (st != GSX_OK) return st;
   if (!h->use_pcg()) {
diff --git a/gtsam_petercdev_amd/csrc/solver.hip b/gtsam_petercdev_amd/csrc/solver.hip
--- a/gtsam_petercdev_amd/csrc/solver.hip
+++ b/gtsam_petercdev_amd/csrc/solver.hip
@@ -83,10 +83,11 @@
   c->smart_begin(true);
   const int* lists[kNumTypeLists];
   for (int k = 0; k < kNumTypeLists; ++k) lists[k] = c->d_type_list[k].p;
-  launch_linearize(c->DP, lists, c->type_count, c->d_values.p, c->d_jac.p, c->d_status.p, c->stream, &c->SD);
+  c->lin0_n = launch_linearize(c->DP, lists, c->type_count, c->d_values.p, c->d_jac.p, c->d_status.p, c->stream, &c->SD,
+                               c->lin0_lists_cover ? c->d_lin0_partials.p : nullptr);
   timer_end(c, PH_LINEARIZE);
   c->sc_dirty |= kXLin;
-  c->blocks_written(true);
+  c->blocks_written(true, c->lin0_lists_cover);
 }
 
 void dev_assemble_h(gsx_context* c) {
@@ -429,23 +430,43 @@
   timer_end(c, PH_BACKSOLVE);
 }
 
-void dev_linear_error(gsx_context* c, bool solved_step) {
+void dev_linear_error(gsx_context* c) {
+  timer_begin(c, PH_LINERR);
+  launch_linear_error(c->DP, c->d_jac.p, c->d_delta.p, c->d_partials.p, gsx_context::kPartials, c->d_scalars.p,
+                      c->lin_err_slice, c->stream);
+  c->sc_dirty |= (1u << SC_LIN0) | (1u << SC_LIND);
+  timer_end(c, PH_LINERR);
+}
+void dev_trial_tail(gsx_context* c) {
   static const bool direct_env = std::getenv("GSX_LINERR_DIRECT") != nullptr;
   const bool direct_only = direct_env || c->constrained() || c->use_pcg();
+  if (direct_only || !c->h_ready) {
+    dev_linear_error(c);
+    dev_retract(c, c->d_delta.p);
+    dev_error(c, c->d_trial.p, SC_TRIAL_ERR);
+    return;
+  }
   timer_begin(c, PH_LINERR);
-  if (solved_step && !direct_only && c->h_ready) {
-    if (!c->lin0_ready) {
-      launch_lin0(c->DP, c->d_jac.p, c->d_partials.p, gsx_context::kPartials, c->d_scalars.p, c->stream);
-      c->lin0_computed();
-    }
-    launch_model_error(c->DP, c->DS, c->d_hvars.p, (int)c->hv_list.size(), c->d_H.p, c->d_delta.p, c->d_damp.p,
-                       c->d_partials.p, gsx_context::kPartials, c->d_scalars.p, c->stream);
-  } else {
-    launch_linear_error(c->DP, c->d_jac.p, c->d_delta.p, c->d_partials.p, gsx_context::kPartials, c->d_scalars.p,
-                        c->lin_err_slice, c->stream);
-  }
-  c->sc_dirty |= (1u << SC_LIN0) | (1u << SC_LIND);
+  const bool sum_lin0 = !c->lin0_ready;
+  if (sum_lin0 && !c->lin0_partials_ready)
+    c->lin0_n = launch_lin0(c->DP, c->d_jac.p, c->d_lin0_partials.p, gsx_context::kPartials, c->stream);
+  const bool all_vars = (int)c->hv_list.size() == c->P.n_vars;
+  const int n_model = launch_trial_vars(c->d_trial_recs.p, (int)c->hv_list.size(), c->d_H.p, c->d_delta.p, c->d_damp.p,
+                                        c->d_scalars.p, c->d_values.p, all_vars ? c->d_trial.p : nullptr,
+                                        c->d_model_partials.p, gsx_context::kPartials, c->stream);
   timer_end(c, PH_LINERR);
+  if (!all_vars) dev_retract(c, c->d_delta.p);
+  timer_begin(c, PH_ERROR);
+  const int* lists[kNumTypeLists];
+  for (int k = 0; k < kNumTypeLists; ++k) lists[k] = c->d_type_list[k].p;
+  c->smart_begin(false);
+  const int n_err = launch_error(c->DP, lists, c->type_count, c->d_trial.p, c->d_partials.p, gsx_context::kPartials,
+                                 c->d_scalars.p, SC_TRIAL_ERR, c->stream, &c->SD, false);
+  launch_trial_final(c->d_lin0_partials.p, c->lin0_n, sum_lin0, c->d_model_partials.p, n_model, c->d_partials.p, n_err,
+                     c->d_scalars.p, SC_TRIAL_ERR, c->stream);
+  if (sum_lin0) c->lin0_computed();
+  c->sc_dirty |= (1u << SC_LIN0) | (1u << SC_LIND) | (1u << SC_TRIAL_ERR);
+  timer_end(c, PH_ERROR);
 }
 void dev_retract(gsx_context* c, const double* d_delta) {
   timer_begin(c, PH_RETRACT);
diff --git a/gtsam_petercdev_amd/csrc/upload.hip b/gtsam_petercdev_amd/csrc/upload.hip
--- a/gtsam_petercdev_amd/csrc/upload.hip
+++ b/gtsam_petercdev_amd/csrc/upload.hip
@@ -45,6 +45,11 @@
     c->DP.f_active = nullptr;
   }
   c->DP.n_active = (int)active.size();
+  int64_t listed = 0;
+  for (int k = 0; k < kNumTypeLists; ++k) listed += c->type_count[k];
+  c->lin0_lists_cover = listed == (int64_t)active.size() && linearize_sums_e0(c->type_count);
+  HIPCHK(c, c->d_lin0_partials.alloc(std::max<int64_t>(linearize_partials(c->type_count), gsx_context::kPartials)));
+  c->some_blocks_written();
   HIPCHK(c, hipStreamSynchronize(st));
   return GSX_OK;
 }
@@ -164,6 +169,7 @@
   HIPCHK(c, c->d_damp.alloc(std::max<int64_t>(P.tan_size, 1)));
   HIPCHK(c, c->d_jac.alloc(std::max<int64_t>(P.jac_size, 1)));
   HIPCHK(c, c->d_partials.alloc(gsx_context::kPartials));
+  HIPCHK(c, c->d_model_partials.alloc(gsx_context::kPartials));
   HIPCHK(c, c->d_scalars.alloc(SC_COUNT));
   HIPCHK(c, c->d_status.alloc(1));
   if (!c->h_scalars) HIPCHK(c, hipHostMalloc((void**)&c->h_scalars, SC_COUNT * sizeof(double)));
@@ -437,6 +443,12 @@
         c->hv_pos[hv[k]] = k;
       }
     HIPCHK(c, c->d_hvars.upload(hv, st));
+    std::vector<TrialVarRec> trec(hv.size());
+    for (size_t k = 0; k < hv.size(); ++k) {
+      const int v = hv[k];
+      trec[k] = TrialVarRec{(i64)S.h_off[v], S.h_rows[v], P.dims[v], P.tan_off[v], P.state_off[v], P.types[v], 0};
+    }
+    HIPCHK(c, c->d_trial_recs.upload(trec, st));
   }
   c->small_launch.assign(S.n_levels, {});
   c->big_descs.clear();
```

After: 592.2 LM iterations/s, median of 6. No clear change (+0.3%).
